# jianwen-xie/Latent-Space-Normalizing-Flow

Measured on NVIDIA B200. Metric: langevin_latent_steps_per_sec, higher is better.
Workload: dtype fp16-hi/lo-3pass-fwd+bf16-hi/lo-3pass-bwd/f32-accumulate (fp32-equivalent)

## Files before the change

### include/lsnf.h

```cpp
#ifndef LSNF_H_
#define LSNF_H_

#include <stddef.h>
#include <stdint.h>

#ifdef __cplusplus
extern "C" {
#endif

#define LSNF_ABI_VERSION 1

typedef struct lsnf_plan lsnf_plan;
typedef void* lsnf_stream;

typedef enum lsnf_status {
  LSNF_OK = 0,
  LSNF_ERR_INVALID = -1,
  LSNF_ERR_CUDA = -2,
  LSNF_ERR_STATE = -3,
  LSNF_ERR_UNSUPPORTED = -4
} lsnf_status;

typedef enum lsnf_arch {
  LSNF_ARCH_NONE = -1,
  LSNF_ARCH_SVHN = 0,
  LSNF_ARCH_CIFAR10 = 1,
  LSNF_ARCH_CELEBA_CROP = 2,
  LSNF_ARCH_CELEBA_HQ256 = 3
} lsnf_arch;

typedef enum lsnf_gemm_impl {
  LSNF_GEMM_TCGEN05 = 0,
  LSNF_GEMM_SIMT = 1
} lsnf_gemm_impl;

typedef struct lsnf_config {
  int32_t arch;
  int32_t batch;
  int32_t nz;
  int32_t ngf;
  int32_t nc;
  int32_t f_depth;
  int32_t f_width;
  int32_t f_permutation;
  int32_t f_coupling;
  float leak;
  int32_t gemm_impl;
  int32_t bwd_passes;
  int32_t train;
  int32_t reserved[3];
} lsnf_config;

#define LSNF_FLOW_PTRS_PER_STEP 12

int lsnf_abi_version(void);
const char* lsnf_last_error(void);

int lsnf_plan_create(const lsnf_config* cfg, lsnf_plan** out);
void lsnf_plan_destroy(lsnf_plan* plan);
size_t lsnf_workspace_bytes(const lsnf_plan* plan);
int lsnf_plan_bind(lsnf_plan* plan, void* workspace, size_t bytes);

int lsnf_pack_generator_weights(lsnf_plan* plan, const float* const* weights, const float* const* biases,
                                int32_t n_layers, lsnf_stream stream);
int lsnf_pack_flow_weights(lsnf_plan* plan, const float* const* params, const int32_t* const* perm,
                           const int32_t* const* perm_inverse, const float* log_abs_det,
                           const float* const* w_inverse, lsnf_stream stream);

int lsnf_generator_forward(lsnf_plan* plan, const float* z, float* x_hat, lsnf_stream stream);
int lsnf_generator_dgrad(lsnf_plan* plan, const float* x, float sigma, float* grad_z, lsnf_stream stream);
int lsnf_flow_forward(lsnf_plan* plan, const float* z, float* z_out, float* logdet, float* logp,
                      float* grad_z, lsnf_stream stream);
int lsnf_flow_inverse(lsnf_plan* plan, const float* eps, float* z, float* neg_objective, lsnf_stream stream);
int lsnf_langevin_update(lsnf_plan* plan, float* z, const float* grad_g, const float* grad_f, float step_size,
                         const float* eps, int32_t with_noise, uint64_t seed, uint64_t sample_offset,
                         uint32_t step, float* gnorms, lsnf_stream stream);

int lsnf_langevin_run(lsnf_plan* plan, const float* z0, const float* x, int32_t steps, float step_size,
                      float sigma, int32_t with_noise, const float* eps, uint64_t seed, uint64_t sample_offset,
                      float* z_out, float* gnorms, lsnf_stream stream);
int lsnf_sample_prior(lsnf_plan* plan, const float* eps, float* x, float* z, int32_t to_unit_range, lsnf_stream stream);
size_t lsnf_generator_grad_floats(const lsnf_plan* plan);
int lsnf_generator_grad_layout(const lsnf_plan* plan, int64_t* offsets, int64_t* sizes);
int lsnf_generator_param_grads(lsnf_plan* plan, const float* z, const float* x, int32_t global_batch, float* grads,
                               float* loss, int32_t part, lsnf_stream stream);
size_t lsnf_flow_grad_floats(const lsnf_plan* plan);
int lsnf_flow_grad_layout(const lsnf_plan* plan, int64_t* offsets, int64_t* sizes);
int lsnf_flow_param_grads(lsnf_plan* plan, const float* z, int32_t global_batch, float* grads, float* loss,
                          lsnf_stream stream);
int lsnf_generator_vjp(lsnf_plan* plan, const float* grad_x_hat, float* grad_z, float* grads, lsnf_stream stream);
int lsnf_flow_vjp(lsnf_plan* plan, const float* z, const float* grad_z_out, const float* grad_logdet, float* grad_z,
                  float* grads, lsnf_stream stream);

int lsnf_adam_step(int32_t n_tensors, float* const* params, const float* const* grads, float* const* exp_avg,
                   float* const* exp_avg_sq, const int64_t* sizes, const int32_t* grad_kk, const int32_t* grad_inner,
                   float lr, float beta1, float beta2, float eps, float weight_decay, int64_t step,
                   const float* grad_scale, lsnf_stream stream);

int lsnf_plan_run_stage(lsnf_plan* plan, int32_t index, lsnf_stream stream);
int lsnf_langevin_launch_count(const lsnf_plan* plan, int32_t steps);

#define LSNF_MAX_TAPS 16
#define LSNF_MAX_PHASES 4

typedef struct lsnf_tap {
  int32_t dy, dx;
  int32_t plane;
  int32_t brow;
} lsnf_tap;

typedef struct lsnf_stage_info {
  int32_t kind;
  int32_t layer;
  int32_t grid_h, grid_w;
  int32_t box_b, box_h, box_w;
  int32_t k_per_tap;
  int32_t n_valid, n_pad;
  int32_t block_n;
  int32_t n_phases;
  int32_t n_taps[LSNF_MAX_PHASES];
  lsnf_tap taps[LSNF_MAX_PHASES][LSNF_MAX_TAPS];
  int32_t out_mul;
  int32_t out_off_y[LSNF_MAX_PHASES], out_off_x[LSNF_MAX_PHASES];
  int32_t out_phase_split;
  int32_t out_channels;
  int32_t epilogue;
  int32_t k_splits;
  int32_t a_planes;
  int32_t a_h, a_w;
  int32_t tap_gen_k;
  int32_t b_k;
  int32_t b_rows;
  int32_t operand_fp16;
  int32_t passes;
  int64_t a_offset, b_offset, out_offset;
  int64_t flops;
} lsnf_stage_info;

int lsnf_plan_num_stages(const lsnf_plan* plan);
int lsnf_plan_stage_info(const lsnf_plan* plan, int32_t index, lsnf_stage_info* out);
int lsnf_plan_pack_index(const lsnf_plan* plan, int32_t index, int32_t ci, int32_t co, int32_t ky, int32_t kx,
                         int64_t* row, int64_t* col);

#define LSNF_KERNEL_SINGLE 0
#define LSNF_KERNEL_PAIR 1
typedef struct lsnf_launch_info {
  int32_t kernel;
  int32_t grid_x, grid_y, grid_z, block;
  int32_t ring_stages;
  int32_t stage_bytes;
  int32_t smem_bytes;
  int32_t ctas_per_sm;
  int32_t tmem_columns;
  int32_t tma_store;
  int32_t stream_k;
  int32_t reserved[4];
} lsnf_launch_info;
int lsnf_plan_stage_launch_info(const lsnf_plan* plan, int32_t index, int32_t num_sms, lsnf_launch_info* out);

#ifdef __cplusplus
}
#endif
#endif
```

### latent-space-normalizing-flow_b200/_cabi.py

```python
from __future__ import annotations

import ctypes as C
import os

_HERE = os.path.dirname(os.path.abspath(__file__))
LIB_PATH = os.environ.get("LSNF_LIB") or os.path.join(_HERE, "_lib", "liblsnf_b200.so")
_lib = None

LSNF_MAX_TAPS = 16
LSNF_MAX_PHASES = 4
FLOW_PTRS_PER_STEP = 12

ARCH = {"none": -1, "svhn": 0, "cifar10": 1, "celeba_crop": 2, "celeba_hq256": 3}
GEMM_TCGEN05, GEMM_SIMT = 0, 1


class Config(C.Structure):
    _fields_ = [("arch", C.c_int32), ("batch", C.c_int32), ("nz", C.c_int32), ("ngf", C.c_int32), ("nc", C.c_int32),
                ("f_depth", C.c_int32), ("f_width", C.c_int32), ("f_permutation", C.c_int32),
                ("f_coupling", C.c_int32), ("leak", C.c_float), ("gemm_impl", C.c_int32),
                ("bwd_passes", C.c_int32), ("train", C.c_int32), ("reserved", C.c_int32 * 3)]


class Tap(C.Structure):
    _fields_ = [("dy", C.c_int32), ("dx", C.c_int32), ("plane", C.c_int32), ("brow", C.c_int32)]


class StageInfo(C.Structure):
    _fields_ = [("kind", C.c_int32), ("layer", C.c_int32), ("grid_h", C.c_int32), ("grid_w", C.c_int32),
                ("box_b", C.c_int32), ("box_h", C.c_int32), ("box_w", C.c_int32), ("k_per_tap", C.c_int32),
                ("n_valid", C.c_int32), ("n_pad", C.c_int32), ("block_n", C.c_int32), ("n_phases", C.c_int32),
                ("n_taps", C.c_int32 * LSNF_MAX_PHASES), ("taps", (Tap * LSNF_MAX_TAPS) * LSNF_MAX_PHASES),
                ("out_mul", C.c_int32), ("out_off_y", C.c_int32 * LSNF_MAX_PHASES),
                ("out_off_x", C.c_int32 * LSNF_MAX_PHASES), ("out_phase_split", C.c_int32),
                ("out_channels", C.c_int32), ("epilogue", C.c_int32), ("k_splits", C.c_int32),
                ("a_planes", C.c_int32), ("a_h", C.c_int32), ("a_w", C.c_int32), ("tap_gen_k", C.c_int32),
                ("b_k", C.c_int32), ("b_rows", C.c_int32), ("operand_fp16", C.c_int32), ("passes", C.c_int32),
                ("a_offset", C.c_int64), ("b_offset", C.c_int64), ("out_offset", C.c_int64), ("flops", C.c_int64)]


class LaunchInfo(C.Structure):
    _fields_ = [("kernel", C.c_int32), ("grid_x", C.c_int32), ("grid_y", C.c_int32), ("grid_z", C.c_int32),
                ("block", C.c_int32), ("ring_stages", C.c_int32), ("stage_bytes", C.c_int32),
                ("smem_bytes", C.c_int32), ("ctas_per_sm", C.c_int32), ("tmem_columns", C.c_int32),
                ("tma_store", C.c_int32), ("stream_k", C.c_int32), ("reserved", C.c_int32 * 4)]


KERNEL_SINGLE, KERNEL_PAIR = 0, 1

EXPORTS = {
    "lsnf_abi_version": (C.c_int, []),
    "lsnf_last_error": (C.c_char_p, []),
    "lsnf_plan_create": (C.c_int, [C.POINTER(Config), C.POINTER(C.c_void_p)]),
    "lsnf_plan_destroy": (None, [C.c_void_p]),
    "lsnf_workspace_bytes": (C.c_size_t, [C.c_void_p]),
    "lsnf_plan_bind": (C.c_int, [C.c_void_p, C.c_void_p, C.c_size_t]),
    "lsnf_pack_generator_weights": (C.c_int, [C.c_void_p, C.POINTER(C.c_void_p), C.POINTER(C.c_void_p), C.c_int32,
                                              C.c_void_p]),
    "lsnf_pack_flow_weights": (C.c_int, [C.c_void_p, C.POINTER(C.c_void_p), C.POINTER(C.c_void_p),
                                         C.POINTER(C.c_void_p), C.c_void_p, C.POINTER(C.c_void_p), C.c_void_p]),
    "lsnf_generator_forward": (C.c_int, [C.c_void_p, C.c_void_p, C.c_void_p, C.c_void_p]),
    "lsnf_generator_dgrad": (C.c_int, [C.c_void_p, C.c_void_p, C.c_float, C.c_void_p, C.c_void_p]),
    "lsnf_flow_forward": (C.c_int, [C.c_void_p, C.c_void_p, C.c_void_p, C.c_void_p, C.c_void_p, C.c_void_p,
                                    C.c_void_p]),
    "lsnf_flow_inverse": (C.c_int, [C.c_void_p, C.c_void_p, C.c_void_p, C.c_void_p, C.c_void_p]),
    "lsnf_langevin_update": (C.c_int, [C.c_void_p, C.c_void_p, C.c_void_p, C.c_void_p, C.c_float, C.c_void_p,
                                       C.c_int32, C.c_uint64, C.c_uint64, C.c_uint32, C.c_void_p, C.c_void_p]),
    "lsnf_langevin_run": (C.c_int, [C.c_void_p, C.c_void_p, C.c_void_p, C.c_int32, C.c_float, C.c_float, C.c_int32,
                                    C.c_void_p, C.c_uint64, C.c_uint64, C.c_void_p, C.c_void_p, C.c_void_p]),
    "lsnf_sample_prior": (C.c_int, [C.c_void_p, C.c_void_p, C.c_void_p, C.c_void_p, C.c_int32, C.c_void_p]),
    "lsnf_generator_grad_floats": (C.c_size_t, [C.c_void_p]),
    "lsnf_generator_grad_layout": (C.c_int, [C.c_void_p, C.POINTER(C.c_int64), C.POINTER(C.c_int64)]),
    "lsnf_generator_param_grads": (C.c_int, [C.c_void_p, C.c_void_p, C.c_void_p, C.c_int32, C.c_void_p, C.c_void_p,
                                             C.c_int32, C.c_void_p]),
    "lsnf_flow_grad_floats": (C.c_size_t, [C.c_void_p]),
    "lsnf_flow_grad_layout": (C.c_int, [C.c_void_p, C.POINTER(C.c_int64), C.POINTER(C.c_int64)]),
    "lsnf_flow_param_grads": (C.c_int, [C.c_void_p, C.c_void_p, C.c_int32, C.c_void_p, C.c_void_p, C.c_void_p]),
    "lsnf_generator_vjp": (C.c_int, [C.c_void_p, C.c_void_p, C.c_void_p, C.c_void_p, C.c_void_p]),
    "lsnf_flow_vjp": (C.c_int, [C.c_void_p, C.c_void_p, C.c_void_p, C.c_void_p, C.c_void_p, C.c_void_p, C.c_void_p]),
    "lsnf_adam_step": (C.c_int, [C.c_int32, C.POINTER(C.c_void_p), C.POINTER(C.c_void_p), C.POINTER(C.c_void_p),
                                 C.POINTER(C.c_void_p), C.POINTER(C.c_int64), C.POINTER(C.c_int32),
                                 C.POINTER(C.c_int32), C.c_float, C.c_float, C.c_float, C.c_float, C.c_float,
                                 C.c_int64, C.c_void_p, C.c_void_p]),
    "lsnf_plan_run_stage": (C.c_int, [C.c_void_p, C.c_int32, C.c_void_p]),
    "lsnf_langevin_launch_count": (C.c_int, [C.c_void_p, C.c_int32]),
    "lsnf_plan_num_stages": (C.c_int, [C.c_void_p]),
    "lsnf_plan_stage_info": (C.c_int, [C.c_void_p, C.c_int32, C.POINTER(StageInfo)]),
    "lsnf_plan_pack_index": (C.c_int, [C.c_void_p, C.c_int32, C.c_int32, C.c_int32, C.c_int32, C.c_int32,
                                       C.POINTER(C.c_int64), C.POINTER(C.c_int64)]),
    "lsnf_plan_stage_launch_info": (C.c_int, [C.c_void_p, C.c_int32, C.c_int32, C.POINTER(LaunchInfo)]),
}


def load():
    global _lib
    if _lib is not None:
        return _lib
    if not os.path.exists(LIB_PATH):
        raise RuntimeError(
            f"lsnf_b200: native library {LIB_PATH} is missing -- build it with "
            "`python __graft_entry__.py` (nvcc, sm_100a). There is no CPU or PyTorch fallback for the Langevin path.")
    lib = C.CDLL(LIB_PATH)
    for name, (res, args) in EXPORTS.items():
        fn = getattr(lib, name)
        fn.restype = res
        fn.argtypes = args
    if lib.lsnf_abi_version() != 1:
        raise RuntimeError("lsnf_b200: ABI version mismatch between _cabi.py and the built library")
    _lib = lib
    return lib


def check(rc: int, what: str):
    if rc != 0:
        msg = load().lsnf_last_error()
        raise RuntimeError(f"lsnf_b200: {what} failed ({rc}): {msg.decode() if msg else ''}")


def ptr_array(ptrs):
    arr = (C.c_void_p * len(ptrs))(*[C.c_void_p(p) for p in ptrs])
    return arr
```

### latent-space-normalizing-flow_b200/csrc/lsnf_internal.cuh

```cuda
#pragma once
#include <cuda.h>
#include <cuda_bf16.h>
#include <cuda_fp16.h>
#include <cuda_runtime.h>
#include <stdint.h>

#include <string>
#include <vector>

#include "lsnf.h"

namespace lsnf {

constexpr int BLOCK_M = 128;
constexpr int BLOCK_K = 64;

enum Epilogue : int32_t {
  EPI_ACT_HL = 0,
  EPI_OUT_TANH = 1,
  EPI_GRAD_HL = 2,
  EPI_PARTIAL = 3
};

struct TapDev {
  int16_t dy, dx, plane;
  int16_t bsh;
  int32_t brow;
};

struct PhaseDev {
  int32_t ntaps;
  int32_t mo, no;
  TapDev taps[LSNF_MAX_TAPS];
};

struct StageDev {
  const __nv_bfloat16* a;
  const __nv_bfloat16* b;
  int32_t aP, B, Hg, Wg, Ka, b_rows;
  int32_t aH, aW, tap_gen, b_k;
  int32_t bB, bH, bW;
  int32_t tiles_b, tiles_h, tiles_w;
  int32_t n_valid, n_pad, block_n;
  int32_t nphase, ksplit, it_per_split;
  int32_t epi, bias_mod, oC, ms, split;
  float leak;
  const float* bias;
  void* out;
  uint32_t* mbits;
  int64_t sP, sB, sH, sW, sPos;
  int32_t nc, Ho, Wo, pad_;
  int32_t fp16, out_fp16;
  int32_t passes, out_single;
  const float* descale;
  int64_t rows_total;
  float* sk_slots;
  int32_t* sk_flags;
  int32_t sk_enable;
  int32_t wgrad;
  int32_t out_tma, nst;
  PhaseDev ph[LSNF_MAX_PHASES];
};

struct StageHost {
  lsnf_stage_info info;
  StageDev dev;
  CUtensorMap tmA, tmB, tmO;
  bool maps_ready = false;
  int layer = 0;
  int kind = 0;
  int k = 0, s = 0, p = 0, ci = 0, co = 0;
  size_t a_off = 0, b_off = 0, out_off = 0, mbits_off = 0, bias_off = 0;
  size_t b_bytes = 0;
  bool last = false, first = false;
  int num_sms = 148;
};

struct FlowLayout {
  int nz, w, n_out, half;
  size_t an_b, an_e, an_ei, W, WT, Winv, W1, W1T, b1, e1, W2, W2T, b2, e2, W3, W3T, b3, e3, perm, perm_inv, ld_const;
  size_t step_floats;
  size_t vec_floats;
  size_t max_mat;
  size_t step_mat;
};

struct FlowStash {
  size_t y, u1, a1, a2, h, gu, gp1, gp2, gp3, gx, gl0, gl1, gl2, gl3;
  size_t layer_floats;
};

struct FlowGradLayout {
  size_t off[LSNF_FLOW_PTRS_PER_STEP];
  size_t size[LSNF_FLOW_PTRS_PER_STEP];
  size_t step_floats;
};

struct TransArgs {
  const uint16_t* src;
  uint16_t* dst;
  int P, B, H, W, C;
  long long s_plane, s_b, s_h, s_w;
  int src_fp16, src_single;
  int Hp, Wp, halo;
  long long Kp;
  int c_rows;
  int xvar;
};

struct FinalizeArgs {
  const float* part;
  float* out;
  long long s_tap, s_split, s_ci;
  int ksplit, kk, C_in, C_out;
  float scale;
};

struct RowSumArgs {
  const uint16_t* src;
  float* out;
  long long Kp;
  int nsel, C;
  float scale;
  int sel[64];
};

struct WgradLayer {
  StageHost st;
  TransArgs ta, tg;
  size_t off_aT = 0, off_gT = 0, off_part = 0;
  int a_rows = 0, g_rows = 0, planes = 1, ntaps = 1, kk = 1, ksplit = 1;
  long long Kp = 0;
  size_t grad_w_off = 0, grad_b_off = 0;
  FinalizeArgs fin;
  RowSumArgs rs;
};

}

struct lsnf_plan {
  lsnf_config cfg;
  int n_layers = 0;
  int img = 0;
  int kp = 0;
  int nzp = 0;
  struct Layer { int ci, co, k, s, p, hin, hout; } layers[8];
  std::vector<lsnf::StageHost> stages;
  lsnf::FlowLayout fl;
  std::vector<lsnf::WgradLayer> wg;
  size_t gen_grad_floats = 0;
  bool wg_ready = false;
  lsnf::FlowStash fstash;
  lsnf::FlowGradLayout fgrad;
  size_t off_fstash = 0, off_fgrad = 0, off_floss = 0, off_flinalg = 0;
  size_t ws_bytes = 0;
  size_t off_zhl = 0, off_act[8] = {0}, off_gpre[8] = {0}, off_mbits[8] = {0}, off_xhat = 0, off_im2col = 0, off_partial = 0;
  size_t off_bias[8] = {0};
  size_t off_norms = 0, off_wscale = 0, off_dlast = 0;
  int dlast_pad = 0;
  size_t off_gradg = 0, off_gradf = 0, off_z = 0, off_flow = 0, off_scalars = 0, off_flow_out = 0;
  int ksplit_first = 1;
  char* ws = nullptr;
  bool bound = false, g_packed = false, f_packed = false, have_winv = false;
  int device = -1;
  int num_sms = 148;
  cudaStream_t side = nullptr;
  cudaEvent_t ev_fork = nullptr, ev_join = nullptr;
  struct LoopGraph { int steps; float step_size, sigma; int with_noise; cudaGraphExec_t exec; };
  std::vector<LoopGraph> graphs;
  cudaStream_t cap_stream = nullptr;
  size_t off_x = 0, off_gnorms = 0, off_dyn = 0, off_sk_slots = 0, off_sk_flags = 0;
  long long runs = 0;
  bool use_graphs = true;
  int graph_chunk = 40;
};

namespace lsnf {

__device__ __forceinline__ void split16(float v, bool fp16, uint16_t& hi, uint16_t& lo) {
  if (fp16) {
    const __half h = __float2half_rn(v);
    const __half l = __float2half_rn(v - __half2float(h));
    hi = __half_as_ushort(h); lo = __half_as_ushort(l);
  } else {
    const __nv_bfloat16 h = __float2bfloat16_rn(v);
    const __nv_bfloat16 l = __float2bfloat16_rn(v - __bfloat162float(h));
    hi = __bfloat16_as_ushort(h); lo = __bfloat16_as_ushort(l);
  }
}
__device__ __forceinline__ float join16(uint16_t hi, uint16_t lo, bool fp16) {
  if (fp16) return __half2float(__ushort_as_half(hi)) + __half2float(__ushort_as_half(lo));
  return __bfloat162float(__ushort_as_bfloat16(hi)) + __bfloat162float(__ushort_as_bfloat16(lo));
}

void set_error(const std::string& msg);
int cuda_fail(cudaError_t e, const char* what);
#define LSNF_CUDA(call)                                       \
  do {                                                        \
    cudaError_t e__ = (call);                                 \
    if (e__ != cudaSuccess) return ::lsnf::cuda_fail(e__, #call); \
  } while (0)

__device__ __forceinline__ void pdl_wait() { asm volatile("griddepcontrol.wait;" ::: "memory"); }
__device__ __forceinline__ void pdl_trigger() { asm volatile("griddepcontrol.launch_dependents;" ::: "memory"); }

extern thread_local int g_launch_pdl;
struct PdlScope {
  explicit PdlScope(bool on) { g_launch_pdl = on ? 1 : 0; }
  ~PdlScope() { g_launch_pdl = 0; }
};

template <typename... KArgs, typename... Args>
inline cudaError_t launch_k(void (*kernel)(KArgs...), dim3 grid, dim3 block, size_t smem, cudaStream_t s,
                            Args&&... args) {
  cudaLaunchConfig_t cfg = {};
  cfg.gridDim = grid; cfg.blockDim = block; cfg.dynamicSmemBytes = smem; cfg.stream = s;
  cudaLaunchAttribute at[1];
  if (g_launch_pdl) {
    at[0].id = cudaLaunchAttributeProgrammaticStreamSerialization;
    at[0].val.programmaticStreamSerializationAllowed = 1;
    cfg.attrs = at; cfg.numAttrs = 1;
  }
  return cudaLaunchKernelEx(&cfg, kernel, static_cast<KArgs>(args)...);
}

int launch_tapgemm_simt(const StageHost& st, cudaStream_t s);
int launch_tapgemm_tc(const StageHost& st, cudaStream_t s);
int tc_encode_maps(lsnf_plan* plan, StageHost& st);
void tc_launch_info(const StageHost& st, int num_sms, lsnf_launch_info* out);
bool tc_stage_is_pair(const StageHost& st);
int launch_pack_stage(const lsnf_plan* plan, const StageHost& st, const float* w, cudaStream_t s);
int launch_split_z(const lsnf_plan* plan, const float* z, cudaStream_t s);
int launch_weight_scales(const lsnf_plan* plan, const float* const* weights, cudaStream_t s);
int launch_last_gather(const lsnf_plan* plan, float* out, int to_unit_range, cudaStream_t s);
int launch_recon_grad_im2col(const lsnf_plan* plan, const float* x, float seed_scale, int upstream, cudaStream_t s);
int launch_last_fused(const lsnf_plan* plan, const float* x, float seed_scale, cudaStream_t s);
int launch_transpose_hl(const TransArgs& a, cudaStream_t s);
int launch_wgrad_finalize(const FinalizeArgs& a, cudaStream_t s);
int launch_bias_rowsum(const RowSumArgs& a, cudaStream_t s);
int launch_mse_sum(const float* xh, const float* x, long long n, float scale, float* partial, unsigned int* ticket,
                   float* out, cudaStream_t s);
int launch_reduce_partial(const lsnf_plan* plan, float* grad_z, float scale, cudaStream_t s);
int launch_flow_pack(lsnf_plan* plan, const float* const* params, const int32_t* const* perm,
                     const int32_t* const* perm_inv, const float* log_abs_det, const float* const* winv,
                     cudaStream_t s);
int launch_flow_forward(const lsnf_plan* plan, const float* z, float* z_out, float* logdet, float* logp,
                        float* grad_z, cudaStream_t s);
int launch_flow_inverse(const lsnf_plan* plan, const float* eps, float* z, float* negobj, cudaStream_t s);
int flow_smem(const FlowLayout& f, int S, int depth, bool stash, bool both_passes, uint32_t* ring_floats,
              size_t* smem_bytes);
constexpr int FLOW_SMEM_BYTES = 227 * 1024;
int launch_adam(int n, float* const* params, const float* const* grads, float* const* m, float* const* v,
                const int64_t* sizes, const int32_t* grad_kk, const int32_t* grad_inner, float lr, float beta1,
                float beta2, float eps, float weight_decay, int64_t step, const float* grad_scale, cudaStream_t s);
int launch_flow_logdet_inverse(const lsnf_plan* plan, const float* const* params, float* winv, float* logdet,
                               cudaStream_t s);
int launch_flow_param_grads(const lsnf_plan* plan, const float* z, float inv_global_batch, float* grads, float* loss,
                            cudaStream_t s);
int launch_flow_vjp(const lsnf_plan* plan, const float* z, const float* seed_g, const float* seed_ld, float* grad_z,
                    float* grads, cudaStream_t s);
int launch_update(const lsnf_plan* plan, float* z, const float* gg, const float* partial, int nsplit, float gscale,
                  const float* gf, float step, const float* eps, int with_noise, uint64_t seed,
                  uint64_t sample_offset, uint32_t step_idx, const uint64_t* dyn, float* gnorms,
                  int write_zhl, cudaStream_t s);
int launch_set_dyn(const lsnf_plan* plan, uint64_t seed, uint64_t sample_offset, uint32_t base_step, cudaStream_t s);
int tc_prepare_device(int device);
int aux_prepare_device(int device);
int flow_prepare_device(int device);

inline float sigma_seed_scale(float sigma) {
  const float inv = 1.f / (sigma * sigma);
  float s = 1.f;
  while (s * 2.f <= inv && s < 16.f) s *= 2.f;
  return s;
}
inline float sigma_post_scale(float sigma) { return 1.f / (sigma * sigma) / sigma_seed_scale(sigma); }

struct PackGeom {
  int kind, first, last, k, ci, co, n_pad, ka;
};

__host__ __device__ inline bool pack_index(const PackGeom& g, int ci, int co, int ky, int kx, long long* row,
                                           long long* col) {
  const int tap = ky * g.k + kx;
  if (g.kind == 0) {
    if (g.first || g.last) {
      *row = (long long)tap * g.co + co;
      *col = ci;
    } else {
      *row = (long long)tap * g.n_pad + co;
      *col = ci;
    }
  } else {
    if (g.first) {
      *row = ci;
      *col = (long long)tap * g.co + co;
    } else if (g.last) {
      *row = ci;
      *col = (long long)tap * g.co + co;
    } else {
      *row = (long long)tap * g.n_pad + ci;
      *col = co;
    }
  }
  return true;
}

}
```

### latent-space-normalizing-flow_b200/csrc/plan.cu

```cuda
#include <algorithm>
#include <cstdio>
#include <cstdlib>
#include <cstring>

#include "lsnf_internal.cuh"

#ifndef LSNF_PDL_DEFAULT
#define LSNF_PDL_DEFAULT 1
#endif

namespace lsnf {

thread_local int g_launch_pdl = 0;
static thread_local std::string g_err;
void set_error(const std::string& msg) { g_err = msg; }
int cuda_fail(cudaError_t e, const char* what) {
  g_err = std::string("CUDA error: ") + cudaGetErrorString(e) + " in " + what;
  return LSNF_ERR_CUDA;
}

static size_t align_up(size_t v, size_t a) { return (v + a - 1) / a * a; }

static int fail(int code, const std::string& msg) {
  set_error(msg);
  return code;
}

static int arch_layers(const lsnf_config& c, lsnf_plan::Layer* L) {
  const int nz = c.nz, g = c.ngf, nc = c.nc;
  auto set = [&](int i, int ci, int co, int k, int s, int p) { L[i] = {ci, co, k, s, p, 0, 0}; };
  switch (c.arch) {
    case LSNF_ARCH_NONE:
      return 0;
    case LSNF_ARCH_SVHN:
      set(0, nz, g * 8, 4, 1, 0); set(1, g * 8, g * 4, 4, 2, 1); set(2, g * 4, g * 2, 4, 2, 1);
      set(3, g * 2, nc, 4, 2, 1);
      return 4;
    case LSNF_ARCH_CIFAR10:
      set(0, nz, g * 8, 8, 1, 0); set(1, g * 8, g * 4, 4, 2, 1); set(2, g * 4, g * 2, 4, 2, 1);
      set(3, g * 2, nc, 3, 1, 1);
      return 4;
    case LSNF_ARCH_CELEBA_CROP:
      set(0, nz, g * 8, 4, 1, 0); set(1, g * 8, g * 4, 4, 2, 1); set(2, g * 4, g * 2, 4, 2, 1);
      set(3, g * 2, g, 4, 2, 1); set(4, g, nc, 4, 2, 1);
      return 5;
    case LSNF_ARCH_CELEBA_HQ256:
      set(0, nz, g * 16, 4, 1, 0); set(1, g * 16, g * 8, 4, 2, 1); set(2, g * 8, g * 4, 4, 2, 1);
      set(3, g * 4, g * 2, 4, 2, 1); set(4, g * 2, g, 4, 2, 1); set(5, g, g, 4, 2, 1); set(6, g, nc, 4, 2, 1);
      return 7;
    default:
      return -1;
  }
}

static int pick_block_n(int n) {
  if (n % 256 == 0) return 256;
  if (n % 128 == 0) return 128;
  return 64;
}

static int pick_block_n_hidden(int n, int rows, int phases, int k_blocks) {
  const int bn = pick_block_n(n);
  if (bn != 256 || k_blocks > 32) return bn;
  const int mtiles = (rows + BLOCK_M - 1) / BLOCK_M;
  const int pair_tiles = (mtiles + 1) / 2 * (n / 256) * phases;
  const int small_tiles = mtiles * (n / 128) * phases;
  return (pair_tiles <= 37 && small_tiles <= 2 * 148) ? 128 : 256;
}

static void make_box(int hg, int wg, int* bb, int* bh, int* bw) {
  *bw = std::min(wg, BLOCK_M);
  *bh = std::min(hg, BLOCK_M / *bw);
  *bb = BLOCK_M / (*bw * *bh);
}

static int up2_fwd_taps(int py, int px, int n_pad, lsnf_tap* t) {
  int n = 0;
  for (int ky = 0; ky < 4; ++ky) {
    if (((ky + 1) & 1) != py) continue;
    const int dy = (py + 1 - ky) / 2;
    for (int kx = 0; kx < 4; ++kx) {
      if (((kx + 1) & 1) != px) continue;
      const int dx = (px + 1 - kx) / 2;
      t[n++] = {dy, dx, 0, (ky * 4 + kx) * n_pad};
    }
  }
  return n;
}

static int up2_bwd_taps(int n_pad, lsnf_tap* t) {
  int n = 0;
  for (int ky = 0; ky < 4; ++ky) {
    const int oy_off = ky - 1;
    const int py = oy_off & 1, dy = (oy_off - py) / 2;
    for (int kx = 0; kx < 4; ++kx) {
      const int ox_off = kx - 1;
      const int px = ox_off & 1, dx = (ox_off - px) / 2;
      t[n++] = {dy, dx, py * 2 + px, (ky * 4 + kx) * n_pad};
    }
  }
  return n;
}

static void fill_dev(lsnf_plan* p, StageHost& st) {
  const lsnf_stage_info& I = st.info;
  StageDev& d = st.dev;
  memset(&d, 0, sizeof(d));
  d.aP = I.a_planes; d.B = p->cfg.batch; d.Hg = I.grid_h; d.Wg = I.grid_w; d.Ka = I.k_per_tap;
  d.bB = I.box_b; d.bH = I.box_h; d.bW = I.box_w;
  d.aH = I.a_h; d.aW = I.a_w; d.tap_gen = I.tap_gen_k; d.b_k = I.b_k; d.b_rows = I.b_rows;
  d.tiles_b = (d.B + d.bB - 1) / d.bB; d.tiles_h = d.Hg / d.bH; d.tiles_w = d.Wg / d.bW;
  d.n_valid = I.n_valid; d.n_pad = I.n_pad; d.block_n = I.block_n;
  d.nphase = I.n_phases; d.ksplit = I.k_splits;
  {
    const int ntaps0 = I.tap_gen_k ? I.tap_gen_k * I.tap_gen_k : I.n_taps[0];
    const int total = ntaps0 * (I.k_per_tap / BLOCK_K);
    d.it_per_split = (total + I.k_splits - 1) / I.k_splits;
  }
  d.epi = I.epilogue; d.oC = I.out_channels; d.ms = I.out_mul; d.split = I.out_phase_split;
  d.leak = p->cfg.leak;
  d.fp16 = I.operand_fp16; d.passes = I.passes;
  const bool single_bwd = p->cfg.bwd_passes == 1;
  d.out_fp16 = (I.epilogue == EPI_ACT_HL || single_bwd) ? 1 : 0;
  d.out_single = (I.epilogue == EPI_GRAD_HL && single_bwd) ? 1 : 0;
  d.rows_total = (int64_t)p->cfg.batch * I.grid_h * I.grid_w;
  for (int ph = 0; ph < I.n_phases; ++ph) {
    d.ph[ph].ntaps = I.tap_gen_k ? I.tap_gen_k * I.tap_gen_k : I.n_taps[ph];
    d.ph[ph].mo = I.out_off_y[ph]; d.ph[ph].no = I.out_off_x[ph];
    for (int t = 0; t < I.n_taps[ph]; ++t) {
      const lsnf_tap& s = I.taps[ph][t];
      d.ph[ph].taps[t] = {(int16_t)s.dy, (int16_t)s.dx, (int16_t)s.plane, 0, s.brow};
    }
  }
}

}

using namespace lsnf;

extern "C" int lsnf_abi_version(void) { return LSNF_ABI_VERSION; }
extern "C" const char* lsnf_last_error(void) { return g_err.c_str(); }

extern "C" int lsnf_plan_create(const lsnf_config* cfg, lsnf_plan** out) {
  if (!cfg || !out) return fail(LSNF_ERR_INVALID, "null argument");
  const lsnf_config& c = *cfg;
  if (c.batch <= 0) return fail(LSNF_ERR_INVALID, "batch must be positive");
  if (c.nz <= 0 || (c.nz & 1)) return fail(LSNF_ERR_INVALID, "nz must be even (model.py:383)");
  if (c.nz % 4) return fail(LSNF_ERR_INVALID, "nz must be a multiple of 4 (128-bit latent rows)");
  if (c.nz > 256) return fail(LSNF_ERR_INVALID, "nz > 256 is not supported");
  if (c.f_depth <= 0 || c.f_depth > 32) return fail(LSNF_ERR_INVALID, "f_depth out of range");
  if (c.f_width <= 0 || c.f_width > 256 || c.f_width % 4) return fail(LSNF_ERR_INVALID, "f_width must be a multiple of 4, <= 256");
  if (c.f_permutation != 1 && c.f_permutation != 2)
    return fail(LSNF_ERR_UNSUPPORTED, "f_flow_permutation must be 1 or 2 (model.py:372-379)");
  if (c.f_coupling != 0 && c.f_coupling != 1)
    return fail(LSNF_ERR_UNSUPPORTED, "f_flow_coupling must be 0 or 1 (model.py:384-387)");
  if (c.gemm_impl != LSNF_GEMM_TCGEN05 && c.gemm_impl != LSNF_GEMM_SIMT) return fail(LSNF_ERR_INVALID, "bad gemm_impl");
  if (c.bwd_passes != 0 && c.bwd_passes != 1 && c.bwd_passes != 3) return fail(LSNF_ERR_INVALID, "bwd_passes must be 0, 1 or 3");

  lsnf_plan* p = new lsnf_plan();
  p->cfg = c;
  const int L = arch_layers(c, p->layers);
  if (L < 0) { delete p; return fail(LSNF_ERR_INVALID, "unknown arch (model.py:154 raises ValueError)"); }
  p->n_layers = L;
  p->kp = (int)align_up(c.nz, BLOCK_K);
  p->nzp = (int)align_up(c.nz, 128);
  const int B = c.batch;

  if (L > 0) {
    if (c.nc <= 0 || c.nc > 4) { delete p; return fail(LSNF_ERR_INVALID, "nc must be in 1..4"); }
    if (c.ngf <= 0) { delete p; return fail(LSNF_ERR_INVALID, "ngf must be positive"); }
    int h = 1;
    for (int l = 0; l < L; ++l) {
      auto& y = p->layers[l];
      y.hin = h;
      y.hout = (h - 1) * y.s - 2 * y.p + y.k;
      h = y.hout;
      if (l < L - 1 && y.co % BLOCK_K) {
        delete p;
        return fail(LSNF_ERR_INVALID, "hidden generator channel counts must be multiples of 64 (raise --ngf)");
      }
      if (y.hin > 128) { delete p; return fail(LSNF_ERR_INVALID, "layer grid wider than 128 not supported"); }
    }
    p->img = h;
  }

  size_t off = 0;
  auto take = [&](size_t bytes) { size_t o = off; off = align_up(off + bytes, 1024); return o; };
  p->off_z = take((size_t)B * c.nz * 4);
  p->off_gradg = take((size_t)B * c.nz * 4);
  p->off_gradf = take((size_t)B * c.nz * 4);
  p->off_scalars = take(256);
  p->off_dyn = take(64);
  p->off_gnorms = take(64);
  p->off_norms = take((size_t)2 * B * 4);
  p->off_flow_out = take((size_t)B * (c.nz + 2) * 4);
  {
    FlowLayout& f = p->fl;
    f.nz = c.nz; f.w = c.f_width; f.half = c.nz / 2; f.n_out = c.f_coupling ? c.nz : c.nz / 2;
    size_t o = 0;
    auto tk = [&](size_t n) { size_t r = o; o += (n + 3) / 4 * 4; return r; };
    f.an_b = tk(f.nz); f.an_e = tk(f.nz); f.an_ei = tk(f.nz);
    f.b1 = tk(f.w); f.e1 = tk(f.w); f.b2 = tk(f.w); f.e2 = tk(f.w); f.b3 = tk(f.n_out); f.e3 = tk(f.n_out);
    f.perm = tk(f.nz); f.perm_inv = tk(f.nz); f.ld_const = tk(4);
    f.vec_floats = o;
    f.W = tk((size_t)f.nz * f.nz); f.WT = tk((size_t)f.nz * f.nz); f.Winv = tk((size_t)f.nz * f.nz);
    f.W1 = tk((size_t)f.half * f.w); f.W1T = tk((size_t)f.half * f.w);
    f.W2 = tk((size_t)f.w * f.w); f.W2T = tk((size_t)f.w * f.w);
    f.W3 = tk((size_t)f.w * f.n_out); f.W3T = tk((size_t)f.w * f.n_out);
    const size_t w_floats = c.f_permutation == 2 ? (size_t)f.nz * f.nz : 0;
    f.max_mat = std::max({w_floats, (size_t)f.half * f.w, (size_t)f.w * f.w, (size_t)f.w * f.n_out});
    f.step_mat = w_floats + (size_t)f.half * f.w + (size_t)f.w * f.w + (size_t)f.w * f.n_out;
    f.step_floats = o;
    uint32_t ring_floats;
    size_t smem_bytes;
    if (flow_smem(f, 1, c.f_depth, true, true, &ring_floats, &smem_bytes)) {
      delete p;
      return fail(LSNF_ERR_INVALID,
                  "flow prior exceeds the " + std::to_string(FLOW_SMEM_BYTES / 1024) +
                      " KB of shared memory of one CTA even at one sample per CTA: its largest matrix (f_width^2, or "
                      "nz^2 with f_flow_permutation 2) plus f_depth * (2 f_width + nz) stashed activations must fit "
                      "(include/lsnf.h, lsnf_config)");
    }
    p->off_flow = take(f.step_floats * 4 * c.f_depth);
    FlowStash& t = p->fstash;
    size_t so = 0;
    auto ts = [&](size_t n) { size_t r = so; so += n; return r; };
    t.y = ts(f.nz); t.u1 = ts(f.half); t.a1 = ts(f.w); t.a2 = ts(f.w); t.h = ts(f.n_out);
    t.gu = ts(f.nz); t.gp1 = ts(f.w); t.gp2 = ts(f.w); t.gp3 = ts(f.n_out); t.gx = ts(f.nz);
    t.gl0 = ts(f.nz); t.gl1 = ts(f.w); t.gl2 = ts(f.w); t.gl3 = ts(f.n_out);
    t.layer_floats = so;
    p->off_fstash = take(so * 4 * (size_t)B * c.f_depth);
    p->off_flinalg = take(((size_t)c.f_depth * f.nz * f.nz + 32) * 4);
    FlowGradLayout& gl = p->fgrad;
    const size_t sizes[LSNF_FLOW_PTRS_PER_STEP] = {
        (size_t)f.nz, (size_t)f.nz, (size_t)f.nz * f.nz, (size_t)f.half * f.w, (size_t)f.w, (size_t)f.w,
        (size_t)f.w * f.w, (size_t)f.w, (size_t)f.w, (size_t)f.w * f.n_out, (size_t)f.n_out, (size_t)f.n_out};
    size_t go = 0;
    for (int i = 0; i < LSNF_FLOW_PTRS_PER_STEP; ++i) { gl.off[i] = go; gl.size[i] = sizes[i]; go += (sizes[i] + 3) / 4 * 4; }
    gl.step_floats = go;
  }

  if (L > 0) {
    p->off_zhl = take((size_t)B * 2 * p->kp * 2);
    p->off_sk_slots = take((size_t)160 * 128 * 256 * 4);
    p->off_sk_flags = take((size_t)160 * 8 * 4);
    p->off_x = take((size_t)B * c.nc * p->img * p->img * 4);
    for (int l = 0; l < L - 1; ++l) {
      const auto& y = p->layers[l];
      const size_t bytes = (size_t)B * y.hout * y.hout * 2 * y.co * 2;
      p->off_act[l] = take(bytes);
      p->off_gpre[l] = take(bytes);
      p->off_mbits[l] = take((size_t)B * y.hout * y.hout * y.co / 8);
    }
    for (int l = 0; l < L; ++l) p->off_bias[l] = take((size_t)p->layers[l].co * 4);
    p->off_xhat = take((size_t)B * c.nc * p->img * p->img * 4);
    p->off_wscale = take((size_t)L * 16);
    {
      const auto& ylast = p->layers[L - 1];
      const int kk = ylast.k * ylast.k * ylast.co;
      p->off_dlast = take((size_t)B * ylast.hin * ylast.hin * (kk <= 32 ? 32 : 64) * 4);
    }
    const auto& yl = p->layers[L - 1];
    p->off_im2col = take((size_t)B * yl.hin * yl.hin * 2 * BLOCK_K * 2);

    p->stages.resize(2 * L);
    for (int l = 0; l < L; ++l) {
      const auto& y = p->layers[l];
      StageHost& st = p->stages[l];
      lsnf_stage_info& I = st.info;
      memset(&I, 0, sizeof(I));
      st.layer = l; st.kind = 0; st.k = y.k; st.s = y.s; st.p = y.p; st.ci = y.ci; st.co = y.co;
      st.first = (l == 0); st.last = (l == L - 1);
      I.kind = 0; I.layer = l;
      I.a_planes = 1;
      I.k_splits = 1;
      if (st.first) {
        if (!(y.s == 1 && y.p == 0)) { delete p; return fail(LSNF_ERR_INVALID, "first layer must be s1 p0"); }
        if (st.last) { delete p; return fail(LSNF_ERR_INVALID, "single-layer generator not supported"); }
        I.grid_h = I.grid_w = 1;
        I.k_per_tap = p->kp;
        I.n_valid = y.k * y.k * y.co; I.n_pad = I.n_valid; I.block_n = pick_block_n(y.co);
        I.n_phases = 1; I.n_taps[0] = 1; I.taps[0][0] = {0, 0, 0, 0};
        I.out_mul = 1; I.out_channels = y.co; I.epilogue = EPI_ACT_HL;
        st.a_off = p->off_zhl;
      } else {
        I.grid_h = I.grid_w = y.hin;
        I.k_per_tap = y.ci;
        I.out_channels = y.co;
        if (st.last) {
          if (!((y.k == 4 && y.s == 2 && y.p == 1) || (y.k == 3 && y.s == 1 && y.p == 1))) {
            delete p; return fail(LSNF_ERR_INVALID, "unsupported last-layer geometry");
          }
          I.n_valid = y.k * y.k * y.co; I.n_pad = I.n_valid <= 32 ? 32 : 64; I.block_n = I.n_pad;
          I.epilogue = EPI_PARTIAL; I.out_channels = I.n_pad;
          I.n_phases = 1; I.out_mul = 1; I.n_taps[0] = 1; I.taps[0][0] = {0, 0, 0, 0};
          p->dlast_pad = I.n_pad;
        } else {
          I.n_valid = I.n_pad = y.co; I.epilogue = EPI_ACT_HL;
          I.block_n = pick_block_n_hidden(y.co, B * y.hin * y.hin, (y.k == 4 && y.s == 2) ? 4 : 1,
                                          ((y.k == 4 && y.s == 2) ? 4 : y.k * y.k) * (y.ci / BLOCK_K));
        }
        if (st.last) {
        } else if (y.k == 4 && y.s == 2 && y.p == 1) {
          I.n_phases = 4; I.out_mul = 2;
          for (int ph = 0; ph < 4; ++ph) {
            I.n_taps[ph] = up2_fwd_taps(ph >> 1, ph & 1, I.n_pad, I.taps[ph]);
            I.out_off_y[ph] = ph >> 1; I.out_off_x[ph] = ph & 1;
          }
        } else if (y.k == 3 && y.s == 1 && y.p == 1) {
          I.n_phases = 1; I.out_mul = 1; I.n_taps[0] = 9;
          for (int ky = 0; ky < 3; ++ky)
            for (int kx = 0; kx < 3; ++kx) I.taps[0][ky * 3 + kx] = {1 - ky, 1 - kx, 0, (ky * 3 + kx) * I.n_pad};
        } else { delete p; return fail(LSNF_ERR_INVALID, "unsupported ConvTranspose2d geometry"); }
        st.a_off = p->off_act[l - 1];
      }
      make_box(I.grid_h, I.grid_w, &I.box_b, &I.box_h, &I.box_w);
      const int total_taps = (st.first || st.last) ? 1 : y.k * y.k;
      const size_t b_rows = (st.first || st.last) ? (size_t)I.n_pad : (size_t)total_taps * I.n_pad;
      I.operand_fp16 = 1; I.passes = 3;
      I.a_h = I.grid_h; I.a_w = I.grid_w; I.tap_gen_k = 0; I.b_k = I.k_per_tap; I.b_rows = (int)b_rows;
      st.b_bytes = b_rows * 2 * I.k_per_tap * 2;
      st.b_off = take(st.b_bytes);
      st.out_off = st.last ? p->off_dlast : p->off_act[l];
      st.mbits_off = st.last ? 0 : p->off_mbits[l];
      st.bias_off = p->off_bias[l];
      I.a_offset = st.a_off; I.b_offset = st.b_off; I.out_offset = st.out_off;
      int taps_sum = 0;
      for (int ph = 0; ph < I.n_phases; ++ph) taps_sum += I.n_taps[ph];
      I.flops = 2LL * B * I.grid_h * I.grid_w * (long long)I.n_valid * I.k_per_tap * taps_sum;
      if (st.first) I.flops = 2LL * B * (long long)I.n_valid * c.nz;
      if (st.last) I.flops = 2LL * B * I.grid_h * I.grid_w * (long long)y.k * y.k * y.co * y.ci;
      fill_dev(p, st);
      StageDev& d = st.dev;
      d.bias_mod = y.co;
      if (st.last) {
        d.nc = c.nc; d.Ho = y.hout; d.Wo = y.hout;
        d.bias = nullptr;
      } else {
        d.sW = 2 * y.co; d.sH = (int64_t)y.hout * d.sW; d.sB = (int64_t)y.hout * d.sH; d.sPos = d.sW; d.sP = 0;
      }
    }
    for (int l = L - 1; l >= 0; --l) {
      const auto& y = p->layers[l];
      StageHost& st = p->stages[L + (L - 1 - l)];
      lsnf_stage_info& I = st.info;
      memset(&I, 0, sizeof(I));
      st.layer = l; st.kind = 1; st.k = y.k; st.s = y.s; st.p = y.p; st.ci = y.ci; st.co = y.co;
      st.first = (l == 0); st.last = (l == L - 1);
      I.kind = 1; I.layer = l; I.a_planes = 1; I.k_splits = 1;
      I.n_phases = 1; I.out_mul = 1;
      size_t b_rows;
      if (st.last) {
        if (y.k * y.k * y.co > BLOCK_K) { delete p; return fail(LSNF_ERR_INVALID, "k*k*nc must be <= 64"); }
        I.grid_h = I.grid_w = y.hin;
        I.k_per_tap = BLOCK_K;
        I.n_valid = I.n_pad = y.ci; I.block_n = pick_block_n(y.ci);
        I.n_taps[0] = 1; I.taps[0][0] = {0, 0, 0, 0};
        st.a_off = p->off_im2col;
        b_rows = I.n_pad;
      } else if (st.first) {
        I.grid_h = I.grid_w = 1;
        I.k_per_tap = y.co;
        I.n_valid = c.nz; I.n_pad = p->nzp; I.block_n = 128;
        I.n_taps[0] = 0;
        st.a_off = p->off_gpre[0];
        b_rows = I.n_pad;
        const int kblocks = y.k * y.k * y.co / BLOCK_K;
        const int mtiles = (B + BLOCK_M - 1) / BLOCK_M;
        int want = std::max(1, (148 + mtiles - 1) / mtiles);
        int per = std::max(2, (kblocks + want - 1) / want);
        I.k_splits = (kblocks + per - 1) / per;
        per = (kblocks + I.k_splits - 1) / I.k_splits;
        I.k_splits = (kblocks + per - 1) / per;
        p->ksplit_first = I.k_splits;
      } else {
        if (!(y.k == 4 && y.s == 2 && y.p == 1)) { delete p; return fail(LSNF_ERR_INVALID, "unsupported hidden layer geometry"); }
        I.grid_h = I.grid_w = y.hin;
        I.k_per_tap = y.co;
        I.n_valid = I.n_pad = y.ci; I.block_n = pick_block_n_hidden(y.ci, B * y.hin * y.hin, 1, 16 * (y.co / BLOCK_K));
        I.a_planes = 4;
        I.n_taps[0] = up2_bwd_taps(I.n_pad, I.taps[0]);
        st.a_off = p->off_gpre[l];
        b_rows = (size_t)16 * I.n_pad;
      }
      make_box(I.grid_h, I.grid_w, &I.box_b, &I.box_h, &I.box_w);
      const size_t b_k = st.first ? (size_t)y.k * y.k * y.co : (size_t)I.k_per_tap;
      I.operand_fp16 = c.bwd_passes == 1 ? 1 : 0; I.passes = c.bwd_passes == 1 ? 1 : 3;
      I.a_h = st.first ? y.k : I.grid_h; I.a_w = st.first ? y.k : I.grid_w;
      I.tap_gen_k = st.first ? y.k : 0; I.b_k = (int)b_k; I.b_rows = (int)b_rows;
      st.b_bytes = b_rows * 2 * b_k * 2;
      st.b_off = take(st.b_bytes);
      if (st.first) {
        I.epilogue = EPI_PARTIAL; I.out_channels = I.n_pad;
      } else {
        I.epilogue = EPI_GRAD_HL; I.out_channels = y.ci;
        I.out_phase_split = (l - 1 > 0) ? 1 : 0;
        st.out_off = p->off_gpre[l - 1];
        st.mbits_off = p->off_mbits[l - 1];
      }
      I.a_offset = st.a_off; I.b_offset = st.b_off; I.out_offset = st.out_off;
      I.flops = 2LL * B * I.grid_h * I.grid_w * (long long)I.n_valid *
                (st.last ? y.k * y.k * y.co : (st.first ? (long long)y.k * y.k * y.co : 16LL * y.co));
      fill_dev(p, st);
      StageDev& d = st.dev;
      if (!st.first) {
        const int hg = I.grid_h;
        d.sW = 2 * y.ci;
        if (I.out_phase_split) {
          d.sH = (int64_t)(hg / 2) * d.sW; d.sB = (int64_t)(hg / 2) * d.sH; d.sP = (int64_t)B * d.sB;
        } else {
          d.sH = (int64_t)hg * d.sW; d.sB = (int64_t)hg * d.sH; d.sP = 0;
        }
      }
    }
    p->off_partial = take((size_t)p->ksplit_first * B * p->nzp * 4);
    p->stages[2 * L - 1].out_off = p->off_partial;
    p->stages[2 * L - 1].info.out_offset = p->off_partial;
  }
  if (L > 0 && c.train) {
    p->wg.resize(L);
    size_t goff = 0;
    for (int l = 0; l < L; ++l) {
      const auto& y = p->layers[l];
      WgradLayer& w = p->wg[l];
      const bool first = (l == 0), last = (l == L - 1);
      const int kk = y.k * y.k;
      const bool single = c.bwd_passes == 1;
      w.kk = kk;
      int n_cols, hp, wp, halo, block_n;
      TransArgs& ta = w.ta;
      TransArgs& tg = w.tg;
      memset(&ta, 0, sizeof(ta)); memset(&tg, 0, sizeof(tg));
      if (first) {
        w.a_rows = (int)align_up(c.nz, 128); hp = wp = 1; halo = 0;
        w.Kp = (long long)align_up(B, BLOCK_K);
        w.planes = 1; w.g_rows = kk * y.co; w.ntaps = 1; n_cols = kk * y.co; block_n = pick_block_n(n_cols);
        ta.P = 1; ta.B = B; ta.H = ta.W = 1; ta.C = p->kp; ta.s_b = 2 * p->kp; ta.src_fp16 = 1; ta.c_rows = w.a_rows;
        tg.P = kk; tg.B = B; tg.H = tg.W = 1; tg.C = y.co; tg.s_plane = 2 * y.co; tg.s_b = (long long)kk * 2 * y.co;
        tg.c_rows = y.co;
      } else if (last) {
        w.a_rows = y.ci; hp = wp = y.hin; halo = 0;
        w.Kp = (long long)align_up((size_t)B * y.hin * y.hin, BLOCK_K);
        w.planes = 1; w.g_rows = BLOCK_K; w.ntaps = 1; n_cols = BLOCK_K; block_n = 64;
        ta.P = 1; ta.B = B; ta.H = ta.W = y.hin; ta.C = y.ci; ta.s_w = 2 * y.ci; ta.s_h = (long long)y.hin * ta.s_w;
        ta.s_b = (long long)y.hin * ta.s_h; ta.src_fp16 = 1; ta.c_rows = y.ci;
        tg.P = 1; tg.B = B; tg.H = tg.W = y.hin; tg.C = BLOCK_K; tg.s_w = 2 * BLOCK_K; tg.s_h = (long long)y.hin * tg.s_w;
        tg.s_b = (long long)y.hin * tg.s_h; tg.c_rows = BLOCK_K;
      } else {
        w.a_rows = y.ci; hp = y.hin + 2; wp = (int)align_up(y.hin, 8); halo = 1;
        w.Kp = (long long)align_up((size_t)B * hp * wp, BLOCK_K);
        w.planes = 8; w.g_rows = y.co; w.ntaps = 16; n_cols = y.co; block_n = pick_block_n(y.co);
        ta.P = 1; ta.B = B; ta.H = ta.W = y.hin; ta.C = y.ci; ta.s_w = 2 * y.ci; ta.s_h = (long long)y.hin * ta.s_w;
        ta.s_b = (long long)y.hin * ta.s_h; ta.src_fp16 = 1; ta.c_rows = y.ci;
        tg.P = 4; tg.B = B; tg.H = tg.W = y.hin; tg.C = y.co; tg.s_w = 2 * y.co; tg.s_h = (long long)y.hin * tg.s_w;
        tg.s_b = (long long)y.hin * tg.s_h; tg.s_plane = (long long)B * tg.s_b; tg.c_rows = y.co; tg.xvar = 1;
      }
      ta.Hp = tg.Hp = hp; ta.Wp = tg.Wp = wp; ta.halo = tg.halo = halo; ta.Kp = tg.Kp = w.Kp;
      tg.src_fp16 = single ? 1 : 0; tg.src_single = single ? 1 : 0;
      w.off_aT = take((size_t)w.a_rows * 2 * w.Kp * 2);
      w.off_gT = take((size_t)w.planes * w.g_rows * 2 * w.Kp * 2);
      StageHost& st = w.st;
      lsnf_stage_info& I = st.info;
      memset(&I, 0, sizeof(I));
      st.layer = l; st.kind = 2; st.k = y.k; st.s = y.s; st.p = y.p; st.ci = y.ci; st.co = y.co;
      st.first = first; st.last = last;
      I.kind = 2; I.layer = l; I.grid_h = 1; I.grid_w = w.a_rows; I.box_b = 1; I.box_h = 1; I.box_w = BLOCK_M;
      I.k_per_tap = (int)w.Kp; I.n_valid = n_cols; I.block_n = block_n; I.n_pad = (int)align_up(n_cols, block_n);
      I.n_phases = 1; I.n_taps[0] = w.ntaps; I.out_mul = 1; I.out_channels = I.n_pad; I.epilogue = EPI_PARTIAL;
      I.a_planes = 1; I.a_h = 1; I.a_w = w.a_rows; I.b_k = (int)w.Kp; I.b_rows = w.planes * w.g_rows;
      I.operand_fp16 = 0; I.passes = 3;
      const int kblocks = (int)(w.Kp / BLOCK_K);
      const int tiles = ((w.a_rows + BLOCK_M - 1) / BLOCK_M) * (I.n_pad / block_n) * w.ntaps;
      int want = std::max(1, (2 * 148 + tiles - 1) / tiles);
      want = std::min(want, std::max(1, kblocks / 4));
      int per = (kblocks + want - 1) / want;
      w.ksplit = (kblocks + per - 1) / per;
      I.k_splits = w.ksplit;
      for (int t = 0; t < w.ntaps; ++t) I.taps[0][t] = {0, 0, 0, 0};
      I.flops = 2LL * w.a_rows * (long long)n_cols * w.Kp * w.ntaps;
      st.a_off = w.off_aT; st.b_off = w.off_gT;
      w.off_part = take((size_t)w.ntaps * w.ksplit * w.a_rows * I.n_pad * 4);
      st.out_off = w.off_part;
      I.a_offset = st.a_off; I.b_offset = st.b_off; I.out_offset = st.out_off;
      fill_dev(p, st);
      StageDev& d = st.dev;
      d.B = 1; d.tiles_b = 1; d.tiles_h = 1; d.tiles_w = (w.a_rows + BLOCK_M - 1) / BLOCK_M;
      d.rows_total = w.a_rows; d.wgrad = 1; d.it_per_split = per;
      if (!first && !last) {
        lsnf_tap tp[16];
        up2_bwd_taps(y.co, tp);
        for (int t = 0; t < 16; ++t) {
          d.ph[0].taps[t].dy = 0; d.ph[0].taps[t].dx = 0; d.ph[0].taps[t].plane = 0;
          d.ph[0].taps[t].bsh = (int16_t)(tp[t].dy * wp);
          d.ph[0].taps[t].brow = (tp[t].plane * 2 + (tp[t].dx != 0 ? 1 : 0)) * y.co;
        }
      }
      w.grad_w_off = goff; goff += align_up((size_t)y.ci * y.co * kk, 4);
      w.grad_b_off = goff; goff += align_up((size_t)y.co, 4);
      FinalizeArgs& f = w.fin;
      memset(&f, 0, sizeof(f));
      f.ksplit = w.ksplit; f.kk = kk; f.C_in = y.ci; f.C_out = y.co;
      if (first) { f.s_tap = y.co; f.s_split = 0; f.s_ci = I.n_pad; f.ksplit = 1; }
      else if (last) { f.s_tap = y.co; f.s_split = (long long)w.a_rows * I.n_pad; f.s_ci = I.n_pad; }
      else { f.s_tap = (long long)w.ksplit * w.a_rows * I.n_pad; f.s_split = (long long)w.a_rows * I.n_pad; f.s_ci = I.n_pad; }
      RowSumArgs& r = w.rs;
      memset(&r, 0, sizeof(r));
      r.Kp = w.Kp; r.C = y.co;
      if (first) { r.nsel = kk; for (int t = 0; t < kk; ++t) r.sel[t] = t * y.co; }
      else if (last) {
        r.nsel = 0;
        for (int ky = 0; ky < y.k; ++ky)
          for (int kx = 0; kx < y.k; ++kx) {
            const bool once_y = y.s == 1 ? ky == y.p : (ky == 1 || ky == 2);
            const bool once_x = y.s == 1 ? kx == y.p : (kx == 1 || kx == 2);
            if (once_y && once_x) r.sel[r.nsel++] = (ky * y.k + kx) * y.co;
          }
      } else { r.nsel = 4; for (int q = 0; q < 4; ++q) r.sel[q] = 2 * q * y.co; }
      if (first && w.ksplit != 1) {  }
    }
    p->gen_grad_floats = goff;
  }
  p->ws_bytes = off;
  *out = p;
  return LSNF_OK;
}

extern "C" void lsnf_plan_destroy(lsnf_plan* plan) {
  if (!plan) return;
  if (plan->side) cudaStreamDestroy(plan->side);
  if (plan->ev_fork) cudaEventDestroy(plan->ev_fork);
  if (plan->ev_join) cudaEventDestroy(plan->ev_join);
  for (auto& g : plan->graphs) cudaGraphExecDestroy(g.exec);
  if (plan->cap_stream) cudaStreamDestroy(plan->cap_stream);
  delete plan;
}

extern "C" size_t lsnf_workspace_bytes(const lsnf_plan* plan) { return plan ? plan->ws_bytes : 0; }

extern "C" int lsnf_plan_num_stages(const lsnf_plan* plan) { return plan ? (int)plan->stages.size() : 0; }

extern "C" int lsnf_plan_stage_info(const lsnf_plan* plan, int32_t index, lsnf_stage_info* out) {
  if (!plan || !out || index < 0 || index >= (int)plan->stages.size()) return fail(LSNF_ERR_INVALID, "bad stage index");
  *out = plan->stages[index].info;
  return LSNF_OK;
}

extern "C" int lsnf_plan_stage_launch_info(const lsnf_plan* plan, int32_t index, int32_t num_sms,
                                           lsnf_launch_info* out) {
  if (!plan || !out || index < 0 || index >= (int)plan->stages.size()) return fail(LSNF_ERR_INVALID, "bad stage index");
  if (num_sms < 2) return fail(LSNF_ERR_INVALID, "num_sms must be at least 2");
  tc_launch_info(plan->stages[index], num_sms, out);
  return LSNF_OK;
}

static PackGeom geom_of(const StageHost& st) {
  PackGeom g;
  g.kind = st.kind; g.first = st.first; g.last = st.last; g.k = st.k; g.ci = st.ci; g.co = st.co;
  g.n_pad = st.info.n_pad;
  g.ka = st.info.b_k;
  return g;
}

extern "C" int lsnf_plan_pack_index(const lsnf_plan* plan, int32_t index, int32_t ci, int32_t co, int32_t ky,
                                    int32_t kx, int64_t* row, int64_t* col) {
  if (!plan || index < 0 || index >= (int)plan->stages.size() || !row || !col) return fail(LSNF_ERR_INVALID, "bad argument");
  const StageHost& st = plan->stages[index];
  if (ci < 0 || ci >= st.ci || co < 0 || co >= st.co || ky < 0 || ky >= st.k || kx < 0 || kx >= st.k)
    return fail(LSNF_ERR_INVALID, "weight index out of range");
  long long r, c;
  pack_index(geom_of(st), ci, co, ky, kx, &r, &c);
  *row = r; *col = c;
  return LSNF_OK;
}

extern "C" int lsnf_plan_bind(lsnf_plan* plan, void* workspace, size_t bytes) {
  if (!plan || !workspace) return fail(LSNF_ERR_INVALID, "null argument");
  if (bytes < plan->ws_bytes) return fail(LSNF_ERR_INVALID, "workspace too small");
  if ((uintptr_t)workspace % 1024) return fail(LSNF_ERR_INVALID, "workspace must be 1024-byte aligned");
  int dev = -1;
  LSNF_CUDA(cudaGetDevice(&dev));
  cudaDeviceProp prop;
  LSNF_CUDA(cudaGetDeviceProperties(&prop, dev));
  if (prop.major != 10) return fail(LSNF_ERR_CUDA, "this library is built for sm_100a (B200) only");
  plan->device = dev;
  plan->num_sms = prop.multiProcessorCount;
  plan->ws = (char*)workspace;
  {
    int rc;
    if ((rc = tc_prepare_device(dev)) || (rc = aux_prepare_device(dev)) || (rc = flow_prepare_device(dev))) return rc;
  }
  for (auto& st : plan->stages) {
    StageDev& d = st.dev;
    st.num_sms = plan->num_sms;
    d.a = (const __nv_bfloat16*)(plan->ws + st.a_off);
    d.b = (const __nv_bfloat16*)(plan->ws + st.b_off);
    d.out = plan->ws + st.out_off;
    d.bias = (st.kind == 0 && !st.last) ? (const float*)(plan->ws + st.bias_off) : nullptr;
    d.sk_slots = (float*)(plan->ws + plan->off_sk_slots);
    d.sk_flags = (int32_t*)(plan->ws + plan->off_sk_flags);
    d.descale = (st.kind == 0 || plan->cfg.bwd_passes == 1) ? (const float*)(plan->ws + plan->off_wscale + (size_t)st.layer * 16 + 8) : nullptr;
    d.mbits = ((st.kind == 0 && !st.last) || (st.kind == 1 && !st.first)) ? (uint32_t*)(plan->ws + st.mbits_off) : nullptr;
    if (plan->cfg.gemm_impl == LSNF_GEMM_TCGEN05) {
      int rc = tc_encode_maps(plan, st);
      if (rc) return rc;
    }
  }
  for (auto& w : plan->wg) {
    StageHost& st = w.st;
    StageDev& d = st.dev;
    st.num_sms = plan->num_sms;
    d.a = (const __nv_bfloat16*)(plan->ws + st.a_off);
    d.b = (const __nv_bfloat16*)(plan->ws + st.b_off);
    d.out = plan->ws + st.out_off;
    d.bias = nullptr; d.descale = nullptr; d.mbits = nullptr;
    d.sk_slots = nullptr; d.sk_flags = nullptr;
    int rc = tc_encode_maps(plan, st);
    if (rc) return rc;
    w.ta.dst = (uint16_t*)(plan->ws + w.off_aT);
    w.tg.dst = (uint16_t*)(plan->ws + w.off_gT);
    w.fin.part = (const float*)(plan->ws + w.off_part);
    w.rs.src = (const uint16_t*)(plan->ws + w.off_gT);
  }
  if (!plan->side) {
    LSNF_CUDA(cudaStreamCreateWithFlags(&plan->side, cudaStreamNonBlocking));
    LSNF_CUDA(cudaEventCreateWithFlags(&plan->ev_fork, cudaEventDisableTiming));
    LSNF_CUDA(cudaEventCreateWithFlags(&plan->ev_join, cudaEventDisableTiming));
    LSNF_CUDA(cudaStreamCreateWithFlags(&plan->cap_stream, cudaStreamNonBlocking));
  }
  for (auto& g : plan->graphs) cudaGraphExecDestroy(g.exec);
  plan->graphs.clear();
  plan->runs = 0;
  {
    const char* e = getenv("LSNF_NO_GRAPH");
    plan->use_graphs = !(e && e[0] == '1');
    const char* c = getenv("LSNF_GRAPH_CHUNK");
    if (c && atoi(c) > 0) plan->graph_chunk = atoi(c);
  }
  plan->bound = true;
  plan->g_packed = plan->f_packed = false;
  return LSNF_OK;
}

static int need(const lsnf_plan* p, bool gen, bool flow) {
  if (!p) return fail(LSNF_ERR_INVALID, "null plan");
  if (!p->bound) return fail(LSNF_ERR_STATE, "lsnf_plan_bind has not been called");
  if (gen && p->n_layers == 0) return fail(LSNF_ERR_STATE, "plan has no generator (arch = none)");
  if (gen && !p->g_packed) return fail(LSNF_ERR_STATE, "generator weights not packed");
  if (flow && !p->f_packed) return fail(LSNF_ERR_STATE, "flow weights not packed");
  return 0;
}

static int run_stage(const lsnf_plan* p, const StageHost& st, cudaStream_t s) {
  return p->cfg.gemm_impl == LSNF_GEMM_TCGEN05 ? launch_tapgemm_tc(st, s) : launch_tapgemm_simt(st, s);
}

extern "C" int lsnf_pack_generator_weights(lsnf_plan* plan, const float* const* weights, const float* const* biases,
                                           int32_t n_layers, lsnf_stream stream) {
  if (!plan || !plan->bound) return fail(LSNF_ERR_STATE, "plan not bound");
  if (n_layers != plan->n_layers || !weights || !biases) return fail(LSNF_ERR_INVALID, "layer count mismatch");
  cudaStream_t s = (cudaStream_t)stream;
  {
    int rc = launch_weight_scales(plan, weights, s);
    if (rc) return rc;
  }
  for (auto& st : plan->stages) {
    int rc = launch_pack_stage(plan, st, weights[st.layer], s);
    if (rc) return rc;
  }
  for (int l = 0; l < plan->n_layers; ++l)
    LSNF_CUDA(cudaMemcpyAsync(plan->ws + plan->off_bias[l], biases[l], (size_t)plan->layers[l].co * 4,
                              cudaMemcpyDeviceToDevice, s));
  plan->g_packed = true;
  plan->wg_ready = false;
  return LSNF_OK;
}

extern "C" int lsnf_pack_flow_weights(lsnf_plan* plan, const float* const* params, const int32_t* const* perm,
                                      const int32_t* const* perm_inverse, const float* log_abs_det,
                                      const float* const* w_inverse, lsnf_stream stream) {
  if (!plan || !plan->bound) return fail(LSNF_ERR_STATE, "plan not bound");
  if (!params) return fail(LSNF_ERR_INVALID, "null argument");
  if (plan->cfg.f_permutation == 1 && (!perm || !perm_inverse)) return fail(LSNF_ERR_INVALID, "permutation indices missing");
  int rc;
  const float* winv_ptrs[32];
  if (!log_abs_det && plan->cfg.f_permutation == 2) {
    float* winv = (float*)(plan->ws + plan->off_flinalg);
    float* ld = winv + (size_t)plan->cfg.f_depth * plan->cfg.nz * plan->cfg.nz;
    if ((rc = launch_flow_logdet_inverse(plan, params, winv, ld, (cudaStream_t)stream))) return rc;
    for (int i = 0; i < plan->cfg.f_depth; ++i) winv_ptrs[i] = winv + (size_t)i * plan->cfg.nz * plan->cfg.nz;
    log_abs_det = ld;
    w_inverse = winv_ptrs;
  }
  rc = launch_flow_pack(plan, params, perm, perm_inverse, log_abs_det, w_inverse, (cudaStream_t)stream);
  if (rc) return rc;
  plan->f_packed = true;
  plan->have_winv = (w_inverse != nullptr) || plan->cfg.f_permutation == 1;
  return LSNF_OK;
}

static int gen_forward(lsnf_plan* p, const float* z, float* x_hat, cudaStream_t s, bool split) {
  int rc;
  if (split && (rc = launch_split_z(p, z, s))) return rc;
  for (int l = 0; l < p->n_layers; ++l)
    if ((rc = run_stage(p, p->stages[l], s))) return rc;
  if ((rc = launch_last_gather(p, nullptr, 0, s))) return rc;
  if (x_hat) {
    const size_t bytes = (size_t)p->cfg.batch * p->cfg.nc * p->img * p->img * 4;
    LSNF_CUDA(cudaMemcpyAsync(x_hat, p->ws + p->off_xhat, bytes, cudaMemcpyDeviceToDevice, s));
  }
  return LSNF_OK;
}

static int gen_dgrad_partial(lsnf_plan* p, const float* x, float sigma, cudaStream_t s) {
  int rc;
  if ((rc = launch_recon_grad_im2col(p, x, sigma_seed_scale(sigma), 0, s))) return rc;
  for (int i = p->n_layers; i < 2 * p->n_layers; ++i)
    if ((rc = run_stage(p, p->stages[i], s))) return rc;
  return LSNF_OK;
}

extern "C" int lsnf_plan_run_stage(lsnf_plan* plan, int32_t index, lsnf_stream stream) {
  int rc = need(plan, true, false);
  if (rc) return rc;
  if (index < 0 || index >= (int)plan->stages.size()) return fail(LSNF_ERR_INVALID, "bad stage index");
  return run_stage(plan, plan->stages[index], (cudaStream_t)stream);
}

extern "C" int lsnf_generator_forward(lsnf_plan* plan, const float* z, float* x_hat, lsnf_stream stream) {
  int rc = need(plan, true, false);
  if (rc) return rc;
  if (!z) return fail(LSNF_ERR_INVALID, "null z");
  return gen_forward(plan, z, x_hat, (cudaStream_t)stream, true);
}

extern "C" int lsnf_generator_dgrad(lsnf_plan* plan, const float* x, float sigma, float* grad_z, lsnf_stream stream) {
  int rc = need(plan, true, false);
  if (rc) return rc;
  if (!x || !grad_z || !(sigma > 0.f)) return fail(LSNF_ERR_INVALID, "bad argument");
  cudaStream_t s = (cudaStream_t)stream;
  if ((rc = gen_dgrad_partial(plan, x, sigma, s))) return rc;
  return launch_reduce_partial(plan, grad_z, sigma_post_scale(sigma), s);
}

extern "C" int lsnf_flow_forward(lsnf_plan* plan, const float* z, float* z_out, float* logdet, float* logp,
                                 float* grad_z, lsnf_stream stream) {
  int rc = need(plan, false, true);
  if (rc) return rc;
  if (!z) return fail(LSNF_ERR_INVALID, "null z");
  return launch_flow_forward(plan, z, z_out, logdet, logp, grad_z, (cudaStream_t)stream);
}

extern "C" int lsnf_flow_inverse(lsnf_plan* plan, const float* eps, float* z, float* neg_objective, lsnf_stream stream) {
  int rc = need(plan, false, true);
  if (rc) return rc;
  if (!eps || !z) return fail(LSNF_ERR_INVALID, "null argument");
  if (!plan->have_winv) return fail(LSNF_ERR_STATE, "flow weights were packed without w_inverse");
  return launch_flow_inverse(plan, eps, z, neg_objective, (cudaStream_t)stream);
}

extern "C" size_t lsnf_generator_grad_floats(const lsnf_plan* plan) { return plan ? plan->gen_grad_floats : 0; }

extern "C" int lsnf_generator_grad_layout(const lsnf_plan* plan, int64_t* offsets, int64_t* sizes) {
  if (!plan || !offsets || !sizes) return fail(LSNF_ERR_INVALID, "null argument");
  if (plan->wg.empty()) return fail(LSNF_ERR_STATE, "plan was created without lsnf_config.train");
  for (int l = 0; l < plan->n_layers; ++l) {
    const auto& y = plan->layers[l];
    offsets[2 * l] = (int64_t)plan->wg[l].grad_w_off; sizes[2 * l] = (int64_t)y.ci * y.co * y.k * y.k;
    offsets[2 * l + 1] = (int64_t)plan->wg[l].grad_b_off; sizes[2 * l + 1] = y.co;
  }
  return LSNF_OK;
}

static int sync_check(cudaStream_t s, const char* what, int l) {
  static const bool dbg = [] { const char* e = getenv("LSNF_SYNC_DEBUG"); return e && e[0] == '1'; }();
  if (!dbg) return 0;
  cudaError_t e = cudaStreamSynchronize(s);
  if (e == cudaSuccess) return 0;
  set_error(std::string("CUDA error: ") + cudaGetErrorString(e) + " after " + what + " of layer " + std::to_string(l));
  return LSNF_ERR_CUDA;
}

static int gen_layer_grads(lsnf_plan* plan, int l, float* grads, float scale, cudaStream_t s) {
  const int L = plan->n_layers;
  int rc;
  WgradLayer& w = plan->wg[l];
  TransArgs ta = w.ta, tg = w.tg;
  ta.src = (const uint16_t*)(plan->ws + (l == 0 ? plan->off_zhl : plan->off_act[l - 1]));
  tg.src = (const uint16_t*)(plan->ws + (l == L - 1 ? plan->off_im2col : plan->off_gpre[l]));
  if ((rc = launch_transpose_hl(ta, s)) || (rc = sync_check(s, "activation transpose", l))) return rc;
  if ((rc = launch_transpose_hl(tg, s)) || (rc = sync_check(s, "gradient transpose", l))) return rc;
  if ((rc = launch_tapgemm_tc(w.st, s)) || (rc = sync_check(s, "weight-gradient tap-GEMM", l))) return rc;
  FinalizeArgs f = w.fin;
  f.out = grads + w.grad_w_off; f.scale = scale;
  if ((rc = launch_wgrad_finalize(f, s)) || (rc = sync_check(s, "finalize", l))) return rc;
  RowSumArgs r = w.rs;
  r.out = grads + w.grad_b_off; r.scale = scale;
  if ((rc = launch_bias_rowsum(r, s)) || (rc = sync_check(s, "bias row sums", l))) return rc;
  return LSNF_OK;
}

extern "C" int lsnf_generator_param_grads(lsnf_plan* plan, const float* z, const float* x, int32_t global_batch,
                                          float* grads, float* loss, int32_t part, lsnf_stream stream) {
  int rc = need(plan, true, false);
  if (rc) return rc;
  if (plan->wg.empty()) return fail(LSNF_ERR_STATE, "plan was created without lsnf_config.train");
  if (plan->cfg.gemm_impl != LSNF_GEMM_TCGEN05) return fail(LSNF_ERR_UNSUPPORTED, "weight gradients need the tcgen05 path");
  if (!z || !x || !grads || global_batch <= 0) return fail(LSNF_ERR_INVALID, "bad argument");
  if (part < -2 || part >= plan->n_layers) return fail(LSNF_ERR_INVALID, "part must be -1 (all), -2 (prologue) or a layer");
  cudaStream_t s = (cudaStream_t)stream;
  const lsnf_config& c = plan->cfg;
  const int L = plan->n_layers;
  const bool prologue = part < 0, layers_all = part == -1;
  if (prologue) {
    if ((rc = gen_forward(plan, z, nullptr, s, true))) return rc;
    if ((rc = sync_check(s, "generator forward", -1))) return rc;
    const long long npix = (long long)c.batch * c.nc * plan->img * plan->img;
    if (loss && (rc = launch_mse_sum((const float*)(plan->ws + plan->off_xhat), x, npix, 1.f / (float)global_batch,
                                     (float*)(plan->ws + plan->off_flow_out),
                                     (unsigned int*)(plan->ws + plan->off_scalars + 64), loss, s)))
      return rc;
    if ((rc = launch_last_fused(plan, x, 1.f, s))) return rc;
    for (int i = L; i < 2 * L - 1; ++i)
      if ((rc = run_stage(plan, plan->stages[i], s))) return rc;
    if ((rc = sync_check(s, "data-gradient chain", -1))) return rc;
    plan->wg_ready = true;
    if (!layers_all) return LSNF_OK;
  }
  if (!plan->wg_ready)
    return fail(LSNF_ERR_STATE, "a layer's gradients were requested before the forward / data-gradient part (part = -2)");
  const float scale = 2.f / (float)global_batch;
  for (int l = L - 1; l >= 0; --l) {
    if (!layers_all && l != part) continue;
    if ((rc = gen_layer_grads(plan, l, grads, scale, s))) return rc;
  }
  return LSNF_OK;
}

extern "C" int lsnf_generator_vjp(lsnf_plan* plan, const float* grad_x_hat, float* grad_z, float* grads,
                                  lsnf_stream stream) {
  int rc = need(plan, true, false);
  if (rc) return rc;
  if (!grad_x_hat) return fail(LSNF_ERR_INVALID, "null grad_x_hat");
  if (plan->cfg.bwd_passes == 1)
    return fail(LSNF_ERR_UNSUPPORTED, "the vector-Jacobian product needs the 3-pass bf16 data gradient (bwd_passes 1 "
                                      "has fp16's range, too narrow for an arbitrary upstream gradient)");
  if (grads && plan->wg.empty()) return fail(LSNF_ERR_STATE, "plan was created without lsnf_config.train");
  if (grads && plan->cfg.gemm_impl != LSNF_GEMM_TCGEN05)
    return fail(LSNF_ERR_UNSUPPORTED, "weight gradients need the tcgen05 path");
  cudaStream_t s = (cudaStream_t)stream;
  const int L = plan->n_layers;
  if ((rc = launch_recon_grad_im2col(plan, grad_x_hat, 1.f, 1, s))) return rc;
  const int end = grad_z ? 2 * L : 2 * L - 1;
  for (int i = L; i < end; ++i)
    if ((rc = run_stage(plan, plan->stages[i], s))) return rc;
  if (grad_z && (rc = launch_reduce_partial(plan, grad_z, 1.f, s))) return rc;
  plan->wg_ready = false;
  if (grads)
    for (int l = L - 1; l >= 0; --l)
      if ((rc = gen_layer_grads(plan, l, grads, 1.f, s))) return rc;
  return LSNF_OK;
}

extern "C" size_t lsnf_flow_grad_floats(const lsnf_plan* plan) {
  return plan ? plan->fgrad.step_floats * (size_t)plan->cfg.f_depth : 0;
}

extern "C" int lsnf_flow_grad_layout(const lsnf_plan* plan, int64_t* offsets, int64_t* sizes) {
  if (!plan || !offsets || !sizes) return fail(LSNF_ERR_INVALID, "null argument");
  for (int L = 0; L < plan->cfg.f_depth; ++L)
    for (int i = 0; i < LSNF_FLOW_PTRS_PER_STEP; ++i) {
      offsets[L * LSNF_FLOW_PTRS_PER_STEP + i] = (int64_t)(L * plan->fgrad.step_floats + plan->fgrad.off[i]);
      sizes[L * LSNF_FLOW_PTRS_PER_STEP + i] = (int64_t)plan->fgrad.size[i];
    }
  return LSNF_OK;
}

extern "C" int lsnf_flow_param_grads(lsnf_plan* plan, const float* z, int32_t global_batch, float* grads, float* loss,
                                     lsnf_stream stream) {
  int rc = need(plan, false, true);
  if (rc) return rc;
  if (!z || !grads || global_batch <= 0) return fail(LSNF_ERR_INVALID, "bad argument");
  if (plan->cfg.f_permutation == 2 && !plan->have_winv)
    return fail(LSNF_ERR_STATE, "flow weights were packed without w_inverse (needed for d log|det W| / dW = W^-T)");
  return launch_flow_param_grads(plan, z, 1.f / (float)global_batch, grads, loss, (cudaStream_t)stream);
}

extern "C" int lsnf_flow_vjp(lsnf_plan* plan, const float* z, const float* grad_z_out, const float* grad_logdet,
                             float* grad_z, float* grads, lsnf_stream stream) {
  int rc = need(plan, false, true);
  if (rc) return rc;
  if (!z) return fail(LSNF_ERR_INVALID, "null z");
  if (grads && plan->cfg.f_permutation == 2 && !plan->have_winv)
    return fail(LSNF_ERR_STATE, "flow weights were packed without w_inverse (needed for d log|det W| / dW = W^-T)");
  cudaStream_t s = (cudaStream_t)stream;
  if (!grad_z_out && !grad_logdet) {
    if (grad_z) LSNF_CUDA(cudaMemsetAsync(grad_z, 0, (size_t)plan->cfg.batch * plan->cfg.nz * 4, s));
    if (grads) LSNF_CUDA(cudaMemsetAsync(grads, 0, lsnf_flow_grad_floats(plan) * 4, s));
    return LSNF_OK;
  }
  if (!grad_z && !grads) return LSNF_OK;
  return launch_flow_vjp(plan, z, grad_z_out, grad_logdet, grad_z, grads, s);
}

extern "C" int lsnf_adam_step(int32_t n_tensors, float* const* params, const float* const* grads, float* const* exp_avg,
                              float* const* exp_avg_sq, const int64_t* sizes, const int32_t* grad_kk,
                              const int32_t* grad_inner, float lr, float beta1, float beta2, float eps,
                              float weight_decay, int64_t step, const float* grad_scale, lsnf_stream stream) {
  if (n_tensors <= 0 || !params || !grads || !exp_avg || !exp_avg_sq || !sizes || step <= 0)
    return fail(LSNF_ERR_INVALID, "bad argument");
  return launch_adam(n_tensors, params, grads, exp_avg, exp_avg_sq, sizes, grad_kk, grad_inner, lr, beta1, beta2, eps,
                     weight_decay, step, grad_scale, (cudaStream_t)stream);
}

extern "C" int lsnf_sample_prior(lsnf_plan* plan, const float* eps, float* x, float* z, int32_t to_unit_range,
                                 lsnf_stream stream) {
  int rc = need(plan, true, true);
  if (rc) return rc;
  if (!eps || !x) return fail(LSNF_ERR_INVALID, "null argument");
  if (!plan->have_winv) return fail(LSNF_ERR_STATE, "flow weights were packed without w_inverse");
  cudaStream_t s = (cudaStream_t)stream;
  float* zw = (float*)(plan->ws + plan->off_z);
  if ((rc = launch_flow_inverse(plan, eps, zw, nullptr, s))) return rc;
  if ((rc = launch_split_z(plan, zw, s))) return rc;
  for (int l = 0; l < plan->n_layers; ++l)
    if ((rc = run_stage(plan, plan->stages[l], s))) return rc;
  if ((rc = launch_last_gather(plan, x, to_unit_range, s))) return rc;
  if (z) LSNF_CUDA(cudaMemcpyAsync(z, zw, (size_t)plan->cfg.batch * plan->cfg.nz * 4, cudaMemcpyDeviceToDevice, s));
  return LSNF_OK;
}

extern "C" int lsnf_langevin_update(lsnf_plan* plan, float* z, const float* grad_g, const float* grad_f,
                                    float step_size, const float* eps, int32_t with_noise, uint64_t seed,
                                    uint64_t sample_offset, uint32_t step, float* gnorms, lsnf_stream stream) {
  if (!plan || !plan->bound) return fail(LSNF_ERR_STATE, "plan not bound");
  if (!z || !grad_g || !grad_f) return fail(LSNF_ERR_INVALID, "null argument");
  return launch_update(plan, z, grad_g, nullptr, 0, 1.f, grad_f, step_size, eps, with_noise, seed, sample_offset, step,
                       nullptr, gnorms, 0, (cudaStream_t)stream);
}

extern "C" int lsnf_langevin_launch_count(const lsnf_plan* plan, int32_t steps) {
  if (!plan) return 0;
  const int chunks = steps > 0 ? (steps + plan->graph_chunk - 1) / plan->graph_chunk : 0;
  return 1 + steps * (2 * plan->n_layers + 3) + chunks;
}

struct LoopTrace {
  std::vector<cudaEvent_t> ev;
  std::vector<std::string> name;
  cudaStream_t s;
  bool on = false;
  void mark(const char* n) {
    if (!on) return;
    cudaEvent_t e;
    cudaEventCreate(&e);
    cudaEventRecord(e, s);
    ev.push_back(e);
    name.push_back(n);
  }
  void report() {
    if (!on || ev.empty()) return;
    cudaEventSynchronize(ev.back());
    float total = 0.f;
    cudaEventElapsedTime(&total, ev.front(), ev.back());
    fprintf(stderr, "[lsnf trace] one Langevin iteration: %.1f us\n", total * 1e3f);
    for (size_t i = 1; i < ev.size(); ++i) {
      float ms = 0.f;
      cudaEventElapsedTime(&ms, ev[i - 1], ev[i]);
      fprintf(stderr, "[lsnf trace]   %-28s %8.1f us\n", name[i].c_str(), ms * 1e3f);
    }
    for (auto e : ev) cudaEventDestroy(e);
    ev.clear();
    name.clear();
  }
};

static int langevin_loop(lsnf_plan* plan, const float* x, int steps, float step_size, float sigma, int with_noise,
                         const float* eps, uint64_t seed, uint64_t sample_offset, const uint64_t* dyn, float* gnorms,
                         cudaStream_t s) {
  const float gscale = sigma_post_scale(sigma);
  int rc;
  static int trace_env = -1;
  if (trace_env < 0) { const char* e = getenv("LSNF_TRACE"); trace_env = (e && e[0] == '1') ? 1 : 0; }
  LoopTrace tr;
  tr.s = s;
  const lsnf_config& c = plan->cfg;
  float* z = (float*)(plan->ws + plan->off_z);
  float* gf = (float*)(plan->ws + plan->off_gradf);
  const float* partial = (const float*)(plan->ws + plan->off_partial);
  static const int pdl_mode = [] { const char* e = getenv("LSNF_PDL"); return e ? atoi(e) : LSNF_PDL_DEFAULT; }();
  const bool tc_path = c.gemm_impl == LSNF_GEMM_TCGEN05;
  bool prev_pair = false, have_prev = false;
  auto pdl_ok = [&](bool this_pair) {
    bool ok = tc_path && have_prev && pdl_mode != 0;
    if (pdl_mode == 2) ok = ok && !this_pair && !prev_pair;
    if (pdl_mode == 3) ok = ok && !this_pair;
    if (pdl_mode == 4) ok = ok && !prev_pair;
    have_prev = true;
    prev_pair = this_pair;
    return ok;
  };
  for (int t = 0; t < steps; ++t) {
    tr.on = trace_env == 1 && t == 1 && !dyn;
    tr.mark("start");
    const int fork_at = plan->n_layers - 1;
    for (int l = 0; l < plan->n_layers; ++l) {
      if (l == fork_at) {
        LSNF_CUDA(cudaEventRecord(plan->ev_fork, s));
        LSNF_CUDA(cudaStreamWaitEvent(plan->side, plan->ev_fork, 0));
        if ((rc = launch_flow_forward(plan, z, nullptr, nullptr, nullptr, gf, plan->side))) return rc;
        LSNF_CUDA(cudaEventRecord(plan->ev_join, plan->side));
      }
      {
        PdlScope pdl(pdl_ok(tc_path && tc_stage_is_pair(plan->stages[l])));
        if ((rc = run_stage(plan, plan->stages[l], s))) return rc;
      }
      tr.mark(("forward layer " + std::to_string(l)).c_str());
    }
    {
      PdlScope pdl(pdl_ok(false));
      if ((rc = launch_last_fused(plan, x, sigma_seed_scale(sigma), s))) return rc;
    }
    tr.mark("gather + tanh + recon grad + im2col");
    for (int i = plan->n_layers; i < 2 * plan->n_layers; ++i) {
      {
        PdlScope pdl(pdl_ok(tc_path && tc_stage_is_pair(plan->stages[i])));
        if ((rc = run_stage(plan, plan->stages[i], s))) return rc;
      }
      tr.mark(("dgrad layer " + std::to_string(plan->stages[i].layer)).c_str());
    }
    LSNF_CUDA(cudaStreamWaitEvent(s, plan->ev_join, 0));
    tr.mark("join flow prior");
    const float* e = eps ? eps + (size_t)t * c.batch * c.nz : nullptr;
    if ((rc = launch_update(plan, z, nullptr, partial, plan->ksplit_first, gscale, gf, step_size, e, with_noise, seed,
                            sample_offset, (uint32_t)t, dyn, t == steps - 1 ? gnorms : nullptr, 1, s)))
      return rc;
    prev_pair = false;
    tr.mark("update");
    tr.report();
  }
  return LSNF_OK;
}

extern "C" int lsnf_langevin_run(lsnf_plan* plan, const float* z0, const float* x, int32_t steps, float step_size,
                                 float sigma, int32_t with_noise, const float* eps, uint64_t seed,
                                 uint64_t sample_offset, float* z_out, float* gnorms, lsnf_stream stream) {
  int rc = need(plan, true, true);
  if (rc) return rc;
  if (!z0 || !x || !z_out || steps < 0 || !(sigma > 0.f)) return fail(LSNF_ERR_INVALID, "bad argument");
  cudaStream_t s = (cudaStream_t)stream;
  const lsnf_config& c = plan->cfg;
  float* z = (float*)(plan->ws + plan->off_z);
  const size_t zbytes = (size_t)c.batch * c.nz * 4;
  LSNF_CUDA(cudaMemcpyAsync(z, z0, zbytes, cudaMemcpyDeviceToDevice, s));
  if ((rc = launch_split_z(plan, z, s))) return rc;
  const bool graph_ok = plan->use_graphs && !eps && steps > 0 && plan->runs > 0;
  plan->runs++;
  if (!graph_ok) {
    if ((rc = langevin_loop(plan, x, steps, step_size, sigma, with_noise, eps, seed, sample_offset, nullptr, gnorms, s)))
      return rc;
  } else {
    float* x_ws = (float*)(plan->ws + plan->off_x);
    float* gn_ws = (float*)(plan->ws + plan->off_gnorms);
    const uint64_t* dyn = (const uint64_t*)(plan->ws + plan->off_dyn);
    LSNF_CUDA(cudaMemcpyAsync(x_ws, x, (size_t)c.batch * c.nc * plan->img * plan->img * 4, cudaMemcpyDeviceToDevice, s));
    for (int done = 0; done < steps;) {
      const int n = std::min(steps - done, plan->graph_chunk);
      cudaGraphExec_t exec = nullptr;
      for (auto& g : plan->graphs)
        if (g.steps == n && g.step_size == step_size && g.sigma == sigma && g.with_noise == with_noise) exec = g.exec;
      if (!exec) {
        cudaGraph_t graph = nullptr;
        cudaStream_t cs = plan->cap_stream;
        LSNF_CUDA(cudaStreamBeginCapture(cs, cudaStreamCaptureModeThreadLocal));
        rc = langevin_loop(plan, x_ws, n, step_size, sigma, with_noise, nullptr, 0, 0, dyn, gn_ws, cs);
        cudaError_t ce = cudaStreamEndCapture(cs, &graph);
        if (rc) { if (graph) cudaGraphDestroy(graph); return rc; }
        if (ce != cudaSuccess) return cuda_fail(ce, "cudaStreamEndCapture");
        ce = cudaGraphInstantiate(&exec, graph, 0);
        cudaGraphDestroy(graph);
        if (ce != cudaSuccess) return cuda_fail(ce, "cudaGraphInstantiate");
        if (plan->graphs.size() >= 8) { cudaGraphExecDestroy(plan->graphs.front().exec); plan->graphs.erase(plan->graphs.begin()); }
        plan->graphs.push_back({n, step_size, sigma, with_noise, exec});
      }
      if ((rc = launch_set_dyn(plan, seed, sample_offset, (uint32_t)done, s))) return rc;
      LSNF_CUDA(cudaGraphLaunch(exec, s));
      done += n;
    }
    if (gnorms) LSNF_CUDA(cudaMemcpyAsync(gnorms, gn_ws, 8, cudaMemcpyDeviceToDevice, s));
  }
  LSNF_CUDA(cudaMemcpyAsync(z_out, z, zbytes, cudaMemcpyDeviceToDevice, s));
  return LSNF_OK;
}
```

### latent-space-normalizing-flow_b200/csrc/tapgemm_tc.cu

```cuda
#include <algorithm>
#include <cstdlib>
#include <mutex>
#include <type_traits>

#include "tapgemm_common.cuh"

namespace lsnf {

#ifndef LSNF_EXP_FWD2PASS
#define LSNF_EXP_FWD2PASS 0
#endif
constexpr int TC_EPI_WARPS = 8;
constexpr int TC_THREADS = 64 + 32 * TC_EPI_WARPS;
constexpr int A_TILE_BYTES = BLOCK_M * BLOCK_K * 2;
constexpr uint64_t L2_EVICT_FIRST = 0x12F0000000000000ull;
constexpr uint64_t L2_EVICT_LAST = 0x14F0000000000000ull;

constexpr int TC_MAX_STAGES = 8;
constexpr int TC_SMEM_EXTRA = 1024  + 256 ;
constexpr int TC_SMEM_MAX = 232448;
template <int BN>
struct TcCfg {
  static constexpr int B_TILE_BYTES = BN * BLOCK_K * 2;
  static constexpr int SPAN = BN >= 64 ? BN / 2 : BN;
  static constexpr int TMEM_COLS = BN < 32 ? 32 : BN;
  static constexpr bool TMA_EPI = BN >= 128;
};

__device__ __forceinline__ uint32_t smem_u32(const void* p) { return (uint32_t)__cvta_generic_to_shared(p); }

__device__ __forceinline__ void mbar_init(uint32_t bar, uint32_t count) {
  asm volatile("mbarrier.init.shared::cta.b64 [%0], %1;" ::"r"(bar), "r"(count));
}
__device__ __forceinline__ void mbar_wait(uint32_t bar, uint32_t parity) {
  asm volatile(
      "{\n"
      ".reg .pred P1;\n"
      "WAIT_LOOP:\n"
      "mbarrier.try_wait.parity.shared::cta.b64 P1, [%0], %1;\n"
      "@P1 bra DONE;\n"
      "bra WAIT_LOOP;\n"
      "DONE:\n"
      "}\n" ::"r"(bar), "r"(parity)
      : "memory");
}
__device__ __forceinline__ bool elect_one() {
  uint32_t pred;
  asm volatile(
      "{\n"
      ".reg .pred P;\n"
      "elect.sync _|P, 0xffffffff;\n"
      "selp.u32 %0, 1, 0, P;\n"
      "}\n"
      : "=r"(pred));
  return pred != 0;
}
__device__ __forceinline__ void mbar_expect_tx(uint32_t bar, uint32_t bytes) {
  asm volatile("mbarrier.arrive.expect_tx.shared::cta.b64 _, [%0], %1;" ::"r"(bar), "r"(bytes) : "memory");
}
__device__ __forceinline__ void tma_load_5d(uint32_t dst, const CUtensorMap* map, uint32_t bar, int c0, int c1, int c2,
                                            int c3, int c4) {
  asm volatile(
      "cp.async.bulk.tensor.5d.shared::cluster.global.mbarrier::complete_tx::bytes [%0], [%1, {%3, %4, %5, %6, %7}], [%2];"
      ::"r"(dst), "l"(map), "r"(bar), "r"(c0), "r"(c1), "r"(c2), "r"(c3), "r"(c4)
      : "memory");
}
__device__ __forceinline__ void tma_load_2d(uint32_t dst, const CUtensorMap* map, uint32_t bar, int c0, int c1) {
  asm volatile(
      "cp.async.bulk.tensor.2d.shared::cluster.global.mbarrier::complete_tx::bytes [%0], [%1, {%3, %4}], [%2];"
      ::"r"(dst), "l"(map), "r"(bar), "r"(c0), "r"(c1)
      : "memory");
}

__device__ __forceinline__ uint64_t umma_desc(uint32_t saddr) {
  uint64_t d = 0;
  d |= (uint64_t)((saddr & 0x3FFFF) >> 4);
  d |= (uint64_t)1 << 16;
  d |= (uint64_t)(1024 >> 4) << 32;
  d |= (uint64_t)1 << 46;
  d |= (uint64_t)2 << 61;
  return d;
}

template <int BN>
__device__ __forceinline__ uint32_t umma_idesc(bool fp16) {
  const uint32_t fmt = fp16 ? 0u : 1u;
  return (1u << 4) | (fmt << 7) | (fmt << 10) | ((uint32_t)(BN >> 3) << 17) | ((uint32_t)(BLOCK_M >> 4) << 24);
}

__device__ __forceinline__ void umma_bf16(uint32_t tmem_d, uint64_t da, uint64_t db, uint32_t idesc, uint32_t accum) {
  asm volatile(
      "{\n"
      ".reg .pred p;\n"
      "setp.ne.b32 p, %4, 0;\n"
      "tcgen05.mma.cta_group::1.kind::f16 [%0], %1, %2, %3, p;\n"
      "}\n" ::"r"(tmem_d), "l"(da), "l"(db), "r"(idesc), "r"(accum)
      : "memory");
}
__device__ __forceinline__ void umma_commit(uint32_t bar) {
  asm volatile("tcgen05.commit.cta_group::1.mbarrier::arrive::one.shared::cluster.b64 [%0];" ::"r"(bar) : "memory");
}

__device__ __forceinline__ void tmem_ld32(uint32_t taddr, uint32_t (&v)[32]) {
  asm volatile(
      "tcgen05.ld.sync.aligned.32x32b.x32.b32 "
      "{%0, %1, %2, %3, %4, %5, %6, %7, %8, %9, %10, %11, %12, %13, %14, %15, "
      "%16, %17, %18, %19, %20, %21, %22, %23, %24, %25, %26, %27, %28, %29, %30, %31}, [%32];"
      : "=r"(v[0]), "=r"(v[1]), "=r"(v[2]), "=r"(v[3]), "=r"(v[4]), "=r"(v[5]), "=r"(v[6]), "=r"(v[7]),
        "=r"(v[8]), "=r"(v[9]), "=r"(v[10]), "=r"(v[11]), "=r"(v[12]), "=r"(v[13]), "=r"(v[14]), "=r"(v[15]),
        "=r"(v[16]), "=r"(v[17]), "=r"(v[18]), "=r"(v[19]), "=r"(v[20]), "=r"(v[21]), "=r"(v[22]), "=r"(v[23]),
        "=r"(v[24]), "=r"(v[25]), "=r"(v[26]), "=r"(v[27]), "=r"(v[28]), "=r"(v[29]), "=r"(v[30]), "=r"(v[31])
      : "r"(taddr));
}
__device__ __forceinline__ void tmem_ld16(uint32_t taddr, uint32_t (&v)[16]) {
  asm volatile(
      "tcgen05.ld.sync.aligned.32x32b.x16.b32 "
      "{%0, %1, %2, %3, %4, %5, %6, %7, %8, %9, %10, %11, %12, %13, %14, %15}, [%16];"
      : "=r"(v[0]), "=r"(v[1]), "=r"(v[2]), "=r"(v[3]), "=r"(v[4]), "=r"(v[5]), "=r"(v[6]), "=r"(v[7]),
        "=r"(v[8]), "=r"(v[9]), "=r"(v[10]), "=r"(v[11]), "=r"(v[12]), "=r"(v[13]), "=r"(v[14]), "=r"(v[15])
      : "r"(taddr));
}

__device__ __forceinline__ void epi_bar_sync() {
  asm volatile("bar.sync 1, %0;" ::"n"(32 * TC_EPI_WARPS) : "memory");
}

template <int N>
__device__ __forceinline__ uint32_t pick_word(const uint32_t (&a)[N], int i) {
  uint32_t r = a[0];
#pragma unroll
  for (int k = 1; k < N; ++k) r = (i == k) ? a[k] : r;
  return r;
}

template <int BN>
__device__ __forceinline__ void tc_epilogue(const StageDev& st, int mtile, int n0, int phase, int split, int warp,
                                            int lane, uint32_t tmem_acc, uint32_t full_bar, uint32_t parity,
                                            bool have_acc, int sk_mode = 0, int sk_self = 0, int sk_first = 0,
                                            int sk_stride = 2) {
  using Cfg = TcCfg<BN>;
  const int quarter = warp & 3;
  const int half = (warp - 2) >> 2;
  const int r = quarter * 32 + lane;
  const RowCtx rc = tile_row(st, mtile, r);
  constexpr int SPAN = Cfg::SPAN;
  constexpr int CH = SPAN >= 32 ? 32 : 16;
  const int c_begin = half * SPAN;
  const bool active = c_begin < BN;
  const int col0 = n0 + c_begin;
  const int epi = st.epi;
  const bool ok = active && rc.valid && col0 < st.n_pad;
  const int lo_off = st.oC;
  const float leak = st.leak;
  const bool out16 = st.out_fp16 != 0;
  uint16_t* o16 = nullptr;
  float* o32 = nullptr;
  const float* bias = nullptr;
  constexpr int NW = (SPAN + 31) / 32;
  uint32_t mb[NW];
  uint32_t* obits = nullptr;
  if (ok) {
    if (epi == EPI_ACT_HL) {
      const int pos = col0 / st.oC, cb = col0 % st.oC;
      const int mo = rc.m * st.ms + st.ph[phase].mo, no = rc.n * st.ms + st.ph[phase].no;
      const size_t off = (size_t)rc.b * st.sB + (size_t)mo * st.sH + (size_t)no * st.sW + (size_t)pos * st.sPos;
      o16 = (uint16_t*)st.out + off + cb;
      obits = act_bits_word(st, off, cb);
      bias = st.bias + cb;
    } else if (epi == EPI_GRAD_HL) {
      size_t off;
      if (st.split)
        off = (size_t)((rc.m & 1) * 2 + (rc.n & 1)) * st.sP + (size_t)rc.b * st.sB + (size_t)(rc.m >> 1) * st.sH +
              (size_t)(rc.n >> 1) * st.sW;
      else
        off = (size_t)rc.b * st.sB + (size_t)rc.m * st.sH + (size_t)rc.n * st.sW;
      o16 = (uint16_t*)st.out + off + col0;
      const uint32_t* mp = grad_bits_row(st, rc) + (col0 >> 5);
#pragma unroll
      for (int j = 0; j < NW; ++j) mb[j] = __ldg(mp + j);
    } else {
      const size_t row = ((size_t)rc.b * st.Hg + rc.m) * st.Wg + rc.n;
      o32 = (float*)st.out + ((size_t)split * st.rows_total + row) * st.n_pad + col0;
    }
  }
  const float descale = st.descale ? __ldg(st.descale) : 1.f;
  if (have_acc) mbar_wait(full_bar, parity);
  asm volatile("tcgen05.fence::after_thread_sync;" ::: "memory");
  if (!active) return;
  const int ewarp = warp - 2;
  if (sk_mode == 1) {
    float* slot = st.sk_slots + ((size_t)sk_self * 256 + c_begin) * BLOCK_M + r;
#pragma unroll 1
    for (int cc = 0; cc < SPAN; cc += CH) {
      uint32_t v[CH];
      const uint32_t taddr = tmem_acc + ((uint32_t)(quarter * 32) << 16) + (uint32_t)(c_begin + cc);
      if constexpr (CH == 32) tmem_ld32(taddr, v); else tmem_ld16(taddr, v);
      asm volatile("tcgen05.wait::ld.sync.aligned;" ::: "memory");
#pragma unroll
      for (int j = 0; j < CH; ++j) slot[(size_t)(cc + j) * BLOCK_M] = __uint_as_float(v[j]);
    }
    __threadfence();
    __syncwarp();
    if (lane == 0) {
      volatile int32_t* flag = st.sk_flags + sk_self * TC_EPI_WARPS + ewarp;
      asm volatile("st.release.gpu.global.s32 [%0], %1;" ::"l"(flag), "r"(1) : "memory");
    }
    return;
  }
  if (sk_mode == 2) {
    if (lane == 0) {
      for (int h = sk_first; h < sk_self; h += sk_stride) {
        const int32_t* flag = st.sk_flags + h * TC_EPI_WARPS + ewarp;
        int32_t f;
        do {
          asm volatile("ld.acquire.gpu.global.s32 %0, [%1];" : "=r"(f) : "l"(flag) : "memory");
        } while (f == 0);
      }
    }
    __syncwarp();
    __threadfence();
  }
#pragma unroll 1
  for (int cc = 0; cc < SPAN; cc += CH) {
    uint32_t v[CH];
    const uint32_t taddr = tmem_acc + ((uint32_t)(quarter * 32) << 16) + (uint32_t)(c_begin + cc);
    if constexpr (CH == 32) tmem_ld32(taddr, v); else tmem_ld16(taddr, v);
    asm volatile("tcgen05.wait::ld.sync.aligned;" ::: "memory");
    const uint32_t mword = pick_word(mb, cc >> 5);
    if (sk_mode == 2) {
      for (int h = sk_first; h < sk_self; h += sk_stride) {
        const float* slot = st.sk_slots + ((size_t)h * 256 + c_begin + cc) * BLOCK_M + r;
#pragma unroll
        for (int j = 0; j < CH; ++j)
          v[j] = __float_as_uint(__uint_as_float(v[j]) + __ldcg(slot + (size_t)j * BLOCK_M));
      }
    }
    if (!ok) continue;
    uint32_t signs = 0u;
#pragma unroll
    for (int j = 0; j < CH; j += 8) {
      float f[8];
#pragma unroll
      for (int q = 0; q < 8; ++q) f[q] = have_acc ? __uint_as_float(v[j + q]) * descale : 0.f;
      if (epi == EPI_ACT_HL) {
        const float4 b0 = __ldg(reinterpret_cast<const float4*>(bias + cc + j));
        const float4 b1 = __ldg(reinterpret_cast<const float4*>(bias + cc + j + 4));
        const float bb[8] = {b0.x, b0.y, b0.z, b0.w, b1.x, b1.y, b1.z, b1.w};
        __align__(16) uint16_t hi[8], lo[8];
#pragma unroll
        for (int q = 0; q < 8; ++q) {
          float t = f[q] + bb[q];
          t = t > 0.f ? t : t * leak;
          split16(t, out16, hi[q], lo[q]);
          signs |= (uint32_t)(hi[q] >> 15) << ((j + q) & 31);
        }
        *reinterpret_cast<uint4*>(o16 + cc + j) = *reinterpret_cast<uint4*>(hi);
        *reinterpret_cast<uint4*>(o16 + lo_off + cc + j) = *reinterpret_cast<uint4*>(lo);
      } else if (epi == EPI_GRAD_HL) {
        const uint32_t mw = mword >> ((cc + j) & 31);
        __align__(16) uint16_t hi[8], lo[8];
#pragma unroll
        for (int q = 0; q < 8; ++q) {
          const float t = ((mw >> q) & 1u) ? f[q] * leak : f[q];
          split16(t, out16, hi[q], lo[q]);
        }
        *reinterpret_cast<uint4*>(o16 + cc + j) = *reinterpret_cast<uint4*>(hi);
        if (!st.out_single) *reinterpret_cast<uint4*>(o16 + lo_off + cc + j) = *reinterpret_cast<uint4*>(lo);
      } else {
        *reinterpret_cast<float4*>(o32 + cc + j) = make_float4(f[0], f[1], f[2], f[3]);
        *reinterpret_cast<float4*>(o32 + cc + j + 4) = make_float4(f[4], f[5], f[6], f[7]);
      }
    }
    if constexpr (CH == 32) {
      if (epi == EPI_ACT_HL) obits[cc >> 5] = signs;
    }
  }
  if (sk_mode == 2) {
    __syncwarp();
    if (lane == 0)
      for (int h = sk_first; h < sk_self; h += sk_stride) st.sk_flags[h * TC_EPI_WARPS + ewarp] = 0;
  }
}

template <int BN, bool SINGLE>
__device__ __forceinline__ void tc_epilogue_tma(const StageDev& st, const CUtensorMap* tmO, uint32_t stage_smem,
                                                int mtile, int n0, int phase, int warp, int lane, uint32_t tmem_acc,
                                                uint32_t full_bar, uint32_t parity, int sk_mode, int sk_self,
                                                int sk_first);

template <int BN>
__global__ void __launch_bounds__(TC_THREADS, 2)
tapgemm_tc_kernel(const __grid_constant__ CUtensorMap tmA, const __grid_constant__ CUtensorMap tmB,
                  const __grid_constant__ CUtensorMap tmO, const __grid_constant__ StageDev st) {
  using Cfg = TcCfg<BN>;
  extern __shared__ uint8_t smem_raw[];
  const uint32_t tiles = (smem_u32(smem_raw) + 1023u) & ~1023u;
  const bool three = st.passes != 1;
  const uint32_t nst = (uint32_t)st.nst;
  const uint32_t a_bytes = three ? 2 * A_TILE_BYTES : A_TILE_BYTES;
  const uint32_t stage_bytes = a_bytes + (three ? 2 : 1) * Cfg::B_TILE_BYTES;
  const uint32_t bars = tiles + nst * stage_bytes;
  auto full_bar = [&](int s) { return bars + 8u * s; };
  auto empty_bar = [&](int s) { return bars + 8u * (TC_MAX_STAGES + s); };
  const uint32_t tmem_full_bar = bars + 8u * (2 * TC_MAX_STAGES);
  const uint32_t tmem_slot = bars + 8u * (2 * TC_MAX_STAGES + 1);
  uint8_t* gen_base = smem_raw + (tiles - smem_u32(smem_raw));
  volatile uint32_t* tmem_slot_ptr =
      reinterpret_cast<volatile uint32_t*>(gen_base + nst * stage_bytes + 8 * (2 * TC_MAX_STAGES + 1));

  const int warp = threadIdx.x >> 5, lane = threadIdx.x & 31;
  const int mtile = blockIdx.x, n0 = blockIdx.y * BN;
  const int zphase = blockIdx.z / st.ksplit, split = blockIdx.z % st.ksplit;
  const bool wg = st.wgrad != 0;
  const int phase = wg ? 0 : zphase, tap0 = wg ? zphase : 0;
  const int kblocks = st.Ka / BLOCK_K;
  const int total = (wg ? 1 : st.ph[phase].ntaps) * kblocks;
  const int it0 = split * st.it_per_split, it1 = min(total, it0 + st.it_per_split);

  if (warp == 0 && lane == 0) {
    asm volatile("prefetch.tensormap [%0];" ::"l"(&tmA) : "memory");
    asm volatile("prefetch.tensormap [%0];" ::"l"(&tmB) : "memory");
    if (Cfg::TMA_EPI && st.out_tma) asm volatile("prefetch.tensormap [%0];" ::"l"(&tmO) : "memory");
    for (int s = 0; s < TC_MAX_STAGES; ++s) {
      mbar_init(full_bar(s), 1);
      mbar_init(empty_bar(s), 1);
    }
    mbar_init(tmem_full_bar, 1);
    asm volatile("fence.mbarrier_init.release.cluster;" ::: "memory");
  }
  if (warp == 1) {
    asm volatile("tcgen05.alloc.cta_group::1.sync.aligned.shared::cta.b32 [%0], %1;" ::"r"(tmem_slot),
                 "r"((uint32_t)Cfg::TMEM_COLS)
                 : "memory");
    asm volatile("tcgen05.relinquish_alloc_permit.cta_group::1.sync.aligned;" ::: "memory");
  }
  asm volatile("tcgen05.fence::before_thread_sync;" ::: "memory");
  __syncthreads();
  asm volatile("tcgen05.fence::after_thread_sync;" ::: "memory");
  const uint32_t tmem_base = *tmem_slot_ptr;
  pdl_wait();
  pdl_trigger();

  if (warp == 0) {
    {
      int b0, h0, w0;
      tile_origin(st, mtile, b0, h0, w0);
      uint32_t s = 0, par = 0, sa = tiles;
      int tp = it0 / kblocks, kc = (it0 - tp * kblocks) * BLOCK_K;
      tp += tap0;
      int dy = 0, dx = 0, plane = 0, brow = 0, bcol = 0;
      if (it1 > it0) get_tap(st, phase, tp, dy, dx, plane, brow, bcol);
      for (int it = it0; it < it1; ++it) {
        mbar_wait(empty_bar(s), par ^ 1u);
        const uint32_t sb = sa + a_bytes;
        if (elect_one()) {
          mbar_expect_tx(full_bar(s), stage_bytes);
          tma_load_5d(sa, &tmA, full_bar(s), kc, w0 + dx, h0 + dy, b0, plane);
          if (three) tma_load_5d(sa + A_TILE_BYTES, &tmA, full_bar(s), st.Ka + kc, w0 + dx, h0 + dy, b0, plane);
          tma_load_2d(sb, &tmB, full_bar(s), bcol + kc, brow + n0);
          if (three) tma_load_2d(sb + Cfg::B_TILE_BYTES, &tmB, full_bar(s), st.b_k + bcol + kc, brow + n0);
        }
        kc += BLOCK_K;
        if (kc == st.Ka) {
          kc = 0; ++tp;
          if (it + 1 < it1) get_tap(st, phase, tp, dy, dx, plane, brow, bcol);
        }
        sa += stage_bytes;
        if (++s == nst) { s = 0; par ^= 1u; sa = tiles; }
      }
    }
  } else if (warp == 1) {
    {
      const uint32_t idesc = umma_idesc<BN>(st.fp16 != 0);
      uint32_t s = 0, par = 0, sa = tiles;
      for (int it = it0; it < it1; ++it) {
        mbar_wait(full_bar(s), par);
        asm volatile("tcgen05.fence::after_thread_sync;" ::: "memory");
        const uint64_t da = umma_desc(sa), db = umma_desc(sa + a_bytes);
        if (elect_one()) {
#pragma unroll
          for (int k = 0; k < BLOCK_K / 16; ++k) {
            const uint64_t a_hi = da + 2 * k, a_lo = a_hi + (A_TILE_BYTES >> 4);
            const uint64_t b_hi = db + 2 * k, b_lo = b_hi + (Cfg::B_TILE_BYTES >> 4);
            if (three) {
#if LSNF_EXP_FWD2PASS
              if (st.fp16) {
                if (LSNF_EXP_FWD2PASS == 1) umma_bf16(tmem_base, a_lo, b_hi, idesc, (it > it0 || k > 0) ? 1u : 0u);
                else umma_bf16(tmem_base, a_hi, b_lo, idesc, (it > it0 || k > 0) ? 1u : 0u);
                umma_bf16(tmem_base, a_hi, b_hi, idesc, 1u);
                continue;
              }
#endif
              umma_bf16(tmem_base, a_lo, b_hi, idesc, (it > it0 || k > 0) ? 1u : 0u);
              umma_bf16(tmem_base, a_hi, b_lo, idesc, 1u);
              umma_bf16(tmem_base, a_hi, b_hi, idesc, 1u);
            } else {
              umma_bf16(tmem_base, a_hi, b_hi, idesc, (it > it0 || k > 0) ? 1u : 0u);
            }
          }
          umma_commit(empty_bar(s));
        }
        sa += stage_bytes;
        if (++s == nst) { s = 0; par ^= 1u; sa = tiles; }
      }
      if (elect_one()) umma_commit(tmem_full_bar);
    }
  } else {
    bool done = false;
    if constexpr (Cfg::TMA_EPI) {
      if (st.out_tma) {
        if (st.out_single)
          tc_epilogue_tma<BN, true>(st, &tmO, tiles, mtile, n0, phase, warp, lane, tmem_base, tmem_full_bar, 0u, 0, 0, 0);
        else
          tc_epilogue_tma<BN, false>(st, &tmO, tiles, mtile, n0, phase, warp, lane, tmem_base, tmem_full_bar, 0u, 0, 0, 0);
        if (warp == 2 && lane == 0) asm volatile("cp.async.bulk.wait_group 0;" ::: "memory");
        done = true;
      }
    }
    if (!done) tc_epilogue<BN>(st, mtile, n0, phase, wg ? (int)blockIdx.z : split, warp, lane, tmem_base, tmem_full_bar,
                               0u, it1 > it0);
  }
  asm volatile("tcgen05.fence::before_thread_sync;" ::: "memory");
  __syncthreads();
  if (warp == 1) {
    asm volatile("tcgen05.dealloc.cta_group::1.sync.aligned.b32 %0, %1;" ::"r"(tmem_base),
                 "r"((uint32_t)Cfg::TMEM_COLS)
                 : "memory");
  }
}

constexpr int P_BN = 256;
constexpr int P_B_TILE_BYTES = (P_BN / 2) * BLOCK_K * 2;
constexpr int P_STAGE_BYTES = 2 * A_TILE_BYTES + 2 * P_B_TILE_BYTES;
constexpr int P_STAGES = 3;
constexpr int P_MAX_STAGES = 2 * P_STAGES;
constexpr int P_EPI_STAGING = 2 * BLOCK_M * 128;
constexpr int P_SMEM_BYTES = P_STAGES * P_STAGE_BYTES + P_EPI_STAGING + 1024 + 256;
constexpr uint32_t PEER_BIT_MASK = 0xFEFFFFFFu;

__device__ __forceinline__ void tma2_load_5d(uint32_t dst, const CUtensorMap* map, uint32_t bar, int c0, int c1, int c2,
                                             int c3, int c4) {
  asm volatile(
      "cp.async.bulk.tensor.5d.cta_group::2.shared::cluster.global.mbarrier::complete_tx::bytes.L2::cache_hint [%0], [%1, {%3, %4, %5, %6, %7}], [%2], %8;"
      ::"r"(dst), "l"(map), "r"(bar), "r"(c0), "r"(c1), "r"(c2), "r"(c3), "r"(c4), "l"(L2_EVICT_LAST)
      : "memory");
}
__device__ __forceinline__ void tma2_load_2d(uint32_t dst, const CUtensorMap* map, uint32_t bar, int c0, int c1) {
  asm volatile(
      "cp.async.bulk.tensor.2d.cta_group::2.shared::cluster.global.mbarrier::complete_tx::bytes.L2::cache_hint [%0], [%1, {%3, %4}], [%2], %5;"
      ::"r"(dst), "l"(map), "r"(bar), "r"(c0), "r"(c1), "l"(L2_EVICT_LAST)
      : "memory");
}
__device__ __forceinline__ void umma2_bf16(uint32_t tmem_d, uint64_t da, uint64_t db, uint32_t idesc, uint32_t accum) {
  asm volatile(
      "{\n"
      ".reg .pred p;\n"
      "setp.ne.b32 p, %4, 0;\n"
      "tcgen05.mma.cta_group::2.kind::f16 [%0], %1, %2, %3, p;\n"
      "}\n" ::"r"(tmem_d), "l"(da), "l"(db), "r"(idesc), "r"(accum)
      : "memory");
}
__device__ __forceinline__ void umma2_commit_both(uint32_t bar) {
  asm volatile(
      "tcgen05.commit.cta_group::2.mbarrier::arrive::one.shared::cluster.multicast::cluster.b64 [%0], %1;" ::"r"(bar),
      "h"((uint16_t)3)
      : "memory");
}
__device__ __forceinline__ void cluster_sync_all() {
  asm volatile("barrier.cluster.arrive.release.aligned;" ::: "memory");
  asm volatile("barrier.cluster.wait.acquire.aligned;" ::: "memory");
}

__device__ __forceinline__ void cluster_sync_relaxed() {
  asm volatile("barrier.cluster.arrive.relaxed.aligned;" ::: "memory");
  asm volatile("barrier.cluster.wait.aligned;" ::: "memory");
}
__device__ __forceinline__ void mbar_arrive_leader(uint32_t bar) {
  asm volatile("mbarrier.arrive.release.cluster.shared::cluster.b64 _, [%0];" ::"r"(bar & PEER_BIT_MASK) : "memory");
}

__device__ __forceinline__ void tma_store_5d(const CUtensorMap* map, uint32_t src, int c0, int c1, int c2, int c3,
                                             int c4) {
  asm volatile(
      "cp.async.bulk.tensor.5d.global.shared::cta.bulk_group.L2::cache_hint [%0, {%2, %3, %4, %5, %6}], [%1], %7;" ::"l"(map),
      "r"(src), "r"(c0), "r"(c1), "r"(c2), "r"(c3), "r"(c4), "l"(L2_EVICT_FIRST)
      : "memory");
}

__device__ __forceinline__ uint32_t pack2_16(float a, float b, bool fp16) {
  if (fp16) { const __half2 h = __floats2half2_rn(a, b); return *reinterpret_cast<const uint32_t*>(&h); }
  const __nv_bfloat162 h = __floats2bfloat162_rn(a, b);
  return *reinterpret_cast<const uint32_t*>(&h);
}

template <int BN, bool SINGLE>
__device__ __forceinline__ void tc_epilogue_tma(const StageDev& st, const CUtensorMap* tmO, uint32_t stage_smem,
                                                int mtile, int n0, int phase, int warp, int lane, uint32_t tmem_acc,
                                                uint32_t full_bar, uint32_t parity, int sk_mode, int sk_self,
                                                int sk_first) {
  const int quarter = warp & 3;
  const int half = (warp - 2) >> 2;
  const int ewarp = warp - 2;
  const int r = quarter * 32 + lane;
  const RowCtx rc = tile_row(st, mtile, r);
  const int epi = st.epi;
  const float leak = st.leak;
  const bool out16 = st.out_fp16 != 0;
  constexpr int NCH = BN / 64;
  uint32_t mb[NCH];
  uint32_t* obits = nullptr;
#pragma unroll
  for (int ch = 0; ch < NCH; ++ch) mb[ch] = 0u;
  if (epi == EPI_GRAD_HL && rc.valid) {
    const uint32_t* mrow = grad_bits_row(st, rc) + (n0 >> 5) + half;
#pragma unroll
    for (int ch = 0; ch < NCH; ++ch) mb[ch] = __ldg(mrow + 2 * ch);
  } else if (epi == EPI_ACT_HL && rc.valid) {
    const int pos = n0 / st.oC;
    const int mo = rc.m * st.ms + st.ph[phase].mo, no = rc.n * st.ms + st.ph[phase].no;
    const size_t off = (size_t)rc.b * st.sB + (size_t)mo * st.sH + (size_t)no * st.sW + (size_t)pos * st.sPos;
    obits = act_bits_word(st, off, n0 % st.oC) + half;
  }
  int b0, h0, w0;
  tile_origin(st, mtile, b0, h0, w0);
  const int cb = n0 % st.oC;
  int c1, c2, c3, c4;
  if (st.out_tma == 1) { c1 = st.ph[phase].no; c2 = w0; c3 = st.ph[phase].mo; c4 = b0 * st.Hg + h0; }
  else if (st.out_tma == 2) { c1 = n0 / st.oC; c2 = 0; c3 = 0; c4 = b0; }
  else if (st.out_tma == 3) { c1 = w0; c2 = h0; c3 = b0; c4 = 0; }
  else { c1 = w0 >> 1; c2 = b0 * (st.Hg >> 1) + (h0 >> 1); c3 = 0; c4 = 0; }
  int srow = r;
  if (st.out_tma == 4) {
    const int nl = r % st.bW, ml = (r / st.bW) % st.bH, bl = r / (st.bW * st.bH);
    srow = (((ml & 1) * 2 + (nl & 1)) * (st.bB * (st.bH >> 1)) + bl * (st.bH >> 1) + (ml >> 1)) * (st.bW >> 1) + (nl >> 1);
  }
  const float* bias = (epi == EPI_ACT_HL) ? st.bias + cb + half * 32 : nullptr;
  const float descale = st.descale ? __ldg(st.descale) : 1.f;
  const uint32_t buf0 = stage_smem, buf1 = stage_smem + 128 * 128;

  mbar_wait(full_bar, parity);
  asm volatile("tcgen05.fence::after_thread_sync;" ::: "memory");
  if (sk_mode == 2) {
    if (lane == 0) {
      for (int h = sk_first; h < sk_self; h += 2) {
        const int32_t* flag = st.sk_flags + h * TC_EPI_WARPS + ewarp;
        int32_t f;
        do {
          asm volatile("ld.acquire.gpu.global.s32 %0, [%1];" : "=r"(f) : "l"(flag) : "memory");
        } while (f == 0);
      }
    }
    __syncwarp();
    __threadfence();
  }
#pragma unroll 1
  for (int ch = 0; ch < NCH; ++ch) {
    const int col = ch * 64 + half * 32;
    uint32_t v[32];
    tmem_ld32(tmem_acc + ((uint32_t)(quarter * 32) << 16) + (uint32_t)col, v);
    asm volatile("tcgen05.wait::ld.sync.aligned;" ::: "memory");
    if (sk_mode == 2) {
      for (int h = sk_first; h < sk_self; h += 2) {
        const float* slot = st.sk_slots + ((size_t)h * 256 + col) * BLOCK_M + r;
#pragma unroll
        for (int j = 0; j < 32; ++j)
          v[j] = __float_as_uint(__uint_as_float(v[j]) + __ldcg(slot + (size_t)j * BLOCK_M));
      }
    }
    const uint32_t hi_buf = SINGLE ? ((ch & 1) ? buf1 : buf0) : buf0;
    const uint32_t lo_buf = buf1;
    if (SINGLE && warp == 2 && lane == 0) asm volatile("cp.async.bulk.wait_group.read 1;" ::: "memory");
    epi_bar_sync();
    uint32_t signs = 0u;
#pragma unroll
    for (int j = 0; j < 32; j += 8) {
      float t[8];
      if (epi == EPI_ACT_HL) {
        const float4 q0 = __ldg(reinterpret_cast<const float4*>(bias + ch * 64 + j));
        const float4 q1 = __ldg(reinterpret_cast<const float4*>(bias + ch * 64 + j + 4));
        const float bb[8] = {q0.x, q0.y, q0.z, q0.w, q1.x, q1.y, q1.z, q1.w};
#pragma unroll
        for (int q = 0; q < 8; ++q) {
          const float a = __uint_as_float(v[j + q]) * descale + bb[q];
          t[q] = a > 0.f ? a : a * leak;
          signs |= (__float_as_uint(t[q]) >> 31) << (j + q);
        }
      } else {
        const uint32_t mw = pick_word(mb, ch) >> j;
#pragma unroll
        for (int q = 0; q < 8; ++q) {
          const float a = __uint_as_float(v[j + q]) * descale;
          t[q] = ((mw >> q) & 1u) ? a * leak : a;
        }
      }
      const uint32_t chunk = (uint32_t)(half * 4 + j / 8) ^ (uint32_t)(srow & 7);
      const uint32_t off = (uint32_t)srow * 128u + chunk * 16u;
      if constexpr (SINGLE) {
        asm volatile("st.shared.v4.b32 [%0], {%1, %2, %3, %4};" ::"r"(hi_buf + off), "r"(pack2_16(t[0], t[1], out16)),
                     "r"(pack2_16(t[2], t[3], out16)), "r"(pack2_16(t[4], t[5], out16)),
                     "r"(pack2_16(t[6], t[7], out16))
                     : "memory");
      } else {
        __align__(16) uint16_t hi[8], lo[8];
#pragma unroll
        for (int q = 0; q < 8; ++q) split16(t[q], out16, hi[q], lo[q]);
        asm volatile("st.shared.v4.b32 [%0], {%1, %2, %3, %4};" ::"r"(hi_buf + off), "r"(((uint32_t*)hi)[0]),
                     "r"(((uint32_t*)hi)[1]), "r"(((uint32_t*)hi)[2]), "r"(((uint32_t*)hi)[3])
                     : "memory");
        if (!st.out_single)
          asm volatile("st.shared.v4.b32 [%0], {%1, %2, %3, %4};" ::"r"(lo_buf + off), "r"(((uint32_t*)lo)[0]),
                       "r"(((uint32_t*)lo)[1]), "r"(((uint32_t*)lo)[2]), "r"(((uint32_t*)lo)[3])
                       : "memory");
      }
    }
    asm volatile("fence.proxy.async.shared::cta;" ::: "memory");
    epi_bar_sync();
    if (warp == 2 && lane == 0) {
      const int c0 = cb + ch * 64;
      tma_store_5d(tmO, hi_buf, c0, c1, c2, c3, c4);
      if (!SINGLE && !st.out_single) tma_store_5d(tmO, lo_buf, c0 + st.oC, c1, c2, c3, c4);
      asm volatile("cp.async.bulk.commit_group;" ::: "memory");
      if (!SINGLE) asm volatile("cp.async.bulk.wait_group.read 0;" ::: "memory");
    }
    if (obits) obits[2 * ch] = signs;
  }
  if (sk_mode == 2) {
    __syncwarp();
    if (lane == 0)
      for (int h = sk_first; h < sk_self; h += 2) st.sk_flags[h * TC_EPI_WARPS + ewarp] = 0;
  }
}

struct SkItem { int tile, ka, kb, mode; };
struct SkPlan {
  int total, t_lo, t_hi, ka_lo, kb_hi, first_fin, last_help, first_help_only, n_items, full_lo, full_hi;
  long long u0, u1;
  int strided, pair_, npairs_;
  __device__ __forceinline__ void init(int pair, int num_pairs, int num_tiles, int total_, bool stream_k) {
    total = total_;
    strided = !stream_k; pair_ = pair; npairs_ = num_pairs;
    if (strided) {
      n_items = pair < num_tiles ? (num_tiles - pair + num_pairs - 1) / num_pairs : 0;
      first_fin = last_help = first_help_only = 0;
      return;
    }
    const long long U = (long long)num_tiles * total;
    u0 = U * pair / num_pairs; u1 = U * (pair + 1) / num_pairs;
    n_items = 0; first_fin = last_help = first_help_only = 0; full_lo = 0; full_hi = -1;
    if (u1 <= u0) return;
    t_lo = (int)(u0 / total); t_hi = (int)((u1 - 1) / total);
    ka_lo = (int)(u0 - (long long)t_lo * total);
    kb_hi = (int)(u1 - (long long)t_hi * total);
    const bool first_cut = ka_lo != 0, last_cut = kb_hi != total;
    if (t_lo == t_hi) {
      if (last_cut) { last_help = 1; }
      else if (first_cut) { first_fin = 1; }
      else { full_lo = full_hi = t_lo; }
    } else {
      last_help = last_cut; first_fin = first_cut;
      full_lo = first_cut ? t_lo + 1 : t_lo;
      full_hi = last_cut ? t_hi - 1 : t_hi;
    }
    n_items = last_help + (full_hi >= full_lo ? full_hi - full_lo + 1 : 0) + first_fin;
  }
  __device__ __forceinline__ SkItem item(int j) const {
    SkItem it;
    if (strided) { it.tile = pair_ + j * npairs_; it.ka = 0; it.kb = total; it.mode = 0; return it; }
    if (last_help) {
      if (j == 0) { it.tile = t_hi; it.ka = (t_lo == t_hi) ? ka_lo : 0; it.kb = kb_hi; it.mode = 1; return it; }
      --j;
    }
    const int nfull = full_hi >= full_lo ? full_hi - full_lo + 1 : 0;
    if (j < nfull) { it.tile = full_lo + j; it.ka = 0; it.kb = total; it.mode = 0; return it; }
    it.tile = t_lo; it.ka = ka_lo; it.kb = total; it.mode = 2;
    return it;
  }
};

__device__ __forceinline__ int sk_pair_of(long long u, long long U, int P) {
  int p = (int)((u * P) / U);
  while (p > 0 && U * p / P > u) --p;
  while (p + 1 < P && U * (p + 1) / P <= u) ++p;
  return p;
}

template <bool DEEP>
__global__ void __cluster_dims__(2, 1, 1) __launch_bounds__(TC_THREADS, 1)
tapgemm_tc2_kernel(const __grid_constant__ CUtensorMap tmA, const __grid_constant__ CUtensorMap tmB,
                   const __grid_constant__ CUtensorMap tmO, const __grid_constant__ StageDev st) {
  extern __shared__ uint8_t smem_raw[];
  const uint32_t tiles = (smem_u32(smem_raw) + 1023u) & ~1023u;
  const uint32_t stage_smem = tiles + P_STAGES * P_STAGE_BYTES;
  const uint32_t bars = stage_smem + P_EPI_STAGING;
  auto full_bar = [&](int s) { return bars + 8u * s; };
  auto empty_bar = [&](int s) { return bars + 8u * (P_MAX_STAGES + s); };
  auto tmem_full_bar = [&](int a) { return bars + 8u * (2 * P_MAX_STAGES + a); };
  auto tmem_empty_bar = [&](int a) { return bars + 8u * (2 * P_MAX_STAGES + 2 + a); };
  const uint32_t tmem_slot = bars + 8u * (2 * P_MAX_STAGES + 4);
  uint8_t* gen_base = smem_raw + (tiles - smem_u32(smem_raw));
  volatile uint32_t* tmem_slot_ptr = reinterpret_cast<volatile uint32_t*>(
      gen_base + P_STAGES * P_STAGE_BYTES + P_EPI_STAGING + 8 * (2 * P_MAX_STAGES + 4));
  constexpr bool three = !DEEP;
  constexpr uint32_t nst = DEEP ? P_MAX_STAGES : P_STAGES;
  constexpr uint32_t stage_bytes = DEEP ? P_STAGE_BYTES / 2 : P_STAGE_BYTES;
  constexpr uint32_t b_off = DEEP ? A_TILE_BYTES : 2 * A_TILE_BYTES;

  uint32_t cta_rank;
  asm volatile("mov.u32 %0, %%cluster_ctarank;" : "=r"(cta_rank));
  const bool leader = cta_rank == 0;
  const int warp = threadIdx.x >> 5, lane = threadIdx.x & 31;
  const int kblocks = st.Ka / BLOCK_K;
  const int mtiles = st.tiles_b * st.tiles_h * st.tiles_w;
  const int m_pairs = (mtiles + 1) >> 1, n_tiles = st.n_pad / P_BN;
  const int num_tiles = m_pairs * n_tiles * st.nphase;
  const int pair_id = blockIdx.x >> 1, num_pairs = gridDim.x >> 1;
  const int total = st.ph[0].ntaps * kblocks;
  SkPlan sk;
  sk.init(pair_id, num_pairs, num_tiles, total, st.sk_enable != 0);

  if (warp == 0 && lane == 0) {
    asm volatile("prefetch.tensormap [%0];" ::"l"(&tmA) : "memory");
    asm volatile("prefetch.tensormap [%0];" ::"l"(&tmB) : "memory");
    if (st.out_tma) asm volatile("prefetch.tensormap [%0];" ::"l"(&tmO) : "memory");
    for (int s = 0; s < P_MAX_STAGES; ++s) {
      mbar_init(full_bar(s), 1);
      mbar_init(empty_bar(s), 1);
    }
    for (int a = 0; a < 2; ++a) {
      mbar_init(tmem_full_bar(a), 1);
      mbar_init(tmem_empty_bar(a), 2 * TC_EPI_WARPS);
    }
    asm volatile("fence.mbarrier_init.release.cluster;" ::: "memory");
  }
  if (warp == 1) {
    asm volatile("tcgen05.alloc.cta_group::2.sync.aligned.shared::cta.b32 [%0], %1;" ::"r"(tmem_slot), "r"(512u)
                 : "memory");
    asm volatile("tcgen05.relinquish_alloc_permit.cta_group::2.sync.aligned;" ::: "memory");
  }
  asm volatile("tcgen05.fence::before_thread_sync;" ::: "memory");
  __syncthreads();
  cluster_sync_all();
  asm volatile("tcgen05.fence::after_thread_sync;" ::: "memory");
  const uint32_t tmem_base = *tmem_slot_ptr;
  pdl_wait();
  pdl_trigger();

  if (warp == 0) {
    {
      uint32_t s = 0, par = 0, sa = tiles;
      constexpr uint32_t tx_bytes = three ? 2 * P_STAGE_BYTES : P_STAGE_BYTES;
      for (int j = 0; j < sk.n_items; ++j) {
        const SkItem w = sk.item(j);
        const int t = w.tile;
        const int mp = t % m_pairs, nt = (t / m_pairs) % n_tiles, phase = t / (m_pairs * n_tiles);
        const int mtile = 2 * mp + (int)cta_rank;
        int b0, h0, w0;
        tile_origin(st, mtile, b0, h0, w0);
        const int nb = nt * P_BN + (int)cta_rank * (P_BN / 2);
        int tp = w.ka / kblocks, kc = (w.ka - tp * kblocks) * BLOCK_K;
        int dy, dx, plane, brow, bcol;
        get_tap(st, phase, tp, dy, dx, plane, brow, bcol);
        for (int it = w.ka; it < w.kb; ++it) {
          mbar_wait(empty_bar(s), par ^ 1u);
          const uint32_t sb = sa + b_off;
          const uint32_t fb = full_bar(s) & PEER_BIT_MASK;
          if (elect_one()) {
            if (leader) mbar_expect_tx(full_bar(s), tx_bytes);
            tma2_load_5d(sa, &tmA, fb, kc, w0 + dx, h0 + dy, b0, plane);
            if (three) tma2_load_5d(sa + A_TILE_BYTES, &tmA, fb, st.Ka + kc, w0 + dx, h0 + dy, b0, plane);
            tma2_load_2d(sb, &tmB, fb, bcol + kc, brow + nb);
            if (three) tma2_load_2d(sb + P_B_TILE_BYTES, &tmB, fb, st.b_k + bcol + kc, brow + nb);
          }
          kc += BLOCK_K;
          if (kc == st.Ka) {
            kc = 0; ++tp;
            if (it + 1 < w.kb) get_tap(st, phase, tp, dy, dx, plane, brow, bcol);
          }
          sa += stage_bytes;
          if (++s == nst) { s = 0; par ^= 1u; sa = tiles; }
        }
      }
    }
  } else if (warp == 1) {
    if (leader) {
      const uint32_t fmt = st.fp16 ? 0u : 1u;
      const uint32_t idesc = (1u << 4) | (fmt << 7) | (fmt << 10) | ((uint32_t)(P_BN >> 3) << 17) | ((uint32_t)(256 >> 4) << 24);
      uint32_t s = 0, par = 0, sa = tiles;
      for (int j = 0; j < sk.n_items; ++j) {
        const SkItem w = sk.item(j);
        const uint32_t acc = (uint32_t)j & 1u;
        mbar_wait(tmem_empty_bar(acc), (((uint32_t)j >> 1) & 1u) ^ 1u);
        asm volatile("tcgen05.fence::after_thread_sync;" ::: "memory");
        const uint32_t d_tmem = tmem_base + acc * P_BN;
        for (int it = w.ka; it < w.kb; ++it) {
          mbar_wait(full_bar(s), par);
          asm volatile("tcgen05.fence::after_thread_sync;" ::: "memory");
          const uint64_t da = umma_desc(sa), db = umma_desc(sa + b_off);
          if (elect_one()) {
#pragma unroll
            for (int k = 0; k < BLOCK_K / 16; ++k) {
              const uint64_t a_hi = da + 2 * k, a_lo = a_hi + (A_TILE_BYTES >> 4);
              const uint64_t b_hi = db + 2 * k, b_lo = b_hi + (P_B_TILE_BYTES >> 4);
              if (three) {
#if LSNF_EXP_FWD2PASS
                if (st.fp16) {
                  if (LSNF_EXP_FWD2PASS == 1) umma2_bf16(d_tmem, a_lo, b_hi, idesc, (it > w.ka || k > 0) ? 1u : 0u);
                  else umma2_bf16(d_tmem, a_hi, b_lo, idesc, (it > w.ka || k > 0) ? 1u : 0u);
                  umma2_bf16(d_tmem, a_hi, b_hi, idesc, 1u);
                  continue;
                }
#endif
                umma2_bf16(d_tmem, a_lo, b_hi, idesc, (it > w.ka || k > 0) ? 1u : 0u);
                umma2_bf16(d_tmem, a_hi, b_lo, idesc, 1u);
                umma2_bf16(d_tmem, a_hi, b_hi, idesc, 1u);
              } else {
                umma2_bf16(d_tmem, a_hi, b_hi, idesc, (it > w.ka || k > 0) ? 1u : 0u);
              }
            }
            umma2_commit_both(empty_bar(s));
          }
          sa += stage_bytes;
          if (++s == nst) { s = 0; par ^= 1u; sa = tiles; }
        }
        if (elect_one()) umma2_commit_both(tmem_full_bar(acc));
      }
    }
  } else {
    const long long U = (long long)num_tiles * total;
    for (int j = 0; j < sk.n_items; ++j) {
      const SkItem w = sk.item(j);
      const int t = w.tile;
      const int mp = t % m_pairs, nt = (t / m_pairs) % n_tiles, phase = t / (m_pairs * n_tiles);
      const int mtile = 2 * mp + (int)cta_rank;
      const uint32_t acc = (uint32_t)j & 1u;
      const int self = 2 * pair_id + (int)cta_rank;
      int first = self;
      if (w.mode == 2) first = 2 * sk_pair_of((long long)t * total, U, num_pairs) + (int)cta_rank;
      if (st.out_tma && w.mode != 1) {
        if (st.out_single)
          tc_epilogue_tma<P_BN, true>(st, &tmO, stage_smem, mtile, nt * P_BN, phase, warp, lane,
                                      tmem_base + acc * P_BN, tmem_full_bar(acc), ((uint32_t)j >> 1) & 1u, w.mode,
                                      self, first);
        else
          tc_epilogue_tma<P_BN, false>(st, &tmO, stage_smem, mtile, nt * P_BN, phase, warp, lane,
                                       tmem_base + acc * P_BN, tmem_full_bar(acc), ((uint32_t)j >> 1) & 1u, w.mode,
                                       self, first);
      } else
        tc_epilogue<P_BN>(st, mtile, nt * P_BN, phase, 0, warp, lane, tmem_base + acc * P_BN, tmem_full_bar(acc),
                          ((uint32_t)j >> 1) & 1u, true, w.mode, self, first, 2);
      asm volatile("tcgen05.fence::before_thread_sync;" ::: "memory");
      __syncwarp();
      if (lane == 0) mbar_arrive_leader(tmem_empty_bar(acc));
    }
    if (st.out_tma && warp == 2 && lane == 0) asm volatile("cp.async.bulk.wait_group 0;" ::: "memory");
  }
  asm volatile("tcgen05.fence::before_thread_sync;" ::: "memory");
  __syncthreads();
  cluster_sync_relaxed();
  if (warp == 1) {
    asm volatile("tcgen05.dealloc.cta_group::2.sync.aligned.b32 %0, %1;" ::"r"(tmem_base), "r"(512u) : "memory");
  }
}

typedef CUresult (*EncodeTiledFn)(CUtensorMap*, CUtensorMapDataType, cuuint32_t, void*, const cuuint64_t*,
                                  const cuuint64_t*, const cuuint32_t*, const cuuint32_t*, CUtensorMapInterleave,
                                  CUtensorMapSwizzle, CUtensorMapL2promotion, CUtensorMapFloatOOBfill);

static EncodeTiledFn get_encode() {
  static EncodeTiledFn fn = nullptr;
  if (fn) return fn;
  void* p = nullptr;
  cudaDriverEntryPointQueryResult q;
  if (cudaGetDriverEntryPoint("cuTensorMapEncodeTiled", &p, cudaEnableDefault, &q) != cudaSuccess ||
      q != cudaDriverEntryPointSuccess)
    return nullptr;
  fn = (EncodeTiledFn)p;
  return fn;
}

static bool pair_enabled() {
  static int v = -1;
  if (v < 0) { const char* e = getenv("LSNF_NO_PAIR"); v = (e && e[0] == '1') ? 0 : 1; }
  return v == 1;
}
static bool use_pair(const StageHost& sh) {
  const StageDev& d = sh.dev;
  const int mtiles = d.tiles_b * d.tiles_h * d.tiles_w;
  const int total = d.ph[0].ntaps * (d.Ka / BLOCK_K);
  return pair_enabled() && !d.wgrad && d.block_n == 256 && d.n_pad % 256 == 0 && d.ksplit == 1 && total >= 3 &&
         (mtiles >= 2 || total >= 8);
}

bool tc_stage_is_pair(const StageHost& sh) { return use_pair(sh); }

struct RingGeom { int nst; size_t stage_bytes, smem; };
static RingGeom ring_geometry(const StageDev& d) {
  const bool three = d.passes != 1;
  const size_t stage = (size_t)(three ? 2 : 1) * (A_TILE_BYTES + (size_t)d.block_n * BLOCK_K * 2);
  const int total = d.ph[0].ntaps * (d.Ka / BLOCK_K);
  const int iters = d.ksplit > 1 ? d.it_per_split : total;
  const size_t budget = (iters <= 4 ? TC_SMEM_MAX / 2 : TC_SMEM_MAX) - TC_SMEM_EXTRA;
  int nst = (int)std::min<size_t>(budget / stage, (size_t)std::min(iters, TC_MAX_STAGES));
  nst = std::max(nst, 1);
  while (d.out_tma && nst * stage < 32768) ++nst;
  size_t smem = nst * stage + TC_SMEM_EXTRA;
  const int tmem_cols = d.block_n < 32 ? 32 : d.block_n;
  const int tmem_ctas = 512 / tmem_cols;
  smem = std::max(smem, (size_t)TC_SMEM_MAX / (tmem_ctas + 1) + 16);
  return {nst, stage, smem};
}

static bool tma_store_enabled() {
  static int v = -1;
  if (v < 0) { const char* e = getenv("LSNF_NO_TMA_STORE"); v = (e && e[0] == '1') ? 0 : 1; }
  return v == 1;
}

static int out_tma_kind(const StageHost& sh) {
  const StageDev& d = sh.dev;
  const bool wide_single = d.block_n >= 128 && d.n_pad % d.block_n == 0 && d.ksplit == 1;
  if (!(use_pair(sh) || wide_single) || !(d.epi == EPI_ACT_HL || d.epi == EPI_GRAD_HL) || !tma_store_enabled()) return 0;
  if (d.epi == EPI_ACT_HL && sh.first) return 2;
  if (d.epi == EPI_ACT_HL && d.ms == 2) return 1;
  if (d.epi == EPI_GRAD_HL && !d.split) return 3;
  if (d.epi == EPI_GRAD_HL && d.split && d.bW >= 2 && d.bH >= 2 && (d.bH % 2) == 0) return 4;
  return 0;
}

int tc_encode_maps(lsnf_plan* plan, StageHost& sh) {
  EncodeTiledFn enc = get_encode();
  if (!enc) { set_error("cuTensorMapEncodeTiled entry point not available"); return LSNF_ERR_CUDA; }
  const StageDev& d = sh.dev;
  {
    const cuuint64_t row = (cuuint64_t)2 * d.Ka * 2;
    cuuint64_t dims[5] = {(cuuint64_t)2 * d.Ka, (cuuint64_t)d.aW, (cuuint64_t)d.aH, (cuuint64_t)d.B, (cuuint64_t)d.aP};
    cuuint64_t strides[4] = {row, row * d.aW, row * d.aW * d.aH, row * d.aW * d.aH * d.B};
    cuuint32_t box[5] = {BLOCK_K, (cuuint32_t)d.bW, (cuuint32_t)d.bH, (cuuint32_t)d.bB, 1};
    cuuint32_t es[5] = {1, 1, 1, 1, 1};
    CUresult r = enc(&sh.tmA, CU_TENSOR_MAP_DATA_TYPE_BFLOAT16, 5, (void*)d.a, dims, strides, box, es,
                     CU_TENSOR_MAP_INTERLEAVE_NONE, CU_TENSOR_MAP_SWIZZLE_128B, CU_TENSOR_MAP_L2_PROMOTION_L2_128B,
                     CU_TENSOR_MAP_FLOAT_OOB_FILL_NONE);
    if (r != CUDA_SUCCESS) {
      set_error("cuTensorMapEncodeTiled(A) failed with code " + std::to_string((int)r) + " for stage layer " +
                std::to_string(sh.layer) + " kind " + std::to_string(sh.kind));
      return LSNF_ERR_CUDA;
    }
  }
  {
    cuuint64_t dims[2] = {(cuuint64_t)2 * d.b_k, (cuuint64_t)d.b_rows};
    cuuint64_t strides[1] = {(cuuint64_t)2 * d.b_k * 2};
    const bool pair = use_pair(sh);
    cuuint32_t box[2] = {BLOCK_K, (cuuint32_t)(pair ? d.block_n / 2 : d.block_n)};
    cuuint32_t es[2] = {1, 1};
    CUresult r = enc(&sh.tmB, CU_TENSOR_MAP_DATA_TYPE_BFLOAT16, 2, (void*)d.b, dims, strides, box, es,
                     CU_TENSOR_MAP_INTERLEAVE_NONE, CU_TENSOR_MAP_SWIZZLE_128B, CU_TENSOR_MAP_L2_PROMOTION_L2_256B,
                     CU_TENSOR_MAP_FLOAT_OOB_FILL_NONE);
    if (r != CUDA_SUCCESS) {
      set_error("cuTensorMapEncodeTiled(B) failed with code " + std::to_string((int)r) + " for stage layer " +
                std::to_string(sh.layer) + " kind " + std::to_string(sh.kind));
      return LSNF_ERR_CUDA;
    }
  }
  sh.dev.out_tma = 0;
  const int want_kind = out_tma_kind(sh);
  if (want_kind) {
    const cuuint64_t C2 = (cuuint64_t)2 * d.oC, eb = 2;
    cuuint64_t dims[5], strides[4];
    cuuint32_t box[5], es[5] = {1, 1, 1, 1, 1};
    int kind = 0;
    if (want_kind == 2) {
      const cuuint64_t kk = (cuuint64_t)sh.k * sh.k;
      dims[0] = C2; dims[1] = kk; dims[2] = 1; dims[3] = 1; dims[4] = d.B;
      strides[0] = C2 * eb; strides[1] = C2 * kk * eb; strides[2] = C2 * kk * eb; strides[3] = C2 * kk * eb;
      box[0] = 64; box[1] = 1; box[2] = 1; box[3] = 1; box[4] = 128;
      kind = 2;
    } else if (want_kind == 1) {
      const cuuint64_t W = d.Wg, H = d.Hg;
      dims[0] = C2; dims[1] = 2; dims[2] = W; dims[3] = 2; dims[4] = (cuuint64_t)d.B * H;
      strides[0] = C2 * eb; strides[1] = 2 * C2 * eb; strides[2] = 2 * W * C2 * eb; strides[3] = 4 * W * C2 * eb;
      box[0] = 64; box[1] = 1; box[2] = d.bW; box[3] = 1; box[4] = d.bB * d.bH;
      kind = 1;
    } else if (want_kind == 3) {
      const cuuint64_t W = d.Wg, H = d.Hg;
      dims[0] = C2; dims[1] = W; dims[2] = H; dims[3] = d.B; dims[4] = 1;
      strides[0] = C2 * eb; strides[1] = W * C2 * eb; strides[2] = H * W * C2 * eb; strides[3] = (cuuint64_t)d.B * H * W * C2 * eb;
      box[0] = 64; box[1] = d.bW; box[2] = d.bH; box[3] = d.bB; box[4] = 1;
      kind = 3;
    } else if (want_kind == 4) {
      const cuuint64_t Wh = d.Wg / 2, Hh = d.Hg / 2;
      const cuuint64_t plane = (cuuint64_t)d.B * Hh * Wh * C2;
      dims[0] = C2; dims[1] = Wh; dims[2] = (cuuint64_t)d.B * Hh; dims[3] = 2; dims[4] = 2;
      strides[0] = C2 * eb; strides[1] = Wh * C2 * eb; strides[2] = plane * eb; strides[3] = 2 * plane * eb;
      box[0] = 64; box[1] = d.bW / 2; box[2] = d.bB * d.bH / 2; box[3] = 2; box[4] = 2;
      kind = 4;
    }
    if (kind) {
      CUresult r = enc(&sh.tmO, CU_TENSOR_MAP_DATA_TYPE_BFLOAT16, 5, d.out, dims, strides, box, es,
                       CU_TENSOR_MAP_INTERLEAVE_NONE, CU_TENSOR_MAP_SWIZZLE_128B, CU_TENSOR_MAP_L2_PROMOTION_NONE,
                       CU_TENSOR_MAP_FLOAT_OOB_FILL_NONE);
      if (r != CUDA_SUCCESS) {
        set_error("cuTensorMapEncodeTiled(out) failed with code " + std::to_string((int)r) + " for stage layer " +
                  std::to_string(sh.layer) + " kind " + std::to_string(sh.kind));
        return LSNF_ERR_CUDA;
      }
      sh.dev.out_tma = kind;
    }
  }
  if (!sh.dev.out_tma) sh.tmO = sh.tmA;
  sh.maps_ready = true;
  return LSNF_OK;
}

template <int BN>
static int launch_bn(const StageHost& sh, cudaStream_t s) {
  StageDev st = sh.dev;
  const RingGeom g = ring_geometry(st);
  st.nst = g.nst;
  dim3 grid(st.tiles_b * st.tiles_h * st.tiles_w, st.n_pad / BN, (st.wgrad ? st.ph[0].ntaps : st.nphase) * st.ksplit);
  LSNF_CUDA(launch_k(tapgemm_tc_kernel<BN>, grid, dim3(TC_THREADS), g.smem, s, sh.tmA, sh.tmB, sh.tmO, st));
  return LSNF_OK;
}

static bool pair_stream_k(const StageDev& st, int max_pairs) {
  const int mtiles = st.tiles_b * st.tiles_h * st.tiles_w;
  const int num_tiles = (mtiles + 1) / 2 * (st.n_pad / P_BN) * st.nphase;
  const int total = st.ph[0].ntaps * (st.Ka / BLOCK_K);
  const int rounds = (num_tiles + max_pairs - 1) / max_pairs;
  const long long static_units = (long long)rounds * total;
  const long long sk_units = ((long long)num_tiles * total + max_pairs - 1) / max_pairs + 35;
  static int sk_env = -1;
  if (sk_env < 0) { const char* e = getenv("LSNF_STREAMK"); sk_env = e ? atoi(e) : 2; }
  return (sk_env == 1 || (sk_env == 2 && sk_units < static_units)) && total >= 8 &&
         (long long)num_tiles * total >= 4LL * max_pairs && max_pairs <= 80;
}

static int launch_pair(const StageHost& sh, cudaStream_t s) {
  const StageDev& st = sh.dev;
  const int mtiles = st.tiles_b * st.tiles_h * st.tiles_w;
  const int num_tiles = (mtiles + 1) / 2 * (st.n_pad / P_BN) * st.nphase;
  const int max_pairs = sh.num_sms / 2;
  StageDev launch_st = st;
  launch_st.sk_enable = pair_stream_k(st, max_pairs);
  const int pairs = launch_st.sk_enable ? max_pairs : std::min(num_tiles, max_pairs);
  dim3 grid(2 * pairs, 1, 1);
  if (st.passes == 1)
    LSNF_CUDA(launch_k(tapgemm_tc2_kernel<true>, grid, dim3(TC_THREADS), P_SMEM_BYTES, s, sh.tmA, sh.tmB, sh.tmO, launch_st));
  else
    LSNF_CUDA(launch_k(tapgemm_tc2_kernel<false>, grid, dim3(TC_THREADS), P_SMEM_BYTES, s, sh.tmA, sh.tmB, sh.tmO, launch_st));
  return LSNF_OK;
}

void tc_launch_info(const StageHost& sh_in, int num_sms, lsnf_launch_info* out) {
  StageHost sh = sh_in;
  sh.dev.out_tma = out_tma_kind(sh);
  const StageDev& d = sh.dev;
  const int mtiles = d.tiles_b * d.tiles_h * d.tiles_w;
  memset(out, 0, sizeof(*out));
  out->block = TC_THREADS;
  out->tma_store = d.out_tma;
  out->tmem_columns = use_pair(sh) ? 512 : (d.block_n < 32 ? 32 : d.block_n);
  if (use_pair(sh)) {
    const int max_pairs = num_sms / 2;
    const int num_tiles = (mtiles + 1) / 2 * (d.n_pad / P_BN) * d.nphase;
    out->kernel = LSNF_KERNEL_PAIR;
    out->stream_k = pair_stream_k(d, max_pairs) ? 1 : 0;
    out->grid_x = 2 * (out->stream_k ? max_pairs : std::min(num_tiles, max_pairs));
    out->grid_y = out->grid_z = 1;
    out->ring_stages = d.passes == 1 ? P_MAX_STAGES : P_STAGES;
    out->stage_bytes = d.passes == 1 ? P_STAGE_BYTES / 2 : P_STAGE_BYTES;
    out->smem_bytes = P_SMEM_BYTES;
    out->ctas_per_sm = 1;
  } else {
    const RingGeom g = ring_geometry(d);
    out->kernel = LSNF_KERNEL_SINGLE;
    out->grid_x = mtiles; out->grid_y = d.n_pad / d.block_n; out->grid_z = d.nphase * d.ksplit;
    out->ring_stages = g.nst;
    out->stage_bytes = (int32_t)g.stage_bytes;
    out->smem_bytes = (int32_t)g.smem;
    const int by_smem = (TC_SMEM_MAX + 1024) / ((int)g.smem + 1024);
    out->ctas_per_sm = std::max(1, std::min(by_smem, 2048 / TC_THREADS));
  }
}

int tc_prepare_device(int device) {
  static std::mutex mu;
  static bool done[64] = {false};
  std::lock_guard<std::mutex> lock(mu);
  if (device < 0 || device >= 64) { set_error("device index out of range"); return LSNF_ERR_INVALID; }
  if (done[device]) return LSNF_OK;
  LSNF_CUDA(cudaFuncSetAttribute(tapgemm_tc_kernel<256>, cudaFuncAttributeMaxDynamicSharedMemorySize, TC_SMEM_MAX));
  LSNF_CUDA(cudaFuncSetAttribute(tapgemm_tc_kernel<128>, cudaFuncAttributeMaxDynamicSharedMemorySize, TC_SMEM_MAX));
  LSNF_CUDA(cudaFuncSetAttribute(tapgemm_tc_kernel<64>, cudaFuncAttributeMaxDynamicSharedMemorySize, TC_SMEM_MAX));
  LSNF_CUDA(cudaFuncSetAttribute(tapgemm_tc_kernel<32>, cudaFuncAttributeMaxDynamicSharedMemorySize, TC_SMEM_MAX));
  LSNF_CUDA(cudaFuncSetAttribute(tapgemm_tc_kernel<16>, cudaFuncAttributeMaxDynamicSharedMemorySize, TC_SMEM_MAX));
  LSNF_CUDA(cudaFuncSetAttribute(tapgemm_tc2_kernel<false>, cudaFuncAttributeMaxDynamicSharedMemorySize, P_SMEM_BYTES));
  LSNF_CUDA(cudaFuncSetAttribute(tapgemm_tc2_kernel<true>, cudaFuncAttributeMaxDynamicSharedMemorySize, P_SMEM_BYTES));
  done[device] = true;
  return LSNF_OK;
}

int launch_tapgemm_tc(const StageHost& sh, cudaStream_t s) {
  if (!sh.maps_ready) { set_error("tensor maps not encoded"); return LSNF_ERR_STATE; }
  if (use_pair(sh)) return launch_pair(sh, s);
  switch (sh.dev.block_n) {
    case 256: return launch_bn<256>(sh, s);
    case 128: return launch_bn<128>(sh, s);
    case 64: return launch_bn<64>(sh, s);
    case 32: return launch_bn<32>(sh, s);
    case 16: return launch_bn<16>(sh, s);
    default: set_error("unsupported N tile"); return LSNF_ERR_INVALID;
  }
}

}
```

Baseline: 92550.

## Chain consecutive pair-GEMM stages into one persistent launch with per-sample readiness flags

Fuses two consecutive cluster-pair tap-GEMM stages (forward or dgrad) into a single persistent kernel. A host-side simulation builds a static work order that interleaves producer and consumer tiles. Consumer tiles wait on per-sample counters that producer epilogues publish with release atomics. This removes a launch and the inter-kernel tail/ramp bubble, at the cost of spin-waiting, extra grid-constant tensor maps, counter reset logic, and a dependence on the simulated schedule being accurate.

New measurement: 94260 (median of 6 runs). 1.9% higher.

```diff
diff --git a/include/lsnf.h b/include/lsnf.h
--- a/include/lsnf.h
+++ b/include/lsnf.h
@@ -98,6 +98,9 @@
                    const float* grad_scale, lsnf_stream stream);
 
 int lsnf_plan_run_stage(lsnf_plan* plan, int32_t index, lsnf_stream stream);
+int lsnf_plan_run_chain(lsnf_plan* plan, int32_t first_stage, int32_t max_pairs, lsnf_stream stream);
+int lsnf_plan_chain_order(const lsnf_plan* plan, int32_t first_stage, int32_t num_sms, int32_t* order,
+                          int32_t capacity, int32_t* n_items, int32_t* target);
 int lsnf_langevin_launch_count(const lsnf_plan* plan, int32_t steps);
 
 #define LSNF_MAX_TAPS 16
diff --git a/latent-space-normalizing-flow_b200/_cabi.py b/latent-space-normalizing-flow_b200/_cabi.py
--- a/latent-space-normalizing-flow_b200/_cabi.py
+++ b/latent-space-normalizing-flow_b200/_cabi.py
@@ -83,6 +83,9 @@
                                  C.POINTER(C.c_int32), C.c_float, C.c_float, C.c_float, C.c_float, C.c_float,
                                  C.c_int64, C.c_void_p, C.c_void_p]),
     "lsnf_plan_run_stage": (C.c_int, [C.c_void_p, C.c_int32, C.c_void_p]),
+    "lsnf_plan_run_chain": (C.c_int, [C.c_void_p, C.c_int32, C.c_int32, C.c_void_p]),
+    "lsnf_plan_chain_order": (C.c_int, [C.c_void_p, C.c_int32, C.c_int32, C.POINTER(C.c_int32), C.c_int32,
+                                        C.POINTER(C.c_int32), C.POINTER(C.c_int32)]),
     "lsnf_langevin_launch_count": (C.c_int, [C.c_void_p, C.c_int32]),
     "lsnf_plan_num_stages": (C.c_int, [C.c_void_p]),
     "lsnf_plan_stage_info": (C.c_int, [C.c_void_p, C.c_int32, C.POINTER(StageInfo)]),
diff --git a/latent-space-normalizing-flow_b200/csrc/lsnf_internal.cuh b/latent-space-normalizing-flow_b200/csrc/lsnf_internal.cuh
--- a/latent-space-normalizing-flow_b200/csrc/lsnf_internal.cuh
+++ b/latent-space-normalizing-flow_b200/csrc/lsnf_internal.cuh
@@ -60,6 +60,12 @@
   int32_t wgrad;
   int32_t out_tma, nst;
   PhaseDev ph[LSNF_MAX_PHASES];
+};
+
+struct ChainDev {
+  const int32_t* order;
+  int32_t* ctl;
+  int32_t n_items, target, on, pad_;
 };
 
 struct StageHost {
@@ -166,10 +172,13 @@
   int num_sms = 148;
   cudaStream_t side = nullptr;
   cudaEvent_t ev_fork = nullptr, ev_join = nullptr;
-  struct LoopGraph { int steps; float step_size, sigma; int with_noise; cudaGraphExec_t exec; };
+  struct LoopGraph { int steps; float step_size, sigma; int with_noise, chain; cudaGraphExec_t exec; };
   std::vector<LoopGraph> graphs;
   cudaStream_t cap_stream = nullptr;
   size_t off_x = 0, off_gnorms = 0, off_dyn = 0, off_sk_slots = 0, off_sk_flags = 0;
+  struct Chain { int first, n_items; int32_t target; size_t off_order; };
+  std::vector<Chain> chains;
+  size_t off_chain_ctl = 0;
   long long runs = 0;
   bool use_graphs = true;
   int graph_chunk = 40;
@@ -229,6 +238,9 @@
 int tc_encode_maps(lsnf_plan* plan, StageHost& st);
 void tc_launch_info(const StageHost& st, int num_sms, lsnf_launch_info* out);
 bool tc_stage_is_pair(const StageHost& st);
+bool tc_chain_ok(const StageHost& a, const StageHost& b);
+void tc_chain_order(const StageDev& a, const StageDev& b, int num_sms, std::vector<int32_t>* order, int32_t* target);
+int launch_tapgemm_tc_chain(const StageHost& a, const StageHost& b, const ChainDev& ch, int max_pairs, cudaStream_t s);
 int launch_pack_stage(const lsnf_plan* plan, const StageHost& st, const float* w, cudaStream_t s);
 int launch_split_z(const lsnf_plan* plan, const float* z, cudaStream_t s);
 int launch_weight_scales(const lsnf_plan* plan, const float* const* weights, cudaStream_t s);
diff --git a/latent-space-normalizing-flow_b200/csrc/plan.cu b/latent-space-normalizing-flow_b200/csrc/plan.cu
--- a/latent-space-normalizing-flow_b200/csrc/plan.cu
+++ b/latent-space-normalizing-flow_b200/csrc/plan.cu
@@ -520,8 +520,41 @@
     }
     p->gen_grad_floats = goff;
   }
+  if (L > 0 && c.gemm_impl == LSNF_GEMM_TCGEN05) {
+    for (int i = 0; i + 1 < 2 * L; ++i) {
+      if (i + 1 == L || !tc_chain_ok(p->stages[i], p->stages[i + 1])) continue;
+      std::vector<int32_t> order;
+      int32_t target = 0;
+      tc_chain_order(p->stages[i].dev, p->stages[i + 1].dev, 148, &order, &target);
+      p->chains.push_back({i, (int)order.size(), target, take(order.size() * 4)});
+      ++i;
+    }
+    if (!p->chains.empty()) p->off_chain_ctl = take((size_t)(2 + B) * 4);
+  }
   p->ws_bytes = off;
   *out = p;
+  return LSNF_OK;
+}
+
+static const lsnf_plan::Chain* chain_at(const lsnf_plan* p, int first) {
+  for (const auto& ch : p->chains)
+    if (ch.first == first) return &ch;
+  return nullptr;
+}
+
+extern "C" int lsnf_plan_chain_order(const lsnf_plan* plan, int32_t first_stage, int32_t num_sms, int32_t* order,
+                                     int32_t capacity, int32_t* n_items, int32_t* target) {
+  if (!plan || !n_items || !target) return fail(LSNF_ERR_INVALID, "null argument");
+  if (num_sms < 2) return fail(LSNF_ERR_INVALID, "num_sms must be at least 2");
+  const lsnf_plan::Chain* ch = chain_at(plan, first_stage);
+  if (!ch) return fail(LSNF_ERR_INVALID, "stage " + std::to_string(first_stage) + " does not start a chained launch");
+  std::vector<int32_t> o;
+  tc_chain_order(plan->stages[first_stage].dev, plan->stages[first_stage + 1].dev, num_sms, &o, target);
+  *n_items = (int32_t)o.size();
+  if (order) {
+    if (capacity < (int32_t)o.size()) return fail(LSNF_ERR_INVALID, "order buffer too small");
+    std::copy(o.begin(), o.end(), order);
+  }
   return LSNF_OK;
 }
 
@@ -621,6 +654,17 @@
     w.fin.part = (const float*)(plan->ws + w.off_part);
     w.rs.src = (const uint16_t*)(plan->ws + w.off_gT);
   }
+  if (!plan->chains.empty()) {
+    LSNF_CUDA(cudaDeviceSynchronize());
+    for (const auto& ch : plan->chains) {
+      std::vector<int32_t> order;
+      int32_t target = 0;
+      tc_chain_order(plan->stages[ch.first].dev, plan->stages[ch.first + 1].dev, plan->num_sms, &order, &target);
+      LSNF_CUDA(cudaMemcpy(plan->ws + ch.off_order, order.data(), order.size() * 4, cudaMemcpyHostToDevice));
+    }
+    LSNF_CUDA(cudaMemset(plan->ws + plan->off_chain_ctl, 0, (size_t)(2 + plan->cfg.batch) * 4));
+    LSNF_CUDA(cudaDeviceSynchronize());
+  }
   if (!plan->side) {
     LSNF_CUDA(cudaStreamCreateWithFlags(&plan->side, cudaStreamNonBlocking));
     LSNF_CUDA(cudaEventCreateWithFlags(&plan->ev_fork, cudaEventDisableTiming));
@@ -698,11 +742,12 @@
   return LSNF_OK;
 }
 
+static int run_forward_stages(const lsnf_plan* p, cudaStream_t s);
+
 static int gen_forward(lsnf_plan* p, const float* z, float* x_hat, cudaStream_t s, bool split) {
   int rc;
   if (split && (rc = launch_split_z(p, z, s))) return rc;
-  for (int l = 0; l < p->n_layers; ++l)
-    if ((rc = run_stage(p, p->stages[l], s))) return rc;
+  if ((rc = run_forward_stages(p, s))) return rc;
   if ((rc = launch_last_gather(p, nullptr, 0, s))) return rc;
   if (x_hat) {
     const size_t bytes = (size_t)p->cfg.batch * p->cfg.nc * p->img * p->img * 4;
@@ -724,6 +769,39 @@
   if (rc) return rc;
   if (index < 0 || index >= (int)plan->stages.size()) return fail(LSNF_ERR_INVALID, "bad stage index");
   return run_stage(plan, plan->stages[index], (cudaStream_t)stream);
+}
+
+static int run_chain(const lsnf_plan* p, const lsnf_plan::Chain& ch, int max_pairs, cudaStream_t s) {
+  ChainDev d = {};
+  d.order = (const int32_t*)(p->ws + ch.off_order);
+  d.ctl = (int32_t*)(p->ws + p->off_chain_ctl);
+  d.n_items = ch.n_items; d.target = ch.target; d.on = 1;
+  return launch_tapgemm_tc_chain(p->stages[ch.first], p->stages[ch.first + 1], d, max_pairs, s);
+}
+
+static bool chain_enabled() {
+  const char* e = getenv("LSNF_CHAIN");
+  return !(e && e[0] == '0');
+}
+
+static int run_forward_stages(const lsnf_plan* p, cudaStream_t s) {
+  const bool chain = chain_enabled();
+  int rc;
+  for (int l = 0; l < p->n_layers; ++l) {
+    const lsnf_plan::Chain* ch = chain ? chain_at(p, l) : nullptr;
+    if ((rc = ch ? run_chain(p, *ch, 0, s) : run_stage(p, p->stages[l], s))) return rc;
+    if (ch) ++l;
+  }
+  return LSNF_OK;
+}
+
+extern "C" int lsnf_plan_run_chain(lsnf_plan* plan, int32_t first_stage, int32_t max_pairs, lsnf_stream stream) {
+  int rc = need(plan, true, false);
+  if (rc) return rc;
+  const lsnf_plan::Chain* ch = chain_at(plan, first_stage);
+  if (!ch) return fail(LSNF_ERR_INVALID, "stage " + std::to_string(first_stage) + " does not start a chained launch");
+  if (max_pairs < 0) return fail(LSNF_ERR_INVALID, "max_pairs must be >= 0");
+  return run_chain(plan, *ch, max_pairs, (cudaStream_t)stream);
 }
 
 extern "C" int lsnf_generator_forward(lsnf_plan* plan, const float* z, float* x_hat, lsnf_stream stream) {
@@ -922,8 +1000,7 @@
   float* zw = (float*)(plan->ws + plan->off_z);
   if ((rc = launch_flow_inverse(plan, eps, zw, nullptr, s))) return rc;
   if ((rc = launch_split_z(plan, zw, s))) return rc;
-  for (int l = 0; l < plan->n_layers; ++l)
-    if ((rc = run_stage(plan, plan->stages[l], s))) return rc;
+  if ((rc = run_forward_stages(plan, s))) return rc;
   if ((rc = launch_last_gather(plan, x, to_unit_range, s))) return rc;
   if (z) LSNF_CUDA(cudaMemcpyAsync(z, zw, (size_t)plan->cfg.batch * plan->cfg.nz * 4, cudaMemcpyDeviceToDevice, s));
   return LSNF_OK;
@@ -941,7 +1018,8 @@
 extern "C" int lsnf_langevin_launch_count(const lsnf_plan* plan, int32_t steps) {
   if (!plan) return 0;
   const int chunks = steps > 0 ? (steps + plan->graph_chunk - 1) / plan->graph_chunk : 0;
-  return 1 + steps * (2 * plan->n_layers + 3) + chunks;
+  const int chained = chain_enabled() ? (int)plan->chains.size() : 0;
+  return 1 + steps * (2 * plan->n_layers + 3 - chained) + chunks;
 }
 
 struct LoopTrace {
@@ -976,7 +1054,7 @@
 
 static int langevin_loop(lsnf_plan* plan, const float* x, int steps, float step_size, float sigma, int with_noise,
                          const float* eps, uint64_t seed, uint64_t sample_offset, const uint64_t* dyn, float* gnorms,
-                         cudaStream_t s) {
+                         bool chain, cudaStream_t s) {
   const float gscale = sigma_post_scale(sigma);
   int rc;
   static int trace_env = -1;
@@ -1010,11 +1088,14 @@
         if ((rc = launch_flow_forward(plan, z, nullptr, nullptr, nullptr, gf, plan->side))) return rc;
         LSNF_CUDA(cudaEventRecord(plan->ev_join, plan->side));
       }
+      const lsnf_plan::Chain* ch = chain && l + 1 != fork_at ? chain_at(plan, l) : nullptr;
       {
         PdlScope pdl(pdl_ok(tc_path && tc_stage_is_pair(plan->stages[l])));
-        if ((rc = run_stage(plan, plan->stages[l], s))) return rc;
+        if ((rc = ch ? run_chain(plan, *ch, 0, s) : run_stage(plan, plan->stages[l], s))) return rc;
       }
-      tr.mark(("forward layer " + std::to_string(l)).c_str());
+      tr.mark(ch ? ("forward layers " + std::to_string(l) + "+" + std::to_string(l + 1)).c_str()
+                 : ("forward layer " + std::to_string(l)).c_str());
+      if (ch) ++l;
     }
     {
       PdlScope pdl(pdl_ok(false));
@@ -1022,11 +1103,15 @@
     }
     tr.mark("gather + tanh + recon grad + im2col");
     for (int i = plan->n_layers; i < 2 * plan->n_layers; ++i) {
+      const lsnf_plan::Chain* ch = chain ? chain_at(plan, i) : nullptr;
       {
         PdlScope pdl(pdl_ok(tc_path && tc_stage_is_pair(plan->stages[i])));
-        if ((rc = run_stage(plan, plan->stages[i], s))) return rc;
+        if ((rc = ch ? run_chain(plan, *ch, 0, s) : run_stage(plan, plan->stages[i], s))) return rc;
       }
-      tr.mark(("dgrad layer " + std::to_string(plan->stages[i].layer)).c_str());
+      tr.mark(ch ? ("dgrad layers " + std::to_string(plan->stages[i].layer) + "+" +
+                    std::to_string(plan->stages[i + 1].layer)).c_str()
+                 : ("dgrad layer " + std::to_string(plan->stages[i].layer)).c_str());
+      if (ch) ++i;
     }
     LSNF_CUDA(cudaStreamWaitEvent(s, plan->ev_join, 0));
     tr.mark("join flow prior");
@@ -1054,9 +1139,11 @@
   LSNF_CUDA(cudaMemcpyAsync(z, z0, zbytes, cudaMemcpyDeviceToDevice, s));
   if ((rc = launch_split_z(plan, z, s))) return rc;
   const bool graph_ok = plan->use_graphs && !eps && steps > 0 && plan->runs > 0;
+  const bool chain = chain_enabled();
   plan->runs++;
   if (!graph_ok) {
-    if ((rc = langevin_loop(plan, x, steps, step_size, sigma, with_noise, eps, seed, sample_offset, nullptr, gnorms, s)))
+    if ((rc = langevin_loop(plan, x, steps, step_size, sigma, with_noise, eps, seed, sample_offset, nullptr, gnorms,
+                            chain, s)))
       return rc;
   } else {
     float* x_ws = (float*)(plan->ws + plan->off_x);
@@ -1067,12 +1154,14 @@
       const int n = std::min(steps - done, plan->graph_chunk);
       cudaGraphExec_t exec = nullptr;
       for (auto& g : plan->graphs)
-        if (g.steps == n && g.step_size == step_size && g.sigma == sigma && g.with_noise == with_noise) exec = g.exec;
+        if (g.steps == n && g.step_size == step_size && g.sigma == sigma && g.with_noise == with_noise &&
+            g.chain == (int)chain)
+          exec = g.exec;
       if (!exec) {
         cudaGraph_t graph = nullptr;
         cudaStream_t cs = plan->cap_stream;
         LSNF_CUDA(cudaStreamBeginCapture(cs, cudaStreamCaptureModeThreadLocal));
-        rc = langevin_loop(plan, x_ws, n, step_size, sigma, with_noise, nullptr, 0, 0, dyn, gn_ws, cs);
+        rc = langevin_loop(plan, x_ws, n, step_size, sigma, with_noise, nullptr, 0, 0, dyn, gn_ws, chain, cs);
         cudaError_t ce = cudaStreamEndCapture(cs, &graph);
         if (rc) { if (graph) cudaGraphDestroy(graph); return rc; }
         if (ce != cudaSuccess) return cuda_fail(ce, "cudaStreamEndCapture");
@@ -1080,7 +1169,7 @@
         cudaGraphDestroy(graph);
         if (ce != cudaSuccess) return cuda_fail(ce, "cudaGraphInstantiate");
         if (plan->graphs.size() >= 8) { cudaGraphExecDestroy(plan->graphs.front().exec); plan->graphs.erase(plan->graphs.begin()); }
-        plan->graphs.push_back({n, step_size, sigma, with_noise, exec});
+        plan->graphs.push_back({n, step_size, sigma, with_noise, (int)chain, exec});
       }
       if ((rc = launch_set_dyn(plan, seed, sample_offset, (uint32_t)done, s))) return rc;
       LSNF_CUDA(cudaGraphLaunch(exec, s));
diff --git a/latent-space-normalizing-flow_b200/csrc/tapgemm_tc.cu b/latent-space-normalizing-flow_b200/csrc/tapgemm_tc.cu
--- a/latent-space-normalizing-flow_b200/csrc/tapgemm_tc.cu
+++ b/latent-space-normalizing-flow_b200/csrc/tapgemm_tc.cu
@@ -684,10 +684,65 @@
   return p;
 }
 
+constexpr int CHAIN_SLOTS = 8;
+struct PairItem { int stage, tile, ka, kb, mode; };
+
+__device__ __forceinline__ void mbar_wait_cluster(uint32_t bar, uint32_t parity) {
+  asm volatile(
+      "{\n"
+      ".reg .pred P1;\n"
+      "WAIT_LOOP_C:\n"
+      "mbarrier.try_wait.parity.acquire.cluster.shared::cta.b64 P1, [%0], %1;\n"
+      "@P1 bra DONE_C;\n"
+      "bra WAIT_LOOP_C;\n"
+      "DONE_C:\n"
+      "}\n" ::"r"(bar), "r"(parity)
+      : "memory");
+}
+__device__ __forceinline__ uint32_t peer_smem(uint32_t addr, uint32_t rank) {
+  uint32_t r;
+  asm volatile("mapa.shared::cluster.u32 %0, %1, %2;" : "=r"(r) : "r"(addr), "r"(rank));
+  return r;
+}
+__device__ __forceinline__ void tile_samples(const StageDev& s, int mtile, int& b0, int& b1) {
+  int h0, w0;
+  tile_origin(s, mtile, b0, h0, w0);
+  b1 = min(b0 + s.bB, s.B);
+}
+__device__ __forceinline__ void chain_wait_ready(const ChainDev& ch, const StageDev& s, int mtile, int lane) {
+  int b0, b1;
+  tile_samples(s, mtile, b0, b1);
+  for (int b = b0 + lane; b < b1; b += 32) {
+    const int32_t* c = ch.ctl + 2 + b;
+    int32_t v;
+    do {
+      asm volatile("ld.acquire.gpu.global.s32 %0, [%1];" : "=r"(v) : "l"(c) : "memory");
+    } while (v < ch.target);
+  }
+  __syncwarp();
+  asm volatile("fence.proxy.async.global;" ::: "memory");
+}
+__device__ __forceinline__ void chain_publish(const ChainDev& ch, const StageDev& s, int mtile, int warp, int lane) {
+  __threadfence();
+  epi_bar_sync();
+  if (warp != 2) return;
+  if (lane == 0) asm volatile("cp.async.bulk.wait_group 0;" ::: "memory");
+  __syncwarp();
+  asm volatile("fence.proxy.async.global;" ::: "memory");
+  __threadfence();
+  int b0, b1;
+  tile_samples(s, mtile, b0, b1);
+  for (int b = b0 + lane; b < b1; b += 32)
+    asm volatile("red.release.gpu.global.add.s32 [%0], 1;" ::"l"(ch.ctl + 2 + b) : "memory");
+}
+
 template <bool DEEP>
 __global__ void __cluster_dims__(2, 1, 1) __launch_bounds__(TC_THREADS, 1)
 tapgemm_tc2_kernel(const __grid_constant__ CUtensorMap tmA, const __grid_constant__ CUtensorMap tmB,
-                   const __grid_constant__ CUtensorMap tmO, const __grid_constant__ StageDev st) {
+                   const __grid_constant__ CUtensorMap tmO, const __grid_constant__ StageDev st,
+                   const __grid_constant__ CUtensorMap tmA2, const __grid_constant__ CUtensorMap tmB2,
+                   const __grid_constant__ CUtensorMap tmO2, const __grid_constant__ StageDev st2,
+                   const __grid_constant__ ChainDev ch) {
   extern __shared__ uint8_t smem_raw[];
   const uint32_t tiles = (smem_u32(smem_raw) + 1023u) & ~1023u;
   const uint32_t stage_smem = tiles + P_STAGES * P_STAGE_BYTES;
@@ -697,6 +752,8 @@
   auto tmem_full_bar = [&](int a) { return bars + 8u * (2 * P_MAX_STAGES + a); };
   auto tmem_empty_bar = [&](int a) { return bars + 8u * (2 * P_MAX_STAGES + 2 + a); };
   const uint32_t tmem_slot = bars + 8u * (2 * P_MAX_STAGES + 4);
+  auto claim_bar = [&](int k) { return bars + 8u * (2 * P_MAX_STAGES + 5 + k); };
+  auto claim_val = [&](int k) { return bars + 8u * (2 * P_MAX_STAGES + 5 + CHAIN_SLOTS) + 4u * k; };
   uint8_t* gen_base = smem_raw + (tiles - smem_u32(smem_raw));
   volatile uint32_t* tmem_slot_ptr = reinterpret_cast<volatile uint32_t*>(
       gen_base + P_STAGES * P_STAGE_BYTES + P_EPI_STAGING + 8 * (2 * P_MAX_STAGES + 4));
@@ -708,20 +765,58 @@
   uint32_t cta_rank;
   asm volatile("mov.u32 %0, %%cluster_ctarank;" : "=r"(cta_rank));
   const bool leader = cta_rank == 0;
+  const bool chained = ch.on != 0;
   const int warp = threadIdx.x >> 5, lane = threadIdx.x & 31;
-  const int kblocks = st.Ka / BLOCK_K;
-  const int mtiles = st.tiles_b * st.tiles_h * st.tiles_w;
-  const int m_pairs = (mtiles + 1) >> 1, n_tiles = st.n_pad / P_BN;
+  auto m_pairs_of = [](const StageDev& s) { return (s.tiles_b * s.tiles_h * s.tiles_w + 1) >> 1; };
+  auto total_of = [](const StageDev& s) { return s.ph[0].ntaps * (s.Ka / BLOCK_K); };
+  const int m_pairs = m_pairs_of(st), n_tiles = st.n_pad / P_BN;
   const int num_tiles = m_pairs * n_tiles * st.nphase;
   const int pair_id = blockIdx.x >> 1, num_pairs = gridDim.x >> 1;
-  const int total = st.ph[0].ntaps * kblocks;
+  const int total = total_of(st);
   SkPlan sk;
-  sk.init(pair_id, num_pairs, num_tiles, total, st.sk_enable != 0);
+  sk.init(pair_id, num_pairs, num_tiles, total, st.sk_enable != 0 && !chained);
+  auto get_item = [&](int j, PairItem& w) -> bool {
+    if (!chained) {
+      if (j >= sk.n_items) return false;
+      const SkItem s = sk.item(j);
+      w.stage = 0; w.tile = s.tile; w.ka = s.ka; w.kb = s.kb; w.mode = s.mode;
+      return true;
+    }
+    const int k = j % CHAIN_SLOTS;
+    mbar_wait_cluster(claim_bar(k), (uint32_t)(j / CHAIN_SLOTS) & 1u);
+    int32_t v;
+    asm volatile("ld.shared.s32 %0, [%1];" : "=r"(v) : "r"(claim_val(k)) : "memory");
+    if (v < 0) return false;
+    w.stage = v >> 24; w.tile = v & 0xFFFFFF; w.ka = 0; w.kb = total_of(w.stage ? st2 : st); w.mode = 0;
+    return true;
+  };
+  auto claim_publish = [&](int j) {
+    int32_t v = -1;
+    if (lane == 0) {
+      const int c = atomicAdd(ch.ctl, 1);
+      v = c < ch.n_items ? __ldg(ch.order + c) : -1;
+    }
+    v = __shfl_sync(0xffffffffu, v, 0);
+    if (elect_one()) {
+      const int k = j % CHAIN_SLOTS;
+      asm volatile("st.shared.s32 [%0], %1;" ::"r"(claim_val(k)), "r"(v) : "memory");
+      asm volatile("mbarrier.arrive.release.cta.shared::cta.b64 _, [%0];" ::"r"(claim_bar(k)) : "memory");
+      asm volatile("st.shared::cluster.s32 [%0], %1;" ::"r"(peer_smem(claim_val(k), 1)), "r"(v) : "memory");
+      asm volatile("mbarrier.arrive.release.cluster.shared::cluster.b64 _, [%0];" ::"r"(peer_smem(claim_bar(k), 1))
+                   : "memory");
+    }
+    __syncwarp();
+  };
 
   if (warp == 0 && lane == 0) {
     asm volatile("prefetch.tensormap [%0];" ::"l"(&tmA) : "memory");
     asm volatile("prefetch.tensormap [%0];" ::"l"(&tmB) : "memory");
     if (st.out_tma) asm volatile("prefetch.tensormap [%0];" ::"l"(&tmO) : "memory");
+    if (chained) {
+      asm volatile("prefetch.tensormap [%0];" ::"l"(&tmA2) : "memory");
+      asm volatile("prefetch.tensormap [%0];" ::"l"(&tmB2) : "memory");
+      if (st2.out_tma) asm volatile("prefetch.tensormap [%0];" ::"l"(&tmO2) : "memory");
+    }
     for (int s = 0; s < P_MAX_STAGES; ++s) {
       mbar_init(full_bar(s), 1);
       mbar_init(empty_bar(s), 1);
@@ -730,6 +825,7 @@
       mbar_init(tmem_full_bar(a), 1);
       mbar_init(tmem_empty_bar(a), 2 * TC_EPI_WARPS);
     }
+    for (int k = 0; k < CHAIN_SLOTS; ++k) mbar_init(claim_bar(k), 1);
     asm volatile("fence.mbarrier_init.release.cluster;" ::: "memory");
   }
   if (warp == 1) {
@@ -749,36 +845,44 @@
     {
       uint32_t s = 0, par = 0, sa = tiles;
       constexpr uint32_t tx_bytes = three ? 2 * P_STAGE_BYTES : P_STAGE_BYTES;
-      for (int j = 0; j < sk.n_items; ++j) {
-        const SkItem w = sk.item(j);
+      if (chained && leader) claim_publish(0);
+      PairItem w;
+      for (int j = 0; get_item(j, w); ++j) {
+        const StageDev& S = w.stage ? st2 : st;
+        const CUtensorMap* tA = w.stage ? &tmA2 : &tmA;
+        const CUtensorMap* tB = w.stage ? &tmB2 : &tmB;
+        const int Ka = S.Ka, bk = S.b_k, kblocks = Ka / BLOCK_K;
+        const int mps = m_pairs_of(S), nts = S.n_pad / P_BN;
         const int t = w.tile;
-        const int mp = t % m_pairs, nt = (t / m_pairs) % n_tiles, phase = t / (m_pairs * n_tiles);
+        const int mp = t % mps, nt = (t / mps) % nts, phase = t / (mps * nts);
         const int mtile = 2 * mp + (int)cta_rank;
+        if (chained && w.stage == 1) chain_wait_ready(ch, S, mtile, lane);
         int b0, h0, w0;
-        tile_origin(st, mtile, b0, h0, w0);
+        tile_origin(S, mtile, b0, h0, w0);
         const int nb = nt * P_BN + (int)cta_rank * (P_BN / 2);
         int tp = w.ka / kblocks, kc = (w.ka - tp * kblocks) * BLOCK_K;
         int dy, dx, plane, brow, bcol;
-        get_tap(st, phase, tp, dy, dx, plane, brow, bcol);
+        get_tap(S, phase, tp, dy, dx, plane, brow, bcol);
         for (int it = w.ka; it < w.kb; ++it) {
           mbar_wait(empty_bar(s), par ^ 1u);
           const uint32_t sb = sa + b_off;
           const uint32_t fb = full_bar(s) & PEER_BIT_MASK;
           if (elect_one()) {
             if (leader) mbar_expect_tx(full_bar(s), tx_bytes);
-            tma2_load_5d(sa, &tmA, fb, kc, w0 + dx, h0 + dy, b0, plane);
-            if (three) tma2_load_5d(sa + A_TILE_BYTES, &tmA, fb, st.Ka + kc, w0 + dx, h0 + dy, b0, plane);
-            tma2_load_2d(sb, &tmB, fb, bcol + kc, brow + nb);
-            if (three) tma2_load_2d(sb + P_B_TILE_BYTES, &tmB, fb, st.b_k + bcol + kc, brow + nb);
+            tma2_load_5d(sa, tA, fb, kc, w0 + dx, h0 + dy, b0, plane);
+            if (three) tma2_load_5d(sa + A_TILE_BYTES, tA, fb, Ka + kc, w0 + dx, h0 + dy, b0, plane);
+            tma2_load_2d(sb, tB, fb, bcol + kc, brow + nb);
+            if (three) tma2_load_2d(sb + P_B_TILE_BYTES, tB, fb, bk + bcol + kc, brow + nb);
           }
           kc += BLOCK_K;
-          if (kc == st.Ka) {
+          if (kc == Ka) {
             kc = 0; ++tp;
-            if (it + 1 < w.kb) get_tap(st, phase, tp, dy, dx, plane, brow, bcol);
+            if (it + 1 < w.kb) get_tap(S, phase, tp, dy, dx, plane, brow, bcol);
           }
           sa += stage_bytes;
           if (++s == nst) { s = 0; par ^= 1u; sa = tiles; }
         }
+        if (chained && leader) claim_publish(j + 1);
       }
     }
   } else if (warp == 1) {
@@ -786,8 +890,8 @@
       const uint32_t fmt = st.fp16 ? 0u : 1u;
       const uint32_t idesc = (1u << 4) | (fmt << 7) | (fmt << 10) | ((uint32_t)(P_BN >> 3) << 17) | ((uint32_t)(256 >> 4) << 24);
       uint32_t s = 0, par = 0, sa = tiles;
-      for (int j = 0; j < sk.n_items; ++j) {
-        const SkItem w = sk.item(j);
+      PairItem w;
+      for (int j = 0; get_item(j, w); ++j) {
         const uint32_t acc = (uint32_t)j & 1u;
         mbar_wait(tmem_empty_bar(acc), (((uint32_t)j >> 1) & 1u) ^ 1u);
         asm volatile("tcgen05.fence::after_thread_sync;" ::: "memory");
@@ -826,39 +930,53 @@
       }
     }
   } else {
-    const long long U = (long long)num_tiles * total;
-    for (int j = 0; j < sk.n_items; ++j) {
-      const SkItem w = sk.item(j);
+    PairItem w;
+    for (int j = 0; get_item(j, w); ++j) {
+      const StageDev& S = w.stage ? st2 : st;
+      const CUtensorMap* tO = w.stage ? &tmO2 : &tmO;
+      const int mps = m_pairs_of(S), nts = S.n_pad / P_BN;
       const int t = w.tile;
-      const int mp = t % m_pairs, nt = (t / m_pairs) % n_tiles, phase = t / (m_pairs * n_tiles);
+      const int mp = t % mps, nt = (t / mps) % nts, phase = t / (mps * nts);
       const int mtile = 2 * mp + (int)cta_rank;
       const uint32_t acc = (uint32_t)j & 1u;
       const int self = 2 * pair_id + (int)cta_rank;
       int first = self;
-      if (w.mode == 2) first = 2 * sk_pair_of((long long)t * total, U, num_pairs) + (int)cta_rank;
-      if (st.out_tma && w.mode != 1) {
-        if (st.out_single)
-          tc_epilogue_tma<P_BN, true>(st, &tmO, stage_smem, mtile, nt * P_BN, phase, warp, lane,
-                                      tmem_base + acc * P_BN, tmem_full_bar(acc), ((uint32_t)j >> 1) & 1u, w.mode,
-                                      self, first);
+      if (w.mode == 2) first = 2 * sk_pair_of((long long)t * total, (long long)num_tiles * total, num_pairs) + (int)cta_rank;
+      if (S.out_tma && w.mode != 1) {
+        if (S.out_single)
+          tc_epilogue_tma<P_BN, true>(S, tO, stage_smem, mtile, nt * P_BN, phase, warp, lane, tmem_base + acc * P_BN,
+                                      tmem_full_bar(acc), ((uint32_t)j >> 1) & 1u, w.mode, self, first);
         else
-          tc_epilogue_tma<P_BN, false>(st, &tmO, stage_smem, mtile, nt * P_BN, phase, warp, lane,
-                                       tmem_base + acc * P_BN, tmem_full_bar(acc), ((uint32_t)j >> 1) & 1u, w.mode,
-                                       self, first);
+          tc_epilogue_tma<P_BN, false>(S, tO, stage_smem, mtile, nt * P_BN, phase, warp, lane, tmem_base + acc * P_BN,
+                                       tmem_full_bar(acc), ((uint32_t)j >> 1) & 1u, w.mode, self, first);
       } else
-        tc_epilogue<P_BN>(st, mtile, nt * P_BN, phase, 0, warp, lane, tmem_base + acc * P_BN, tmem_full_bar(acc),
+        tc_epilogue<P_BN>(S, mtile, nt * P_BN, phase, 0, warp, lane, tmem_base + acc * P_BN, tmem_full_bar(acc),
                           ((uint32_t)j >> 1) & 1u, true, w.mode, self, first, 2);
       asm volatile("tcgen05.fence::before_thread_sync;" ::: "memory");
       __syncwarp();
       if (lane == 0) mbar_arrive_leader(tmem_empty_bar(acc));
-    }
-    if (st.out_tma && warp == 2 && lane == 0) asm volatile("cp.async.bulk.wait_group 0;" ::: "memory");
+      if (chained && w.stage == 0) chain_publish(ch, S, mtile, warp, lane);
+    }
+    if ((st.out_tma || (chained && st2.out_tma)) && warp == 2 && lane == 0)
+      asm volatile("cp.async.bulk.wait_group 0;" ::: "memory");
   }
   asm volatile("tcgen05.fence::before_thread_sync;" ::: "memory");
   __syncthreads();
-  cluster_sync_relaxed();
+  if (chained) cluster_sync_all(); else cluster_sync_relaxed();
   if (warp == 1) {
     asm volatile("tcgen05.dealloc.cta_group::2.sync.aligned.b32 %0, %1;" ::"r"(tmem_base), "r"(512u) : "memory");
+  }
+  if (chained && leader && warp == 0) {
+    int last = 0;
+    if (lane == 0) {
+      __threadfence();
+      last = atomicAdd(ch.ctl + 1, 1) == num_pairs - 1;
+    }
+    last = __shfl_sync(0xffffffffu, last, 0);
+    if (last) {
+      __threadfence();
+      for (int i = lane; i < 2 + st.B; i += 32) ch.ctl[i] = 0;
+    }
   }
 }
 
@@ -1021,17 +1139,29 @@
   return LSNF_OK;
 }
 
+static void pair_path_units(const StageDev& st, int max_pairs, long long* static_units, long long* sk_units) {
+  const int mtiles = st.tiles_b * st.tiles_h * st.tiles_w;
+  const int num_tiles = (mtiles + 1) / 2 * (st.n_pad / P_BN) * st.nphase;
+  const int total = st.ph[0].ntaps * (st.Ka / BLOCK_K);
+  const int rounds = (num_tiles + max_pairs - 1) / max_pairs;
+  *static_units = (long long)rounds * total;
+  *sk_units = ((long long)num_tiles * total + max_pairs - 1) / max_pairs + 35;
+}
 static bool pair_stream_k(const StageDev& st, int max_pairs) {
   const int mtiles = st.tiles_b * st.tiles_h * st.tiles_w;
   const int num_tiles = (mtiles + 1) / 2 * (st.n_pad / P_BN) * st.nphase;
   const int total = st.ph[0].ntaps * (st.Ka / BLOCK_K);
-  const int rounds = (num_tiles + max_pairs - 1) / max_pairs;
-  const long long static_units = (long long)rounds * total;
-  const long long sk_units = ((long long)num_tiles * total + max_pairs - 1) / max_pairs + 35;
+  long long static_units, sk_units;
+  pair_path_units(st, max_pairs, &static_units, &sk_units);
   static int sk_env = -1;
   if (sk_env < 0) { const char* e = getenv("LSNF_STREAMK"); sk_env = e ? atoi(e) : 2; }
   return (sk_env == 1 || (sk_env == 2 && sk_units < static_units)) && total >= 8 &&
          (long long)num_tiles * total >= 4LL * max_pairs && max_pairs <= 80;
+}
+static long long pair_units(const StageDev& st, int max_pairs) {
+  long long static_units, sk_units;
+  pair_path_units(st, max_pairs, &static_units, &sk_units);
+  return pair_stream_k(st, max_pairs) ? sk_units : static_units;
 }
 
 static int launch_pair(const StageHost& sh, cudaStream_t s) {
@@ -1043,10 +1173,119 @@
   launch_st.sk_enable = pair_stream_k(st, max_pairs);
   const int pairs = launch_st.sk_enable ? max_pairs : std::min(num_tiles, max_pairs);
   dim3 grid(2 * pairs, 1, 1);
+  const ChainDev none = {};
   if (st.passes == 1)
-    LSNF_CUDA(launch_k(tapgemm_tc2_kernel<true>, grid, dim3(TC_THREADS), P_SMEM_BYTES, s, sh.tmA, sh.tmB, sh.tmO, launch_st));
+    LSNF_CUDA(launch_k(tapgemm_tc2_kernel<true>, grid, dim3(TC_THREADS), P_SMEM_BYTES, s, sh.tmA, sh.tmB, sh.tmO,
+                       launch_st, sh.tmA, sh.tmB, sh.tmO, launch_st, none));
   else
-    LSNF_CUDA(launch_k(tapgemm_tc2_kernel<false>, grid, dim3(TC_THREADS), P_SMEM_BYTES, s, sh.tmA, sh.tmB, sh.tmO, launch_st));
+    LSNF_CUDA(launch_k(tapgemm_tc2_kernel<false>, grid, dim3(TC_THREADS), P_SMEM_BYTES, s, sh.tmA, sh.tmB, sh.tmO,
+                       launch_st, sh.tmA, sh.tmB, sh.tmO, launch_st, none));
+  return LSNF_OK;
+}
+
+static void chain_tiles(const StageDev& d, std::vector<int>* tiles) {
+  const int mtiles = d.tiles_b * d.tiles_h * d.tiles_w, m_pairs = (mtiles + 1) / 2, n_tiles = d.n_pad / P_BN;
+  for (int mp = 0; mp < m_pairs; ++mp)
+    for (int ph = 0; ph < d.nphase; ++ph)
+      for (int nt = 0; nt < n_tiles; ++nt) tiles->push_back((ph * n_tiles + nt) * m_pairs + mp);
+}
+static void pair_tile_samples(const StageDev& d, int t, int* b0, int* b1) {
+  const int mtiles = d.tiles_b * d.tiles_h * d.tiles_w, m_pairs = (mtiles + 1) / 2;
+  const int mp = t % m_pairs, per_b = d.tiles_h * d.tiles_w;
+  const int lo = std::min(2 * mp, mtiles - 1), hi = std::min(2 * mp + 1, mtiles - 1);
+  *b0 = lo / per_b * d.bB;
+  *b1 = std::min(d.B, (hi / per_b + 1) * d.bB);
+}
+static int units_per_tile(const StageDev& d) { return d.ph[0].ntaps * (d.Ka / BLOCK_K); }
+
+static long long chain_simulate(const StageDev& a, const StageDev& b, int pairs, int quota, std::vector<int32_t>* order) {
+  std::vector<int> prod, cons;
+  chain_tiles(a, &prod);
+  chain_tiles(b, &cons);
+  const long long ua = units_per_tile(a), ub = units_per_tile(b);
+  std::vector<int> pending(a.B, 0);
+  std::vector<long long> ready(a.B, 0);
+  for (int t : prod) {
+    int b0, b1;
+    pair_tile_samples(a, t, &b0, &b1);
+    for (int s = b0; s < b1; ++s) ++pending[s];
+  }
+  std::vector<long long> free_at(pairs, 0);
+  std::vector<char> on_cons(pairs, 0);
+  size_t ip = 0, ic = 0;
+  long long end = 0;
+  order->clear();
+  while (ip < prod.size() || ic < cons.size()) {
+    const int p = (int)(std::min_element(free_at.begin(), free_at.end()) - free_at.begin());
+    const long long now = free_at[p];
+    long long cons_ready = -1;
+    if (ic < cons.size()) {
+      int b0, b1;
+      pair_tile_samples(b, cons[ic], &b0, &b1);
+      cons_ready = 0;
+      for (int s = b0; s < b1 && cons_ready >= 0; ++s) cons_ready = pending[s] ? -1 : std::max(cons_ready, ready[s]);
+    }
+    bool take_cons = ic < cons.size() && ip == prod.size();
+    if (!take_cons && ic < cons.size() && cons_ready >= 0 && cons_ready <= now) {
+      int running = 0;
+      for (int q = 0; q < pairs; ++q) running += (q != p && on_cons[q] && free_at[q] > now) ? 1 : 0;
+      take_cons = running < quota;
+    }
+    if (take_cons) {
+      free_at[p] = std::max(now, cons_ready) + ub;
+      on_cons[p] = 1;
+      order->push_back((1 << 24) | cons[ic++]);
+    } else {
+      free_at[p] = now + ua;
+      on_cons[p] = 0;
+      int b0, b1;
+      pair_tile_samples(a, prod[ip], &b0, &b1);
+      for (int s = b0; s < b1; ++s) { --pending[s]; ready[s] = std::max(ready[s], free_at[p]); }
+      order->push_back(prod[ip++]);
+    }
+    end = std::max(end, free_at[p]);
+  }
+  return end;
+}
+
+static long long chain_best(const StageDev& a, const StageDev& b, int pairs, std::vector<int32_t>* order) {
+  long long best = -1;
+  std::vector<int32_t> o;
+  for (int quota = 0; quota <= pairs; quota += std::max(1, pairs / 37)) {
+    const long long t = chain_simulate(a, b, pairs, quota, &o);
+    if (best < 0 || t < best) { best = t; if (order) order->swap(o); }
+  }
+  return best;
+}
+
+void tc_chain_order(const StageDev& a, const StageDev& b, int num_sms, std::vector<int32_t>* order, int32_t* target) {
+  chain_best(a, b, std::max(1, num_sms / 2), order);
+  *target = a.nphase * (a.n_pad / P_BN) * a.tiles_h * a.tiles_w;
+}
+
+bool tc_chain_ok(const StageHost& a, const StageHost& b) {
+  const StageDev &x = a.dev, &y = b.dev;
+  if (!(use_pair(a) && use_pair(b) && x.passes == y.passes && x.fp16 == y.fp16 && x.epi == y.epi &&
+        x.out_single == y.out_single && x.epi == EPI_ACT_HL && b.a_off == a.out_off &&
+        x.B == y.B && x.tiles_b * x.tiles_h * x.tiles_w < (1 << 24) / 2 && y.tiles_b * y.tiles_h * y.tiles_w < (1 << 24) / 2))
+    return false;
+  const int pairs = 148 / 2;
+  return chain_best(x, y, pairs, nullptr) < pair_units(x, pairs) + pair_units(y, pairs) + 15;
+}
+
+int launch_tapgemm_tc_chain(const StageHost& a, const StageHost& b, const ChainDev& ch, int max_pairs, cudaStream_t s) {
+  if (!a.maps_ready || !b.maps_ready) { set_error("tensor maps not encoded"); return LSNF_ERR_STATE; }
+  StageDev da = a.dev, db = b.dev;
+  da.sk_enable = db.sk_enable = 0;
+  int pairs = std::min(ch.n_items, a.num_sms / 2);
+  if (max_pairs > 0) pairs = std::min(pairs, max_pairs);
+  dim3 grid(2 * std::max(pairs, 1), 1, 1);
+  if (da.passes == 1)
+    LSNF_CUDA(launch_k(tapgemm_tc2_kernel<true>, grid, dim3(TC_THREADS), P_SMEM_BYTES, s, a.tmA, a.tmB, a.tmO, da,
+                       b.tmA, b.tmB, b.tmO, db, ch));
+  else
+    LSNF_CUDA(launch_k(tapgemm_tc2_kernel<false>, grid, dim3(TC_THREADS), P_SMEM_BYTES, s, a.tmA, a.tmB, a.tmO, da,
+                       b.tmA, b.tmB, b.tmO, db, ch));
   return LSNF_OK;
 }
 
```
